# unanan/UNet_Nested4Tiny_Objects_Keypoints

Hardware: AMD Instinct MI355X
Metric: images/sec (train step) UNet++ L=4 256x256 (higher is better)
Workload: dtype f32

## Files before the change

### include/unetpp_hip.h

```cpp
#ifndef UNETPP_HIP_H
#define UNETPP_HIP_H

#include <stdint.h>

#ifdef __cplusplus
extern "C" {
#endif

#define UNETPP_ABI_VERSION 13
#define UNETPP_MAX_VIEWS 8

#define UNETPP_OK 0
#define UNETPP_EINVAL (-1)
#define UNETPP_ELAUNCH (-2)

typedef struct unetpp_view {
  float* ptr;
  int32_t C, c_off, c_len;
  int32_t Hs, Ws;
  int32_t sy, sx, oy, ox;
  const float* scale;
  const float* shift;
  const float* gate;
  int32_t relu;
  int32_t accumulate;
  int32_t gate_sum;
  int32_t reserved;
} unetpp_view;

#define UNETPP_GEMM_DIRECT 1
#define UNETPP_GEMM_BF16 2
typedef struct unetpp_bn_fused {
  const float* gamma;
  const float* beta;
  float* running_mean;
  float* running_var;
  float* mean;
  float* invstd;
  float* scale;
  float* shift;
  int64_t count;
  float eps, momentum;
} unetpp_bn_fused;

typedef struct unetpp_gemm_desc {
  int32_t N, H, W;
  int32_t taps;
  int32_t n_in;
  int32_t n_out;
  int32_t flags;
  int32_t reserved;
  unetpp_view in[UNETPP_MAX_VIEWS];
  unetpp_view out[UNETPP_MAX_VIEWS];
  const float* weight;
  const float* bias;
  float* stats_partial;
  const float* weight_image;
  unetpp_bn_fused bn;
} unetpp_gemm_desc;

typedef struct unetpp_wgrad_desc {
  int32_t N, H, W;
  int32_t taps;
  int32_t n_x;
  int32_t n_dy;
  unetpp_view x[UNETPP_MAX_VIEWS];
  unetpp_view dy[UNETPP_MAX_VIEWS];
  int32_t n_split;
  int32_t flags;
  float* slabs;
} unetpp_wgrad_desc;

int unetpp_abi_version(void);
const char* unetpp_build_arch(void);

const char* unetpp_last_kernel_name(void);

int unetpp_debug_set(const char* name, int64_t value, int32_t set);
int unetpp_debug_get(const char* name, int64_t* value);

int32_t unetpp_set_reserved_cus(int32_t n);
int32_t unetpp_usable_cus(int32_t* physical);

int64_t unetpp_gemm_pixel_blocks(int32_t N, int32_t H, int32_t W);
int64_t unetpp_gemm_stats_rows(int32_t N, int32_t H, int32_t W);
typedef struct unetpp_gemm_sizes {
  int64_t image_floats;
  int64_t bn_rows;
  int32_t workgroups, threads;
  const char* kernel;
} unetpp_gemm_sizes;
int unetpp_gemm_plan(const unetpp_gemm_desc* d, int32_t cus, unetpp_gemm_sizes* out);
int unetpp_gemm_fwd(const unetpp_gemm_desc* d, void* stream);
int64_t unetpp_gemm_weight_image_floats(const unetpp_gemm_desc* d);
int unetpp_gemm_pack_weight_image(const unetpp_gemm_desc* d, float* image, void* stream);
typedef struct unetpp_weight_src {
  const float* src;
  int64_t s_t, s_k, s_ko, s_n, s_no;
  int32_t k_inner, n_inner, flip, reserved;
} unetpp_weight_src;
int unetpp_gemm_pack_weight_image_from(const unetpp_gemm_desc* d, const unetpp_weight_src* src, float* image, void* stream);
typedef struct unetpp_pack_job {
  unetpp_weight_src src;
  float* image;
  int32_t taps, flags, n_in, n_out;
  int32_t in_len[UNETPP_MAX_VIEWS], out_len[UNETPP_MAX_VIEWS];
} unetpp_pack_job;
int unetpp_gemm_pack_weight_images(const unetpp_pack_job* jobs_device, int32_t n_jobs, int64_t max_image_floats,
                                   void* stream);

typedef struct unetpp_wgrad_sizes {
  int32_t n_split;
  int32_t planes;
  int32_t pairs_per_workgroup;
  int32_t reserved;
  int64_t slab_floats;
  const char* kernel;
} unetpp_wgrad_sizes;
int unetpp_wgrad_plan(const unetpp_wgrad_desc* d, int32_t target_blocks, unetpp_wgrad_sizes* out);
int unetpp_wgrad(const unetpp_wgrad_desc* d, void* stream);
int unetpp_wgrad_finish(const float* slabs, int32_t n_split, int32_t taps, int32_t K, int32_t Ncols, int32_t n_inner,
                        float* dw, int64_t d_t, int64_t d_k, int64_t d_n, int64_t d_o, float* db, void* stream);

int unetpp_pack_weight(float* dst, const float* src, int32_t T, int32_t K, int32_t Ncols,
                       int64_t d_t, int64_t d_k, int64_t d_n, int64_t s_t, int64_t s_k, int64_t s_n,
                       int32_t flip, void* stream);
typedef struct unetpp_copy_job {
  const float* src;
  float* dst;
  int64_t n_outer, n_inner, src_stride, dst_stride;
} unetpp_copy_job;
int unetpp_copy_jobs(const unetpp_copy_job* jobs_device, int32_t n_jobs, int64_t max_elems, void* stream);

int unetpp_bn_finalize(const float* partial, int64_t n_blocks, int32_t C, int64_t count,
                       const float* gamma, const float* beta, float eps, float momentum,
                       float* running_mean, float* running_var,
                       float* mean, float* invstd, float* scale, float* shift, void* stream);
int unetpp_bn_eval_coeffs(const float* gamma, const float* beta, const float* running_mean,
                          const float* running_var, float eps, int32_t C, float* scale, float* shift,
                          void* stream);
int unetpp_bn_eval_coeffs_stats(const float* gamma, const float* beta, const float* running_mean,
                                const float* running_var, float eps, int32_t C, float* scale, float* shift,
                                float* mean, float* invstd, void* stream);
int unetpp_affine_relu_pool(const float* y, const float* scale, const float* shift, int32_t relu,
                            int32_t N, int32_t H, int32_t W, int32_t C,
                            float* act, float* pooled, uint8_t* pool_idx, void* stream);
int unetpp_maxpool_bwd(const float* d_pooled, const uint8_t* pool_idx, int32_t N, int32_t H, int32_t W,
                       int32_t C, float* d_act, void* stream);
int64_t unetpp_bn_bwd_blocks(int64_t pixels, int32_t C);
int unetpp_bn_bwd_reduce(const float* d_act, const float* y, const float* scale, const float* shift,
                         const float* mean, const float* invstd, int64_t pixels, int32_t C,
                         float* partial, void* stream);
int unetpp_bn_bwd_finalize(const float* partial, int64_t n_blocks, int32_t C, float* dgamma, float* dbeta,
                           void* stream);
int unetpp_bn_bwd_apply(const float* d_act, const float* y, const float* scale, const float* shift,
                        const float* mean, const float* invstd, const float* gamma,
                        const float* dgamma, const float* dbeta, int64_t pixels, int32_t C,
                        float* dy, void* stream);

int unetpp_bn_bwd_pool_ok(int32_t N, int32_t H, int32_t W, int32_t C);
int unetpp_bn_bwd_reduce_pool(const float* d_act, const float* y, const float* scale, const float* shift,
                              const float* mean, const float* invstd, const float* d_pooled, const uint8_t* pool_idx,
                              int32_t N, int32_t H, int32_t W, int32_t C, float* partial, void* stream);
int unetpp_bn_bwd_apply_pool(const float* d_act, const float* y, const float* scale, const float* shift,
                             const float* mean, const float* invstd, const float* gamma, const float* dgamma,
                             const float* dbeta, const float* d_pooled, const uint8_t* pool_idx, int32_t N, int32_t H,
                             int32_t W, int32_t C, float* dy, void* stream);

int64_t unetpp_bn_frozen_bwd_blocks(int64_t pixels, int32_t C);
int unetpp_bn_frozen_bwd(const float* d_act, const float* y, const float* scale, const float* shift,
                         const float* mean, const float* invstd, const float* d_pooled, const uint8_t* pool_idx,
                         int32_t N, int32_t H, int32_t W, int32_t C, float* dy, float* partial, void* stream);

int unetpp_head_fwd(const float* x, const float* weight, const float* bias, int32_t N, int32_t H, int32_t W,
                    int32_t C, int32_t n_cls, float p_drop, uint64_t seed, const uint8_t* mask, const uint64_t* seed_dev,
                    float* out_nchw, void* stream);
int64_t unetpp_head_bwd_blocks(int64_t pixels);
int unetpp_head_bwd(const float* d_out_nchw, const float* out_nchw, const float* x, const float* weight,
                    int32_t N, int32_t H, int32_t W, int32_t C, int32_t n_cls, float p_drop, uint64_t seed,
                    const uint8_t* mask, const uint64_t* seed_dev, float* dx, int32_t accumulate, int32_t gate_x, float* partial,
                    void* stream);
int unetpp_head_train(const float* x, const float* weight, const float* bias, const float* target_nchw, int32_t N,
                      int32_t H, int32_t W, int32_t C, int32_t n_cls, float p_drop, uint64_t seed, const uint8_t* mask,
                      const uint64_t* seed_dev, int64_t rows, float gamma, int32_t n_heads, float* out_nchw, float* dx,
                      int32_t gate_x, float* partial, void* stream);
int unetpp_sum_partials(const float* partial, int64_t n_blocks, int64_t len, float* out, void* stream);

int unetpp_bilinear2x_fwd(const float* x, int32_t N, int32_t H, int32_t W, int32_t C, float* y, void* stream);
int unetpp_bilinear2x_bwd(const float* dy, int32_t N, int32_t H, int32_t W, int32_t C, float* dx, int32_t accumulate,
                          void* stream);

int64_t unetpp_focal_bce_blocks(int64_t n);
int unetpp_focal_bce(const float* pred, const float* target, int64_t n, int64_t rows, float gamma, float* grad,
                     float* partial, float* loss, void* stream);
#define UNETPP_MAX_HEADS 8
typedef struct unetpp_focal_heads {
  const float* pred[UNETPP_MAX_HEADS];
  float* grad[UNETPP_MAX_HEADS];
  int32_t n_heads, reserved;
} unetpp_focal_heads;
int unetpp_focal_bce_heads(const unetpp_focal_heads* heads, const float* target, int64_t n, int64_t rows, float gamma,
                           float* partial, float* loss, void* stream);
int64_t unetpp_topk_focal_workspace_bytes(int32_t n_heads, int64_t rows, int64_t P);
int unetpp_topk_focal_heads(const unetpp_focal_heads* heads, const float* target, int64_t rows, int64_t P, int64_t k,
                            int64_t denom, float gamma, void* workspace, float* kth, float* loss, void* stream);
int64_t unetpp_pr_focal_workspace_bytes(int32_t n_heads, int64_t n);
int unetpp_pr_focal_heads(const unetpp_focal_heads* heads, const float* target, int64_t n, float alpha, float beta,
                          float eps, float positive, void* workspace, int64_t* n_pos, float* loss ,
                          void* stream);
int unetpp_focal_bce_heads_ignore(const unetpp_focal_heads* heads, const float* target, int64_t n, int64_t rows,
                                  float gamma, float* partial, float* loss, void* stream);
int unetpp_topk_focal_heads_ignore(const unetpp_focal_heads* heads, const float* target, int64_t rows, int64_t P,
                                   int64_t k, int64_t denom, float gamma, void* workspace, float* kth, float* loss,
                                   void* stream);
int unetpp_pr_focal_heads_ignore(const unetpp_focal_heads* heads, const float* target, int64_t n, float alpha, float beta,
                                 float eps, float positive, void* workspace, int64_t* n_pos,
                                 float* loss , void* stream);
typedef struct unetpp_head_src {
  const void* x;
  const float* weight;
  const float* bias;
} unetpp_head_src;
typedef struct unetpp_heads_mean {
  unetpp_head_src head[UNETPP_MAX_HEADS];
  int32_t n_heads, reserved;
} unetpp_heads_mean;
int unetpp_heads_mean_fwd(const unetpp_heads_mean* heads, int32_t N, int32_t H, int32_t W, int32_t C, int32_t n_cls,
                          float* out_nchw, void* stream);
int unetpp_heads_mean_fwd_bf16(const unetpp_heads_mean* heads, int32_t N, int32_t H, int32_t W, int32_t C,
                               int32_t n_cls, float* out_nchw, void* stream);
typedef struct unetpp_head_grad {
  void* dx;
  float* partial;
  int32_t accumulate, gate_x;
} unetpp_head_grad;
typedef struct unetpp_heads_mean_grad {
  unetpp_head_grad head[UNETPP_MAX_HEADS];
  int32_t n_heads, reserved;
} unetpp_heads_mean_grad;
int unetpp_heads_mean_bwd(const unetpp_heads_mean* heads, const unetpp_heads_mean_grad* grads, const float* d_out_nchw,
                          int32_t N, int32_t H, int32_t W, int32_t C, int32_t n_cls, void* stream);
int unetpp_heads_mean_bwd_bf16(const unetpp_heads_mean* heads, const unetpp_heads_mean_grad* grads,
                               const float* d_out_nchw, int32_t N, int32_t H, int32_t W, int32_t C, int32_t n_cls,
                               void* stream);
int64_t unetpp_heatmap_workspace_bytes(int32_t N, int32_t H, int32_t W);
int unetpp_create_heatmap(const float* points, int32_t N, int32_t P, int32_t H, int32_t W, float radius,
                          float* out_nchw, void* workspace, void* stream);

int unetpp_nchw_to_nhwc(const float* src, int32_t N, int32_t C, int32_t H, int32_t W, float* dst, void* stream);
int unetpp_nhwc_to_nchw(const float* src, int32_t N, int32_t C, int32_t H, int32_t W, float* dst, void* stream);

int unetpp_affine_relu_pool_bf16(const void* y, const float* scale, const float* shift, int32_t relu,
                                 int32_t N, int32_t H, int32_t W, int32_t C,
                                 void* act, void* pooled, uint8_t* pool_idx, void* stream);
int64_t unetpp_bn_bwd_blocks_bf16(int64_t pixels, int32_t C);
int unetpp_bn_bwd_reduce_bf16(const void* d_act, const void* y, const float* scale, const float* shift,
                              const float* mean, const float* invstd, const void* d_pooled, const uint8_t* pool_idx,
                              int32_t N, int32_t H, int32_t W, int32_t C, float* partial, void* stream);
int unetpp_bn_bwd_apply_bf16(const void* d_act, const void* y, const float* scale, const float* shift,
                             const float* mean, const float* invstd, const float* gamma, const float* dgamma,
                             const float* dbeta, const void* d_pooled, const uint8_t* pool_idx,
                             int32_t N, int32_t H, int32_t W, int32_t C, void* dy, void* stream);
int64_t unetpp_bn_frozen_bwd_blocks_bf16(int64_t pixels, int32_t C);
int unetpp_bn_frozen_bwd_bf16(const void* d_act, const void* y, const float* scale, const float* shift,
                              const float* mean, const float* invstd, const void* d_pooled, const uint8_t* pool_idx,
                              int32_t N, int32_t H, int32_t W, int32_t C, void* dy, float* partial, void* stream);
int unetpp_head_fwd_bf16(const void* x, const float* weight, const float* bias, int32_t N, int32_t H, int32_t W,
                         int32_t C, int32_t n_cls, float p_drop, uint64_t seed, const uint8_t* mask, const uint64_t* seed_dev,
                         float* out_nchw, void* stream);
int unetpp_head_bwd_bf16(const float* d_out_nchw, const float* out_nchw, const void* x, const float* weight,
                         int32_t N, int32_t H, int32_t W, int32_t C, int32_t n_cls, float p_drop, uint64_t seed,
                         const uint8_t* mask, const uint64_t* seed_dev, void* dx, int32_t accumulate, int32_t gate_x, float* partial,
                         void* stream);

int unetpp_maxpool_bwd_bf16(const void* d_pooled, const uint8_t* pool_idx, int32_t N, int32_t H, int32_t W, int32_t C,
                            void* d_act, const void* gate, void* stream);
int unetpp_bilinear2x_fwd_bf16(const void* x, int32_t N, int32_t H, int32_t W, int32_t C, void* y, void* stream);
int unetpp_bilinear2x_bwd_bf16(const void* dy, int32_t N, int32_t H, int32_t W, int32_t C, void* dx, int32_t accumulate,
                               const void* gate, void* stream);

int unetpp_first_layer_dgrad_bf16(const void* dy, const float* weight, int32_t N, int32_t H, int32_t W, int32_t CIN,
                                  int32_t COUT, float* dx, void* stream);

int64_t unetpp_heatmap_pattern_workspace_bytes(int32_t N, int32_t n_maps, int32_t H, int32_t W);
int unetpp_heatmap_pattern(const float* points, int32_t N, int32_t P, const int32_t* map_points,
                           const int32_t* map_begin, int32_t n_maps, int32_t H, int32_t W, float radius,
                           float* out_nchw, void* workspace, void* stream);
int64_t unetpp_keypoints_workspace_bytes(int32_t maps, int32_t H, int32_t W, int32_t max_regions);
int unetpp_keypoints_extract(int32_t stage, const float* heat, int32_t maps, int32_t H, int32_t W,
                             const float* thr_per_map, int32_t num, int32_t max_regions, int32_t sweeps,
                             void* workspace, int32_t* changed, float* points, int32_t* counts, void* stream);

#define UNETPP_OPTIM_ADAMW 0
#define UNETPP_OPTIM_ADABOUND 1
#define UNETPP_OPTIM_SGDW 2
#define UNETPP_OPTIM_AMS 1
#define UNETPP_OPTIM_CAPTURABLE 2
#define UNETPP_OPTIM_HYPER 8
#define UNETPP_OPTIM_H_MAX_NORM 7
#define UNETPP_OPTIM_SKIP_NONFINITE 4

typedef struct unetpp_optim_segment {
  float* param;
  const float* grad;
  float* exp_avg;
  float* exp_avg_sq;
  float* aux;
  float* step;
  int64_t numel;
  int64_t chunk_begin;
  int32_t group;
  int32_t vec;
} unetpp_optim_segment;

int64_t unetpp_optim_chunk_elems(void);
int unetpp_optim_step(int32_t kind, int32_t flags, const unetpp_optim_segment* segments, int32_t n_segments,
                      const int32_t* chunk_segment, int64_t n_chunks, const double* hyper, const double* steps,
                      int32_t* done, void* stream);
int unetpp_optim_upload(void* dst, const void* host_src, int64_t bytes, void* stream);

typedef struct unetpp_clip_state {
  float total_norm;
  float coef;
  int32_t skipped_steps;
  int32_t reserved;
} unetpp_clip_state;

int unetpp_grad_norm(const unetpp_optim_segment* segments, int32_t n_segments, const int32_t* chunk_segment,
                     int64_t n_chunks, double* partials, void* stream);
int unetpp_optim_step_clip(int32_t kind, int32_t flags, const unetpp_optim_segment* segments, int32_t n_segments,
                           const int32_t* chunk_segment, int64_t n_chunks, const double* hyper, const double* steps,
                           int32_t* done, const double* partials, unetpp_clip_state* state, void* stream);
int unetpp_grad_scale(const unetpp_optim_segment* segments, int32_t n_segments, const int32_t* chunk_segment,
                      int64_t n_chunks, const double* partials, float max_norm, unetpp_clip_state* state, void* stream);

#define UNETPP_MATCH_MAX 64

int unetpp_match_points(const float* points, const int32_t* found, int32_t heads, int32_t N, int32_t C, int32_t K,
                        const float* labels, int32_t S, const int32_t* map_points, const int32_t* map_begin,
                        float* matched, uint8_t* mask, float* loss, int32_t* count, void* stream);

#define UNETPP_AVG_MEAN 0
#define UNETPP_AVG_EMA 1
#define UNETPP_AVG_SWAP 2
#define UNETPP_AVG_CAPTURABLE 1

typedef struct unetpp_avg_segment {
  float* avg;
  float* src;
  int64_t numel;
  int64_t chunk_begin;
  int32_t vec;
  int32_t copy;
} unetpp_avg_segment;

int unetpp_avg_update(int32_t kind, int32_t flags, const unetpp_avg_segment* segments, int32_t n_segments,
                      const int32_t* chunk_segment, int64_t n_chunks, int64_t count, double decay, float* count_dev,
                      const double* hyper_dev, int32_t* done, void* stream);

#define UNETPP_WARP_PARAMS 16
#define UNETPP_WARP_MAX_C 8
#define UNETPP_STORE_U8 0
#define UNETPP_STORE_F32 1

int unetpp_warp_batch(const void* store, int32_t store_type, int64_t M, int32_t Hs, int32_t Ws, int32_t C,
                      const int64_t* index, int32_t N, const float* params, const float* mul, const float* add,
                      float fill, float* out, int32_t Ho, int32_t Wo, const float* labels, int32_t S,
                      float* labels_out, uint8_t* inside, void* stream);

typedef struct unetpp_augment {
  float p_flip_h, p_flip_v;
  int32_t rot90;
  float max_deg;
  float scale_lo, scale_hi;
  float max_tx, max_ty;
  float gain_lo, gain_hi;
  float max_bias;
  int32_t reserved;
} unetpp_augment;

int unetpp_augment_draw(float* params, int32_t N, uint64_t seed, int32_t Hs, int32_t Ws, int32_t Ho, int32_t Wo,
                        const unetpp_augment* augment, void* stream);

#define UNETPP_SCENE_MAX_VARIANTS 8
#define UNETPP_SCENE_FLIP_X 1
#define UNETPP_SCENE_FLIP_Y 2
#define UNETPP_SCENE_TRANSPOSE 4

typedef struct unetpp_scene_rect {
  int32_t frame;
  int32_t oy, ox;
  int32_t y_lo, y_hi, x_lo, x_hi;
  int32_t reserved;
} unetpp_scene_rect;

int unetpp_scene_stitch(const float* tiles, int32_t n_tiles, int32_t K, int32_t C, int32_t Th, int32_t Tw,
// ... 35 lines not shown
```

### unet_nested4tiny_objects_keypoints_amd/_lib.py

```python
from __future__ import annotations

import ctypes as C
import os
import subprocess

_PKG_DIR = os.path.dirname(os.path.abspath(__file__))
_REPO = os.path.dirname(_PKG_DIR)
LIB_PATH = os.environ.get("UNETPP_LIB", os.path.join(_PKG_DIR, "libunetpp_hip.so"))
CSRC = os.path.join(_PKG_DIR, "csrc")
INCLUDE = os.path.join(_REPO, "include")
SOURCES = ("gemm_pix.hip", "gemm_fast.hip", "gemm_pw.hip", "gemm_pw_bf16.hip", "gemm_wino.hip", "gemm_bf16.hip", "gemm_bf16_dma.hip", "wgrad_bf16.hip", "pointwise_bf16.hip", "keypoints.hip", "weight_image.hip", "wgrad.hip", "wgrad_fast.hip", "wgrad_dma.hip", "wgrad_pw.hip", "wgrad_wino.hip", "first_layer.hip", "pointwise.hip", "heads.hip", "caller.hip", "optim.hip", "validate.hip", "average.hip", "loader.hip", "scene.hip",
           "detect.hip", "crops.hip", "topk_loss.hip", "pr_focal.hip")
HEADERS = ("common.h", "gemm_units.h", "wgrad_reduce.h", "lds_asm.h", "bf16_common.h", "dropout.h", "bn_fused.h",
           "wino_experiments.h", "dma_experiments.h", "heads_mean.h", "head_select.h", "focal_element.h", "multi_tensor.h")
MAX_VIEWS = 8
ABI_VERSION = 13
EXTRA_FLAGS = {"gemm_wino.hip": ("-fno-slp-vectorize",), "wgrad_wino.hip": ("-fno-slp-vectorize",)}
GEMM_DIRECT = 1
GEMM_BF16 = 2


class View(C.Structure):
    _fields_ = [
        ("ptr", C.c_void_p),
        ("C", C.c_int32), ("c_off", C.c_int32), ("c_len", C.c_int32),
        ("Hs", C.c_int32), ("Ws", C.c_int32),
        ("sy", C.c_int32), ("sx", C.c_int32), ("oy", C.c_int32), ("ox", C.c_int32),
        ("scale", C.c_void_p), ("shift", C.c_void_p), ("gate", C.c_void_p),
        ("relu", C.c_int32), ("accumulate", C.c_int32), ("gate_sum", C.c_int32), ("reserved", C.c_int32),
    ]


class BnFused(C.Structure):
    _fields_ = [
        ("gamma", C.c_void_p), ("beta", C.c_void_p), ("running_mean", C.c_void_p), ("running_var", C.c_void_p),
        ("mean", C.c_void_p), ("invstd", C.c_void_p), ("scale", C.c_void_p), ("shift", C.c_void_p),
        ("count", C.c_int64), ("eps", C.c_float), ("momentum", C.c_float),
    ]


class GemmDesc(C.Structure):
    _fields_ = [
        ("N", C.c_int32), ("H", C.c_int32), ("W", C.c_int32),
        ("taps", C.c_int32), ("n_in", C.c_int32), ("n_out", C.c_int32),
        ("flags", C.c_int32), ("reserved", C.c_int32),
        ("inp", View * MAX_VIEWS), ("out", View * MAX_VIEWS),
        ("weight", C.c_void_p), ("bias", C.c_void_p), ("stats_partial", C.c_void_p),
        ("weight_image", C.c_void_p),
        ("bn", BnFused),
    ]


class WeightSrc(C.Structure):
    _fields_ = [
        ("src", C.c_void_p),
        ("s_t", C.c_int64), ("s_k", C.c_int64), ("s_ko", C.c_int64), ("s_n", C.c_int64), ("s_no", C.c_int64),
        ("k_inner", C.c_int32), ("n_inner", C.c_int32), ("flip", C.c_int32), ("reserved", C.c_int32),
    ]


class PackJob(C.Structure):
    _fields_ = [
        ("src", WeightSrc),
        ("image", C.c_void_p),
        ("taps", C.c_int32), ("flags", C.c_int32), ("n_in", C.c_int32), ("n_out", C.c_int32),
        ("in_len", C.c_int32 * MAX_VIEWS), ("out_len", C.c_int32 * MAX_VIEWS),
    ]


class CopyJob(C.Structure):
    _fields_ = [
        ("src", C.c_void_p), ("dst", C.c_void_p),
        ("n_outer", C.c_int64), ("n_inner", C.c_int64), ("src_stride", C.c_int64), ("dst_stride", C.c_int64),
    ]


MAX_HEADS = 8


class FocalHeads(C.Structure):
    _fields_ = [
        ("pred", C.c_void_p * MAX_HEADS), ("grad", C.c_void_p * MAX_HEADS),
        ("n_heads", C.c_int32), ("reserved", C.c_int32),
    ]


class HeadSrc(C.Structure):
    _fields_ = [("x", C.c_void_p), ("weight", C.c_void_p), ("bias", C.c_void_p)]


class HeadsMean(C.Structure):
    _fields_ = [("head", HeadSrc * MAX_HEADS), ("n_heads", C.c_int32), ("reserved", C.c_int32)]


class HeadGrad(C.Structure):
    _fields_ = [("dx", C.c_void_p), ("partial", C.c_void_p), ("accumulate", C.c_int32), ("gate_x", C.c_int32)]


class HeadsMeanGrad(C.Structure):
    _fields_ = [("head", HeadGrad * MAX_HEADS), ("n_heads", C.c_int32), ("reserved", C.c_int32)]


class WgradDesc(C.Structure):
    _fields_ = [
        ("N", C.c_int32), ("H", C.c_int32), ("W", C.c_int32),
        ("taps", C.c_int32), ("n_x", C.c_int32), ("n_dy", C.c_int32),
        ("x", View * MAX_VIEWS), ("dy", View * MAX_VIEWS),
        ("n_split", C.c_int32), ("flags", C.c_int32),
        ("slabs", C.c_void_p),
    ]


class WgradSizes(C.Structure):
    _fields_ = [
        ("n_split", C.c_int32), ("planes", C.c_int32), ("pairs_per_workgroup", C.c_int32), ("reserved", C.c_int32),
        ("slab_floats", C.c_int64),
        ("kernel", C.c_char_p),
    ]


class GemmSizes(C.Structure):
    _fields_ = [
        ("image_floats", C.c_int64), ("bn_rows", C.c_int64),
        ("workgroups", C.c_int32), ("threads", C.c_int32),
        ("kernel", C.c_char_p),
    ]


class OptimSegment(C.Structure):
    _fields_ = [
        ("param", C.c_void_p), ("grad", C.c_void_p), ("exp_avg", C.c_void_p), ("exp_avg_sq", C.c_void_p),
        ("aux", C.c_void_p), ("step", C.c_void_p),
        ("numel", C.c_int64), ("chunk_begin", C.c_int64), ("group", C.c_int32), ("vec", C.c_int32),
    ]


class ClipState(C.Structure):
    _fields_ = [("total_norm", C.c_float), ("coef", C.c_float), ("skipped_steps", C.c_int32), ("reserved", C.c_int32)]


class AvgSegment(C.Structure):
    _fields_ = [
        ("avg", C.c_void_p), ("src", C.c_void_p),
        ("numel", C.c_int64), ("chunk_begin", C.c_int64), ("vec", C.c_int32), ("copy", C.c_int32),
    ]


class AugmentDesc(C.Structure):
    _fields_ = [
        ("p_flip_h", C.c_float), ("p_flip_v", C.c_float), ("rot90", C.c_int32), ("max_deg", C.c_float),
        ("scale_lo", C.c_float), ("scale_hi", C.c_float), ("max_tx", C.c_float), ("max_ty", C.c_float),
        ("gain_lo", C.c_float), ("gain_hi", C.c_float), ("max_bias", C.c_float), ("reserved", C.c_int32),
    ]


class SceneRect(C.Structure):
    _fields_ = [
        ("frame", C.c_int32), ("oy", C.c_int32), ("ox", C.c_int32),
        ("y_lo", C.c_int32), ("y_hi", C.c_int32), ("x_lo", C.c_int32), ("x_hi", C.c_int32), ("reserved", C.c_int32),
    ]


OPTIM_ADAMW, OPTIM_ADABOUND, OPTIM_SGDW = 0, 1, 2
OPTIM_AMS, OPTIM_CAPTURABLE = 1, 2
OPTIM_SKIP_NONFINITE = 4
OPTIM_HYPER = 8
OPTIM_H_MAX_NORM = 7
AVG_MEAN, AVG_EMA, AVG_SWAP = 0, 1, 2
AVG_CAPTURABLE = 1
WARP_PARAMS, WARP_MAX_C = 16, 8
STORE_U8, STORE_F32 = 0, 1
SCENE_MAX_VARIANTS = 8
SCENE_FLIP_X, SCENE_FLIP_Y, SCENE_TRANSPOSE = 1, 2, 4
PEAKS_MAX_RADIUS, PEAKS_MAX_MAPS = 8, 65535
MATCH_MAX = 64

_P, _I32, _I64, _F, _U64 = C.c_void_p, C.c_int32, C.c_int64, C.c_float, C.c_uint64

SIGNATURES = {
    "unetpp_abi_version": (C.c_int, []),
    "unetpp_build_arch": (C.c_char_p, []),
    "unetpp_last_kernel_name": (C.c_char_p, []),
    "unetpp_set_reserved_cus": (_I32, [_I32]),
    "unetpp_debug_set": (C.c_int, [C.c_char_p, _I64, _I32]),
    "unetpp_debug_get": (C.c_int, [C.c_char_p, C.POINTER(C.c_int64)]),
    "unetpp_usable_cus": (_I32, [C.POINTER(C.c_int32)]),
    "unetpp_gemm_pixel_blocks": (_I64, [_I32, _I32, _I32]),
    "unetpp_gemm_stats_rows": (_I64, [_I32, _I32, _I32]),
    "unetpp_gemm_plan": (C.c_int, [C.POINTER(GemmDesc), _I32, C.POINTER(GemmSizes)]),
    "unetpp_gemm_fwd": (C.c_int, [C.POINTER(GemmDesc), _P]),
    "unetpp_gemm_weight_image_floats": (_I64, [C.POINTER(GemmDesc)]),
    "unetpp_gemm_pack_weight_image": (C.c_int, [C.POINTER(GemmDesc), _P, _P]),
    "unetpp_gemm_pack_weight_image_from": (C.c_int, [C.POINTER(GemmDesc), C.POINTER(WeightSrc), _P, _P]),
    "unetpp_gemm_pack_weight_images": (C.c_int, [_P, _I32, _I64, _P]),
    "unetpp_wgrad_plan": (C.c_int, [C.POINTER(WgradDesc), _I32, C.POINTER(WgradSizes)]),
    "unetpp_wgrad": (C.c_int, [C.POINTER(WgradDesc), _P]),
    "unetpp_wgrad_finish": (C.c_int, [_P, _I32, _I32, _I32, _I32, _I32, _P, _I64, _I64, _I64, _I64, _P, _P]),
    "unetpp_pack_weight": (C.c_int, [_P, _P, _I32, _I32, _I32, _I64, _I64, _I64, _I64, _I64, _I64, _I32, _P]),
    "unetpp_bn_finalize": (C.c_int, [_P, _I64, _I32, _I64, _P, _P, _F, _F, _P, _P, _P, _P, _P, _P, _P]),
    "unetpp_bn_eval_coeffs": (C.c_int, [_P, _P, _P, _P, _F, _I32, _P, _P, _P]),
    "unetpp_affine_relu_pool": (C.c_int, [_P, _P, _P, _I32, _I32, _I32, _I32, _I32, _P, _P, _P, _P]),
    "unetpp_maxpool_bwd": (C.c_int, [_P, _P, _I32, _I32, _I32, _I32, _P, _P]),
    "unetpp_bn_bwd_blocks": (_I64, [_I64, _I32]),
    "unetpp_bn_bwd_reduce": (C.c_int, [_P, _P, _P, _P, _P, _P, _I64, _I32, _P, _P]),
    "unetpp_bn_bwd_finalize": (C.c_int, [_P, _I64, _I32, _P, _P, _P]),
    "unetpp_bn_bwd_apply": (C.c_int, [_P, _P, _P, _P, _P, _P, _P, _P, _P, _I64, _I32, _P, _P]),
    "unetpp_bn_bwd_pool_ok": (C.c_int, [_I32, _I32, _I32, _I32]),
    "unetpp_bn_bwd_reduce_pool": (C.c_int, [_P, _P, _P, _P, _P, _P, _P, _P, _I32, _I32, _I32, _I32, _P, _P]),
    "unetpp_bn_bwd_apply_pool": (C.c_int, [_P, _P, _P, _P, _P, _P, _P, _P, _P, _P, _P, _I32, _I32, _I32, _I32, _P, _P]),
    "unetpp_head_fwd": (C.c_int, [_P, _P, _P, _I32, _I32, _I32, _I32, _I32, _F, _U64, _P, _P, _P, _P]),
    "unetpp_head_bwd_blocks": (_I64, [_I64]),
    "unetpp_head_bwd": (C.c_int, [_P, _P, _P, _P, _I32, _I32, _I32, _I32, _I32, _F, _U64, _P, _P, _P, _I32, _I32, _P, _P]),
    "unetpp_head_train": (C.c_int, [_P, _P, _P, _P, _I32, _I32, _I32, _I32, _I32, _F, _U64, _P, _P, _I64, _F, _I32, _P, _P,
                                    _I32, _P, _P]),
    "unetpp_sum_partials": (C.c_int, [_P, _I64, _I64, _P, _P]),
    "unetpp_focal_bce_blocks": (_I64, [_I64]),
    "unetpp_focal_bce": (C.c_int, [_P, _P, _I64, _I64, _F, _P, _P, _P, _P]),
    "unetpp_focal_bce_heads": (C.c_int, [C.POINTER(FocalHeads), _P, _I64, _I64, _F, _P, _P, _P]),
    "unetpp_heads_mean_fwd": (C.c_int, [C.POINTER(HeadsMean), _I32, _I32, _I32, _I32, _I32, _P, _P]),
    "unetpp_heads_mean_fwd_bf16": (C.c_int, [C.POINTER(HeadsMean), _I32, _I32, _I32, _I32, _I32, _P, _P]),
    "unetpp_heads_mean_bwd": (C.c_int, [C.POINTER(HeadsMean), C.POINTER(HeadsMeanGrad), _P, _I32, _I32, _I32, _I32, _I32, _P]),
    "unetpp_heads_mean_bwd_bf16": (C.c_int, [C.POINTER(HeadsMean), C.POINTER(HeadsMeanGrad), _P, _I32, _I32, _I32, _I32, _I32,
                                             _P]),
    "unetpp_bn_eval_coeffs_stats": (C.c_int, [_P, _P, _P, _P, _F, _I32, _P, _P, _P, _P, _P]),
    "unetpp_bn_frozen_bwd_blocks": (_I64, [_I64, _I32]),
    "unetpp_bn_frozen_bwd": (C.c_int, [_P, _P, _P, _P, _P, _P, _P, _P, _I32, _I32, _I32, _I32, _P, _P, _P]),
    "unetpp_bn_frozen_bwd_blocks_bf16": (_I64, [_I64, _I32]),
    "unetpp_bn_frozen_bwd_bf16": (C.c_int, [_P, _P, _P, _P, _P, _P, _P, _P, _I32, _I32, _I32, _I32, _P, _P, _P]),
    "unetpp_copy_jobs": (C.c_int, [_P, _I32, _I64, _P]),
    "unetpp_heatmap_workspace_bytes": (_I64, [_I32, _I32, _I32]),
    "unetpp_create_heatmap": (C.c_int, [_P, _I32, _I32, _I32, _I32, _F, _P, _P, _P]),
    "unetpp_bilinear2x_fwd": (C.c_int, [_P, _I32, _I32, _I32, _I32, _P, _P]),
    "unetpp_bilinear2x_bwd": (C.c_int, [_P, _I32, _I32, _I32, _I32, _P, _I32, _P]),
    "unetpp_nchw_to_nhwc": (C.c_int, [_P, _I32, _I32, _I32, _I32, _P, _P]),
    "unetpp_nhwc_to_nchw": (C.c_int, [_P, _I32, _I32, _I32, _I32, _P, _P]),
    "unetpp_affine_relu_pool_bf16": (C.c_int, [_P, _P, _P, _I32, _I32, _I32, _I32, _I32, _P, _P, _P, _P]),
    "unetpp_bn_bwd_blocks_bf16": (_I64, [_I64, _I32]),
    "unetpp_bn_bwd_reduce_bf16": (C.c_int, [_P, _P, _P, _P, _P, _P, _P, _P, _I32, _I32, _I32, _I32, _P, _P]),
    "unetpp_bn_bwd_apply_bf16": (C.c_int, [_P, _P, _P, _P, _P, _P, _P, _P, _P, _P, _P, _I32, _I32, _I32, _I32, _P, _P]),
    "unetpp_head_fwd_bf16": (C.c_int, [_P, _P, _P, _I32, _I32, _I32, _I32, _I32, _F, _U64, _P, _P, _P, _P]),
    "unetpp_first_layer_dgrad_bf16": (C.c_int, [_P, _P, _I32, _I32, _I32, _I32, _I32, _P, _P]),
    "unetpp_maxpool_bwd_bf16": (C.c_int, [_P, _P, _I32, _I32, _I32, _I32, _P, _P, _P]),
    "unetpp_bilinear2x_fwd_bf16": (C.c_int, [_P, _I32, _I32, _I32, _I32, _P, _P]),
    "unetpp_bilinear2x_bwd_bf16": (C.c_int, [_P, _I32, _I32, _I32, _I32, _P, _I32, _P, _P]),
    "unetpp_heatmap_pattern_workspace_bytes": (_I64, [_I32, _I32, _I32, _I32]),
    "unetpp_heatmap_pattern": (C.c_int, [_P, _I32, _I32, _P, _P, _I32, _I32, _I32, _F, _P, _P, _P]),
    "unetpp_keypoints_workspace_bytes": (_I64, [_I32, _I32, _I32, _I32]),
    "unetpp_keypoints_extract": (C.c_int, [_I32, _P, _I32, _I32, _I32, _P, _I32, _I32, _I32, _P, _P, _P, _P, _P]),
    "unetpp_head_bwd_bf16": (C.c_int, [_P, _P, _P, _P, _I32, _I32, _I32, _I32, _I32, _F, _U64, _P, _P, _P, _I32, _I32, _P, _P]),
    "unetpp_optim_chunk_elems": (_I64, []),
    "unetpp_optim_step": (C.c_int, [_I32, _I32, _P, _I32, _P, _I64, _P, _P, _P, _P]),
    "unetpp_optim_upload": (C.c_int, [_P, _P, _I64, _P]),
    "unetpp_match_points": (C.c_int, [_P, _P, _I32, _I32, _I32, _I32, _P, _I32, _P, _P, _P, _P, _P, _P, _P]),
    "unetpp_avg_update": (C.c_int, [_I32, _I32, _P, _I32, _P, _I64, _I64, C.c_double, _P, _P, _P, _P]),
    "unetpp_grad_norm": (C.c_int, [_P, _I32, _P, _I64, _P, _P]),
    "unetpp_optim_step_clip": (C.c_int, [_I32, _I32, _P, _I32, _P, _I64, _P, _P, _P, _P, _P, _P]),
    "unetpp_grad_scale": (C.c_int, [_P, _I32, _P, _I64, _P, _F, _P, _P]),
    "unetpp_warp_batch": (C.c_int, [_P, _I32, _I64, _I32, _I32, _I32, _P, _I32, _P, _P, _P, _F, _P, _I32, _I32, _P, _I32,
                                    _P, _P, _P]),
    "unetpp_augment_draw": (C.c_int, [_P, _I32, _U64, _I32, _I32, _I32, _I32, C.POINTER(AugmentDesc), _P]),
    "unetpp_scene_stitch": (C.c_int, [_P, _I32, _I32, _I32, _I32, _I32, C.POINTER(C.c_int32), C.POINTER(SceneRect), _P, _P,
                                      _I32, _I32, _I32, _P]),
    "unetpp_scene_screen": (C.c_int, [_P, _I32, _I32, _I32, _I32, C.POINTER(SceneRect), _P, _I32, _F, _P, _P, _P]),
    "unetpp_peaks_workspace_bytes": (_I64, [_I32, _I32, _I32]),
    "unetpp_peaks_detect": (C.c_int, [_P, _I32, _I32, _I32, _F, _I32, _I32, _I32, _P, _P, _P, _P, _P]),
    "unetpp_detect_match": (C.c_int, [_P, _P, _P, _I32, _I32, _I32, _P, _P, _I32, _F, _P, _P, _P, _P]),
    "unetpp_points_target": (C.c_int, [_P, _P, _I64, _I32, _P, _I32, _P, _I32, _I32, _I32, _F, _P, _P]),
    "unetpp_crops_draw": (C.c_int, [_P, _P, _P, _I32, _U64, _I32, _I32, _I32, _I32, _I32, _P, _P, _I32, _F, _F, _F,
                                    C.POINTER(AugmentDesc), _P]),
    "unetpp_topk_focal_workspace_bytes": (_I64, [_I32, _I64, _I64]),
    "unetpp_topk_focal_heads": (C.c_int, [C.POINTER(FocalHeads), _P, _I64, _I64, _I64, _I64, _F, _P, _P, _P, _P]),
    "unetpp_pr_focal_workspace_bytes": (_I64, [_I32, _I64]),
    "unetpp_pr_focal_heads": (C.c_int, [C.POINTER(FocalHeads), _P, _I64, _F, _F, _F, _F, _P, _P, _P, _P]),
    "unetpp_focal_bce_heads_ignore": (C.c_int, [C.POINTER(FocalHeads), _P, _I64, _I64, _F, _P, _P, _P]),
    "unetpp_topk_focal_heads_ignore": (C.c_int, [C.POINTER(FocalHeads), _P, _I64, _I64, _I64, _I64, _F, _P, _P, _P, _P]),
    "unetpp_pr_focal_heads_ignore": (C.c_int, [C.POINTER(FocalHeads), _P, _I64, _F, _F, _F, _F, _P, _P, _P, _P]),
    "unetpp_target_ignore": (C.c_int, [_P, _P, _I64, _I32, _P, _I32, _P, _I32, _I32, _I32, _I32, _I32, _I32, _P, _P]),
}

_LIB = None


def source_hash() -> str:
    import hashlib
    h = hashlib.sha256()
    for path in [os.path.join(CSRC, s) for s in SOURCES + HEADERS] + [os.path.join(INCLUDE, "unetpp_hip.h")]:
        with open(path, "rb") as f:
            h.update(f.read())
    return h.hexdigest()[:16]


def build_library(force: bool = False, verbose: bool = False, out_path: str = None, obj_dir: str = None) -> str:
    srcs = [os.path.join(CSRC, s) for s in SOURCES]
    deps = srcs + [os.path.join(CSRC, h) for h in HEADERS] + [os.path.join(INCLUDE, "unetpp_hip.h")]
    lib_path = out_path or LIB_PATH
    if not force and os.path.exists(lib_path) and all(os.path.getmtime(lib_path) >= os.path.getmtime(d) for d in deps):
        return lib_path
    hipcc = os.environ.get("HIPCC", "/opt/rocm/bin/hipcc")
    common = [hipcc, "--offload-arch=gfx950", "-O3", "-std=c++17", "-fPIC", "-I", INCLUDE, "-I", CSRC]
    obj_dir = obj_dir or os.path.join(_REPO, "build", "obj")
    os.makedirs(obj_dir, exist_ok=True)
    jobs = []
    for src in SOURCES:
        obj = os.path.join(obj_dir, src.replace(".hip", ".o"))
        cmd = common + list(EXTRA_FLAGS.get(src, ())) + ["-c", os.path.join(CSRC, src), "-o", obj]
        if verbose:
            print(" ".join(cmd))
        jobs.append((obj, cmd, subprocess.Popen(cmd)))
    for obj, cmd, proc in jobs:
        if proc.wait() != 0:
            raise subprocess.CalledProcessError(proc.returncode, cmd)
    staged = os.path.join(obj_dir, os.path.basename(lib_path) + ".link")
    link = [hipcc, "--offload-arch=gfx950", "-shared", "-fPIC", "-o", staged] + [j[0] for j in jobs]
    if verbose:
        print(" ".join(link))
    subprocess.run(link, check=True)
    os.replace(staged, lib_path)
    if out_path is None:
        global _LIB
        _LIB = None
    return lib_path


def lib():
    global _LIB
    if _LIB is None:
        if not os.path.exists(LIB_PATH):
            raise RuntimeError(
                "unetpp HIP library not built: %s is missing. Run `python -c 'import __graft_entry__ as g; g.build()'` "
                "(there is no CPU fallback for this path)." % LIB_PATH)
        handle = C.CDLL(LIB_PATH)
        for name, (res, args) in SIGNATURES.items():
            fn = getattr(handle, name)
            fn.restype = res
            fn.argtypes = args
        if handle.unetpp_abi_version() != ABI_VERSION:
            raise RuntimeError("unetpp HIP library ABI mismatch")
        _LIB = handle
    return _LIB


def check(status: int, what: str) -> None:
    if status != 0:
        raise RuntimeError("%s failed with status %d (%s)" % (
            what, status, {-1: "invalid argument", -2: "kernel launch error"}.get(status, "unknown")))


class debug_switch:

    def __init__(self, name: str, value: int):
        self.name, self.value = name.encode(), int(value)
        self._before = None

    def __enter__(self):
        old = C.c_int64(0)
        state = lib().unetpp_debug_get(self.name, C.byref(old))
        if state < 0:
            check(state, "unetpp_debug_get")
        self._before = (state == 1, int(old.value))
        check(lib().unetpp_debug_set(self.name, self.value, 1), "unetpp_debug_set")
        return self

    def __exit__(self, *exc):
        was_set, value = self._before
        check(lib().unetpp_debug_set(self.name, value if was_set else 0, 1 if was_set else 0), "unetpp_debug_set")
        return False
```

### unet_nested4tiny_objects_keypoints_amd/csrc/common.h

```cpp
#pragma once
#include <hip/hip_runtime.h>
#include <stdint.h>

#include <atomic>

#include "unetpp_hip.h"

typedef float f32x16 __attribute__((ext_vector_type(16)));
typedef float f32x4 __attribute__((ext_vector_type(4)));

namespace unetpp {

constexpr int kBlockPixels = 256;
constexpr int kThreads = 256;
constexpr int kMaxHaloPixels = 340;

struct TileGeom {
  int log2tw, tiles_x, tiles_y;
};

inline TileGeom tile_geom(int H, int W) {
  int l = 3;
  while ((1 << l) < W && l < 5) ++l;
  TileGeom g;
  g.log2tw = l;
  const int TW = 1 << l, TH = kBlockPixels >> l;
  g.tiles_x = (W + TW - 1) / TW;
  g.tiles_y = (H + TH - 1) / TH;
  return g;
}

template <int OFF>
__device__ __forceinline__ float xor_lane(float v) {
  static_assert(OFF == 1 || OFF == 2 || OFF == 4 || OFF == 8 || OFF == 16, "xor_lane: 1, 2, 4, 8 or 16");
  const int i = __builtin_bit_cast(int, v);
  int r;
  if constexpr (OFF == 1) r = __builtin_amdgcn_mov_dpp(i, 0xB1, 0xF, 0xF, true);
  else if constexpr (OFF == 2) r = __builtin_amdgcn_mov_dpp(i, 0x4E, 0xF, 0xF, true);
  else r = __builtin_amdgcn_ds_swizzle(i, 0x1F | (OFF << 10));
  return __builtin_bit_cast(float, r);
}

__device__ __forceinline__ float row16_sum(float v) {
  v += xor_lane<1>(v);
  v += xor_lane<2>(v);
  v += __builtin_bit_cast(float, __builtin_amdgcn_mov_dpp(__builtin_bit_cast(int, v), 0x141, 0xF, 0xF, true));
  v += __builtin_bit_cast(float, __builtin_amdgcn_mov_dpp(__builtin_bit_cast(int, v), 0x140, 0xF, 0xF, true));
  return v;
}

__device__ __forceinline__ float relu_keep_nan(float v) { return !(v <= 0.f) ? v : 0.f; }
__device__ __forceinline__ float relu_floor(bool relu) { return relu ? 0.f : -__builtin_inff(); }
__device__ __forceinline__ float floor_keep_nan(float v, float floor_v) { return !(v <= floor_v) ? v : floor_v; }

__device__ __forceinline__ bool pool_takes(float t, float best) { return t > best || t != t; }

inline int finish_log2_groups(int n_split) {
  int l = 0;
  while ((1 << l) < n_split && l < 4) ++l;
  return l;
}

inline bool view_ok(const unetpp_view& v, bool need_ptr = true) {
  if (need_ptr && v.ptr == nullptr) return false;
  if (v.C <= 0 || v.c_len <= 0 || v.c_off < 0 || v.c_off + v.c_len > v.C) return false;
  if (v.Hs <= 0 || v.Ws <= 0 || v.sy <= 0 || v.sx <= 0 || v.oy < 0 || v.ox < 0) return false;
  if ((v.scale == nullptr) != (v.shift == nullptr)) return false;
  return true;
}

inline bool view_covers(const unetpp_view& v, int H, int W) {
  return (H - 1) * v.sy + v.oy < v.Hs && (W - 1) * v.sx + v.ox < v.Ws;
}

__device__ __forceinline__ bool view_vec4(const unetpp_view& v) {
  return ((v.C | v.c_off) & 3) == 0 && ((reinterpret_cast<uintptr_t>(v.ptr) & 15) == 0) &&
         (v.gate == nullptr || (reinterpret_cast<uintptr_t>(v.gate) & 15) == 0);
}

__device__ __forceinline__ long view_pixel_offset(const unetpp_view& v, int n, int y, int x) {
  return ((static_cast<long>(n) * v.Hs + (y * v.sy + v.oy)) * v.Ws + (x * v.sx + v.ox)) * v.C + v.c_off;
}

__device__ __forceinline__ f32x4 view_load4(const unetpp_view& v, long off, int c, int rem, bool vec) {
  f32x4 val = {0.f, 0.f, 0.f, 0.f};
  const float* p = v.ptr + off + c;
  if (vec && rem >= 4) {
    val = *reinterpret_cast<const f32x4*>(p);
  } else {
#pragma unroll
    for (int i = 0; i < 4; ++i)
      if (i < rem) val[i] = p[i];
  }
  if (v.scale != nullptr) {
#pragma unroll
    for (int i = 0; i < 4; ++i)
      if (i < rem) val[i] = fmaf(val[i], v.scale[c + i], v.shift[c + i]);
  }
  if (v.relu) {
#pragma unroll
    for (int i = 0; i < 4; ++i) val[i] = relu_keep_nan(val[i]);
  }
  if (v.gate != nullptr) {
    const float* g = v.gate + off + c;
#pragma unroll
    for (int i = 0; i < 4; ++i)
      if (i < rem) val[i] = (g[i] > 0.f) ? val[i] : 0.f;
  }
  return val;
}

inline hipStream_t ST(void* s) { return static_cast<hipStream_t>(s); }
inline bool aligned16(const void* p) { return (reinterpret_cast<uintptr_t>(p) & 15) == 0; }
inline unsigned grid_for(long items, long cap = 2048 * 8) {
  long b = (items + kThreads - 1) / kThreads;
  if (b < 1) b = 1;
  if (b > cap) b = cap;
  return static_cast<unsigned>(b);
}

inline int launch_status() { return hipGetLastError() == hipSuccess ? UNETPP_OK : UNETPP_ELAUNCH; }

constexpr int kMaxDevices = 64;
inline bool allow_dynamic_lds(const void* func, int bytes, std::atomic<bool> (&raised)[kMaxDevices]) {
  int dev = 0;
  if (hipGetDevice(&dev) != hipSuccess || dev < 0 || dev >= kMaxDevices) return false;
  if (raised[dev].load(std::memory_order_acquire)) return true;
  if (hipFuncSetAttribute(func, hipFuncAttributeMaxDynamicSharedMemorySize, bytes) != hipSuccess) return false;
  raised[dev].store(true, std::memory_order_release);
  return true;
}

int reserved_cus();
inline int physical_cu_count() {
  static int cached[64] = {};
  int dev = 0;
  if (hipGetDevice(&dev) != hipSuccess || dev < 0) return 0;
  if (dev < 64 && cached[dev] > 0) return cached[dev];
  int cus = 0;
  if (hipDeviceGetAttribute(&cus, hipDeviceAttributeMultiprocessorCount, dev) != hipSuccess || cus <= 0) return 0;
  if (dev < 64) cached[dev] = cus;
  return cus;
}
inline int device_cu_count() {
  const int cus = physical_cu_count();
  if (cus <= 0) return 0;
  const int left = cus - reserved_cus();
  return left < 8 ? (cus < 8 ? cus : 8) : left;
}

void note_kernel(const char* name);

enum Opt {
  OPT_BF16_NO_DMA,
  OPT_BF16_DMA_ALL,
  OPT_BF16_DMA_MIN8,
  OPT_BF16_DMA_FORM,
  OPT_BF16_DMA_SMALL,
  OPT_BF16_DMA_STATS,
  OPT_BF16_DMA_POINTWISE,
  OPT_BF16_DMA_SPLIT,
  OPT_BF16_WGRAD_QUAD,
  OPT_WINO_NO_LEAN,
  OPT_WINO_ONE_PER_CU,
  OPT_MEMSET_NODES,
  OPT_BF16_PW_PLAIN,
  OPT_PW_DIRECT,
  OPT_PW_NT,
  OPT_HEAD_WGS_PER_CU,
  OPT_SMALL_WGRAD_BLOCKS,
  OPT_COUNT
};
bool opt_is_set(Opt o);
long opt_value(Opt o, long dflt);

struct FastArgs;
struct GemmSel;
int gemm_select(const unetpp_gemm_desc* d, int cus, GemmSel& s);
bool gemm_image_of(const unetpp_gemm_desc* d, GemmSel& s);
bool small_cin_fwd_applies(const unetpp_gemm_desc* d);
void small_cin_fwd_plan(const unetpp_gemm_desc* d, GemmSel& s);
int launch_small_cin_fwd(const unetpp_gemm_desc* d, const GemmSel& s, hipStream_t st);
bool gemm_pw_bf16_applies(const unetpp_gemm_desc* d, GemmSel& s);
int launch_gemm_pw_bf16(const unetpp_gemm_desc* d, const GemmSel& s, hipStream_t st);
bool gemm_bf16_dma_applies(const unetpp_gemm_desc* d, GemmSel& s);
int launch_gemm_bf16_dma(const unetpp_gemm_desc* d, const GemmSel& s, hipStream_t st);
bool bf16_gemm_args(const unetpp_gemm_desc* d, FastArgs& a);
void gemm_bf16_plan(const unetpp_gemm_desc* d, GemmSel& s);
int launch_gemm_bf16(const unetpp_gemm_desc* d, const GemmSel& s, hipStream_t st);
bool wino_applies(const unetpp_gemm_desc* d);
void gemm_wino_plan(const unetpp_gemm_desc* d, GemmSel& s);
int launch_gemm_wino(const unetpp_gemm_desc* d, const GemmSel& s, hipStream_t st);
bool gemm_pw_applies(const unetpp_gemm_desc* d, GemmSel& s);
int launch_gemm_pw(const unetpp_gemm_desc* d, const GemmSel& s, hipStream_t st);
void gemm_fast_plan(const unetpp_gemm_desc* d, GemmSel& s);
int launch_gemm_fast(const unetpp_gemm_desc* d, const GemmSel& s, hipStream_t st);
enum WgradKernel {
  WGRAD_FIRST_LAYER, WGRAD_BF16_QUAD, WGRAD_BF16_PAIR, WGRAD_PW, WGRAD_WINO, WGRAD_DMA, WGRAD_FAST, WGRAD_GENERIC
};
struct WgradSel {
  WgradKernel kernel;
  const char* label;
  int planes;
  int pairs_per_workgroup;
  int max_split;
  int Ktot, Ncols;
  int k_tiles, n_tiles_cols;
};
int wgrad_select(const unetpp_wgrad_desc* d, WgradSel& s);
bool small_cin_wgrad_applies(const unetpp_wgrad_desc* d);
int launch_small_cin_wgrad(const unetpp_wgrad_desc* d, hipStream_t st);
bool wgrad_bf16_views_ok(const unetpp_wgrad_desc* d);
bool wgrad_bf16_quads(const unetpp_wgrad_desc* d);
int launch_wgrad_bf16(const unetpp_wgrad_desc* d, const WgradSel& s, hipStream_t st);
bool wgrad_pw_applies(const unetpp_wgrad_desc* d);
int launch_wgrad_pw(const unetpp_wgrad_desc* d, hipStream_t st);
bool wgrad_wino_applies(const unetpp_wgrad_desc* d);
int launch_wgrad_wino(const unetpp_wgrad_desc* d, const WgradSel& s, hipStream_t st);
int launch_wgrad_finish_wino(const float* slabs, int n_split, int K, int Ncols, float* dw, long d_t, long d_k, long d_n,
                             float* db, hipStream_t st);
bool wgrad_dma_applies(const unetpp_wgrad_desc* d);
int launch_wgrad_dma(const unetpp_wgrad_desc* d, const WgradSel& s, hipStream_t st);
bool wgrad_fast_applies(const unetpp_wgrad_desc* d);
int launch_wgrad_fast(const unetpp_wgrad_desc* d, const WgradSel& s, hipStream_t st);

}
```

### unet_nested4tiny_objects_keypoints_amd/csrc/gemm_pix.hip

```cpp
#include "bn_fused.h"
#include <atomic>
#include <cstdio>
#include <cstdlib>
#include <cstring>
#include <mutex>

#include "common.h"
#include "gemm_units.h"

namespace unetpp {
namespace {

constexpr int KC = 16;
constexpr int KCP = 20;
constexpr int WJ = 12;

struct GemmArgs {
  unetpp_gemm_desc d;
  int log2tw, tiles_x, tiles_y;
  int Ktot, Ncols;
};

template <int TAPS>
__global__ __launch_bounds__(kThreads, 2) void gemm_pix_kernel(const GemmArgs a) {
  constexpr int HALO = (TAPS == 9) ? 1 : 0;
  constexpr int IN_FLOATS = (TAPS == 9 ? kMaxHaloPixels : kBlockPixels) * KCP;
  constexpr int W_FLOATS = TAPS * (KC / 8) * 32 * WJ;
  __shared__ __attribute__((aligned(16))) float smem[IN_FLOATS + W_FLOATS];
  float* in_tile = smem;
  float* w_tile = smem + IN_FLOATS;

  const unetpp_gemm_desc& d = a.d;
  const int tid = threadIdx.x;
  const int wave = tid >> 6, lane = tid & 63, j = lane & 31, h = lane >> 5;

  int bid = blockIdx.x;
  const int txi = bid % a.tiles_x;
  bid /= a.tiles_x;
  const int tyi = bid % a.tiles_y;
  const int n = bid / a.tiles_y;
  const int TW = 1 << a.log2tw, TH = kBlockPixels >> a.log2tw;
  const int ty0 = tyi * TH, tx0 = txi * TW;
  const int HWp = TW + 2 * HALO, HHp = TH + 2 * HALO;
  const int npix = HWp * HHp;

  int ov = 0, nt = blockIdx.y, col_base = 0;
  while (ov < d.n_out - 1) {
    const int tiles_v = (d.out[ov].c_len + 31) >> 5;
    if (nt < tiles_v) break;
    nt -= tiles_v;
    col_base += d.out[ov].c_len;
    ++ov;
  }
  const unetpp_view& O = d.out[ov];
  const int n0 = col_base + nt * 32;
  const int n_cnt = min(32, O.c_len - nt * 32);

  int abase[2];
#pragma unroll
  for (int mt = 0; mt < 2; ++mt) {
    const int p = 64 * wave + 32 * mt + j;
    abase[mt] = ((p >> a.log2tw) * HWp + (p & (TW - 1))) * KCP + 4 * h;
  }
  const int wbase = j * WJ + 4 * h;

  f32x16 acc[2];
#pragma unroll
  for (int mt = 0; mt < 2; ++mt)
#pragma unroll
    for (int r = 0; r < 16; ++r) acc[mt][r] = 0.f;

  int kbase = 0;
  for (int s = 0; s < d.n_in; ++s) {
    const unetpp_view& V = d.in[s];
    const bool vec = view_vec4(V);
    for (int c0 = 0; c0 < V.c_len; c0 += KC) {
      const int c_cnt = min(KC, V.c_len - c0);
      __syncthreads();
      for (int it = tid; it < npix * (KC / 4); it += kThreads) {
        const int hp = it >> 2, cc = (it & 3) * 4;
        const int hy = hp / HWp, hx = hp - hy * HWp;
        const int y = ty0 + hy - HALO, x = tx0 + hx - HALO;
        f32x4 val = {0.f, 0.f, 0.f, 0.f};
        if (cc < c_cnt && y >= 0 && y < d.H && x >= 0 && x < d.W)
          val = view_load4(V, view_pixel_offset(V, n, y, x), c0 + cc, c_cnt - cc, vec);
        *reinterpret_cast<f32x4*>(&in_tile[hp * KCP + cc]) = val;
      }
      for (int it = tid; it < TAPS * (KC / 4) * 32; it += kThreads) {
        const int jj = it & 31, kq = (it >> 5) & 3, tap = it >> 7;
        f32x4 wv = {0.f, 0.f, 0.f, 0.f};
        if (jj < n_cnt) {
          const float* wp = d.weight + (static_cast<long>(tap) * a.Ktot + kbase + c0 + kq * 4) * a.Ncols + n0 + jj;
#pragma unroll
          for (int i = 0; i < 4; ++i)
            if (kq * 4 + i < c_cnt) wv[i] = wp[static_cast<long>(i) * a.Ncols];
        }
        *reinterpret_cast<f32x4*>(&w_tile[((tap * 2 + (kq >> 1)) * 32 + jj) * WJ + (kq & 1) * 4]) = wv;
      }
      __syncthreads();
      const int ngroups = (c_cnt + 7) >> 3;
#pragma unroll
      for (int tap = 0; tap < TAPS; ++tap) {
        const int toff = (TAPS == 9) ? ((tap / 3) * HWp + (tap % 3)) * KCP : 0;
#pragma unroll
        for (int g = 0; g < KC / 8; ++g) {
          if (g < ngroups) {
            const f32x4 b = *reinterpret_cast<const f32x4*>(&w_tile[(tap * 2 + g) * 32 * WJ + wbase]);
#pragma unroll
            for (int mt = 0; mt < 2; ++mt) {
              const f32x4 av = *reinterpret_cast<const f32x4*>(&in_tile[abase[mt] + toff + 8 * g]);
#pragma unroll
              for (int t = 0; t < 4; ++t)
                acc[mt] = __builtin_amdgcn_mfma_f32_32x32x2f32(av[t], b[t], acc[mt], 0, 0, 0);
            }
          }
        }
      }
    }
    kbase += V.c_len;
  }

  const bool col_ok = j < n_cnt;
  const float bj = (d.bias != nullptr && col_ok) ? d.bias[n0 + j] : 0.f;
  float s1 = 0.f, s2 = 0.f;
#pragma unroll
  for (int mt = 0; mt < 2; ++mt) {
#pragma unroll
    for (int r = 0; r < 16; ++r) {
      const int i = (r & 3) + 8 * (r >> 2) + 4 * h;
      const int p = 64 * wave + 32 * mt + i;
      const int y = ty0 + (p >> a.log2tw), x = tx0 + (p & (TW - 1));
      if (col_ok && y < d.H && x < d.W) {
        float v = acc[mt][r] + bj;
        v = floor_keep_nan(v, relu_floor(O.relu));
        s1 += v;
        s2 = fmaf(v, v, s2);
        const long off = view_pixel_offset(O, n, y, x) + nt * 32 + j;
        if (O.gate != nullptr && !O.gate_sum) v = (O.gate[off] > 0.f) ? v : 0.f;
        if (O.accumulate) v += O.ptr[off];
        if (O.gate != nullptr && O.gate_sum) v = (O.gate[off] > 0.f) ? v : 0.f;
        O.ptr[off] = v;
      }
    }
  }
  if (d.stats_partial != nullptr) {
    s1 += __shfl_xor(s1, 32);
    s2 += __shfl_xor(s2, 32);
    __syncthreads();
    if (h == 0) {
      smem[(wave * 32 + j) * 2 + 0] = s1;
      smem[(wave * 32 + j) * 2 + 1] = s2;
    }
    __syncthreads();
    if (tid < 32 && tid < n_cnt) {
      float t1 = 0.f, t2 = 0.f;
#pragma unroll
      for (int w = 0; w < 4; ++w) {
        t1 += smem[(w * 32 + tid) * 2 + 0];
        t2 += smem[(w * 32 + tid) * 2 + 1];
      }
      float* dst = d.stats_partial + (static_cast<long>(blockIdx.x) * a.Ncols + n0 + tid) * 2;
      dst[0] = t1;
      dst[1] = t2;
    }
  }
}

}
}

namespace unetpp {
namespace {
thread_local const char* g_last_kernel = "";

const char* const kOptNames[OPT_COUNT] = {
    "BF16_NO_DMA", "BF16_DMA_ALL", "BF16_DMA_MIN8", "BF16_DMA_FORM", "BF16_DMA_SMALL", "BF16_DMA_STATS",
    "BF16_DMA_POINTWISE", "BF16_DMA_SPLIT", "BF16_WGRAD_QUAD", "WINO_NO_LEAN", "WINO_ONE_PER_CU", "MEMSET_NODES",
    "BF16_PW_PLAIN", "PW_DIRECT", "PW_NT", "HEAD_WGS_PER_CU", "SMALL_WGRAD_BLOCKS"};
struct OptSlot {
  std::atomic<long> value{0};
  std::atomic<bool> set{false};
};
OptSlot g_opts[OPT_COUNT];
std::atomic<int> g_reserved_cus{0};
std::once_flag g_opts_once;

void opts_from_environment() {
  std::call_once(g_opts_once, [] {
    char name[64];
    for (int i = 0; i < OPT_COUNT; ++i) {
      snprintf(name, sizeof(name), "UNETPP_%s", kOptNames[i]);
      const char* e = getenv(name);
      if (e != nullptr) {
        char* end = nullptr;
        const long v = strtol(e, &end, 10);
        g_opts[i].value.store(end == e ? 1 : v, std::memory_order_relaxed);
        g_opts[i].set.store(true, std::memory_order_release);
      }
    }
    if (const char* e = getenv("UNETPP_RESERVED_CUS"); e != nullptr) {
      const int v = atoi(e);
      g_reserved_cus.store(v < 0 ? 0 : v, std::memory_order_relaxed);
    }
  });
}
}

bool opt_is_set(Opt o) {
  opts_from_environment();
  return g_opts[o].set.load(std::memory_order_acquire);
}
long opt_value(Opt o, long dflt) {
  opts_from_environment();
  return g_opts[o].set.load(std::memory_order_acquire) ? g_opts[o].value.load(std::memory_order_relaxed) : dflt;
}
int reserved_cus() {
  opts_from_environment();
  return g_reserved_cus.load(std::memory_order_relaxed);
}
void note_kernel(const char* name) { g_last_kernel = name; }
}

using namespace unetpp;

extern "C" const char* unetpp_last_kernel_name(void) { return g_last_kernel; }

extern "C" int unetpp_debug_set(const char* name, int64_t value, int32_t set) {
  if (name == nullptr) return UNETPP_EINVAL;
  opts_from_environment();
  for (int i = 0; i < OPT_COUNT; ++i)
    if (strcmp(name, kOptNames[i]) == 0) {
      g_opts[i].value.store(static_cast<long>(value), std::memory_order_relaxed);
      g_opts[i].set.store(set != 0, std::memory_order_release);
      return UNETPP_OK;
    }
  return UNETPP_EINVAL;
}

extern "C" int unetpp_debug_get(const char* name, int64_t* value) {
  if (name == nullptr) return UNETPP_EINVAL;
  opts_from_environment();
  for (int i = 0; i < OPT_COUNT; ++i)
    if (strcmp(name, kOptNames[i]) == 0) {
      if (!g_opts[i].set.load(std::memory_order_acquire)) return 0;
      if (value != nullptr) *value = g_opts[i].value.load(std::memory_order_relaxed);
      return 1;
    }
  return UNETPP_EINVAL;
}

extern "C" int32_t unetpp_set_reserved_cus(int32_t n) {
  opts_from_environment();
  if (n >= 0) {
    const int cus = physical_cu_count();
    const int cap = cus > 8 ? cus - 8 : 0;
    g_reserved_cus.store(n > cap ? cap : n, std::memory_order_relaxed);
  }
  return reserved_cus();
}

extern "C" int32_t unetpp_usable_cus(int32_t* physical) {
  if (physical != nullptr) *physical = physical_cu_count();
  return device_cu_count();
}

extern "C" int64_t unetpp_gemm_pixel_blocks(int32_t N, int32_t H, int32_t W) {
  if (N <= 0 || H <= 0 || W <= 0) return 0;
  const TileGeom g = tile_geom(H, W);
  return static_cast<int64_t>(N) * g.tiles_y * g.tiles_x;
}

extern "C" int64_t unetpp_gemm_stats_rows(int32_t N, int32_t H, int32_t W) {
  const int64_t blocks = unetpp_gemm_pixel_blocks(N, H, W);
  if (blocks <= 0) return 0;
  return blocks > kBnFusedRows ? blocks : kBnFusedRows;
}

bool unetpp::gemm_image_of(const unetpp_gemm_desc* d, GemmSel& s) {
  s.image_kind = s.image_kc = 0;
  s.image_floats = 0;
  if (d == nullptr) return false;
  const bool bf = (d->flags & UNETPP_GEMM_BF16) != 0, wino = wino_applies(d);
  const int kc = bf ? 32 : (wino ? 8 : 16);
  if (bf ? !bf16_gemm_args(d, s.fa) : !fast_args(d, s.fa, kc, 32)) return false;
  s.image_kind = bf ? kKindBf16 : (wino ? kKindWino : kKindFast);
  s.image_kc = kc;
  s.image_floats = static_cast<long>(s.fa.n_tiles) * s.fa.n_chunks * (wino ? 4096 : d->taps * 512L);
  return true;
}

namespace {
bool gemm_generic_applies(const unetpp_gemm_desc* d, GemmSel& s) {
  FastArgs& a = s.fa;
  a.Ktot = a.Ncols = a.n_tiles = 0;
  for (int i = 0; i < d->n_in; ++i) {
    if (!view_ok(d->in[i]) || !view_covers(d->in[i], d->H, d->W)) return false;
    a.Ktot += d->in[i].c_len;
  }
  for (int i = 0; i < d->n_out; ++i) {
    if (!view_ok(d->out[i]) || !view_covers(d->out[i], d->H, d->W)) return false;
    a.Ncols += d->out[i].c_len;
    a.n_tiles += (d->out[i].c_len + 31) / 32;
  }
  const TileGeom g = tile_geom(d->H, d->W);
  a.log2tw = g.log2tw;
  a.tiles_x = g.tiles_x;
  a.tiles_y = g.tiles_y;
  const int64_t pix_blocks = static_cast<int64_t>(d->N) * g.tiles_y * g.tiles_x;
  if (pix_blocks > 0x7fffffffLL || a.n_tiles > 65535) return false;
  s.kernel = GEMM_GENERIC;
  s.label = d->taps == 9 ? "gemm_pix_kernel<9>" : "gemm_pix_kernel<1>";
  s.grid_x = static_cast<unsigned>(pix_blocks);
  s.grid_y = static_cast<unsigned>(a.n_tiles);
  return true;
}

int launch_gemm_generic(const unetpp_gemm_desc* d, const GemmSel& s, hipStream_t st) {
  GemmArgs a;
  a.d = *d;
  a.log2tw = s.fa.log2tw;
  a.tiles_x = s.fa.tiles_x;
  a.tiles_y = s.fa.tiles_y;
  a.Ktot = s.fa.Ktot;
  a.Ncols = s.fa.Ncols;
  const dim3 grid(s.grid_x, s.grid_y);
  if (d->taps == 9)
    hipLaunchKernelGGL(gemm_pix_kernel<9>, grid, dim3(kThreads), 0, st, a);
  else
    hipLaunchKernelGGL(gemm_pix_kernel<1>, grid, dim3(kThreads), 0, st, a);
  return launch_status();
}
}

int unetpp::gemm_select(const unetpp_gemm_desc* d, int cus, GemmSel& s) {
  if (d == nullptr || d->N <= 0 || d->H <= 0 || d->W <= 0) return UNETPP_EINVAL;
  if (d->taps != 9 && d->taps != 1) return UNETPP_EINVAL;
  if (d->n_in < 1 || d->n_in > UNETPP_MAX_VIEWS || d->n_out < 1 || d->n_out > UNETPP_MAX_VIEWS) return UNETPP_EINVAL;
  if (d->weight == nullptr && d->weight_image == nullptr) return UNETPP_EINVAL;
  if (d->stats_partial != nullptr && d->n_out != 1) return UNETPP_EINVAL;
  const unetpp_bn_fused& bn = d->bn;
  if (bn.scale != nullptr &&
      (!d->stats_partial || !bn.gamma || !bn.beta || !bn.mean || !bn.invstd || !bn.shift || bn.count < 1 ||
       (bn.running_mean == nullptr) != (bn.running_var == nullptr) || d->n_out != 1))
    return UNETPP_EINVAL;
  const bool bf = (d->flags & UNETPP_GEMM_BF16) != 0;
  const bool has_image = gemm_image_of(d, s);
  s.cus = cus;
  s.grid_y = 1;
  s.threads = kThreads;
  s.lds_bytes = 0;
  s.bn_rows = 0;
  if (d->weight_image == nullptr) {
    const bool small = small_cin_fwd_applies(d);
    if (bf ? !small : !gemm_generic_applies(d, s)) return UNETPP_EINVAL;
    if (cus <= 0) return UNETPP_ELAUNCH;
    if (small) small_cin_fwd_plan(d, s);
    return UNETPP_OK;
  }
  if (!has_image) return UNETPP_EINVAL;
  if (cus <= 0) return UNETPP_ELAUNCH;
  if (bf) {
    if (!gemm_pw_bf16_applies(d, s) && !gemm_bf16_dma_applies(d, s)) gemm_bf16_plan(d, s);
  } else if (wino_applies(d)) {
    gemm_wino_plan(d, s);
  } else if (!gemm_pw_applies(d, s)) {
    gemm_fast_plan(d, s);
  }
  return UNETPP_OK;
}

extern "C" int unetpp_gemm_plan(const unetpp_gemm_desc* d, int32_t cus, unetpp_gemm_sizes* out) {
  GemmSel s;
  if (out == nullptr) return UNETPP_EINVAL;
  const int rc = gemm_select(d, cus > 0 ? cus : device_cu_count(), s);
  if (rc != UNETPP_OK) return rc;
  out->image_floats = s.image_floats;
  out->bn_rows = s.bn_rows;
  out->workgroups = static_cast<int32_t>(s.grid_x * s.grid_y);
  out->threads = static_cast<int32_t>(s.threads);
  out->kernel = s.label;
  return UNETPP_OK;
}

extern "C" int unetpp_gemm_fwd(const unetpp_gemm_desc* d, void* stream) {
  GemmSel s;
  int rc = gemm_select(d, device_cu_count(), s);
  if (rc != UNETPP_OK) return rc;
  hipStream_t st = static_cast<hipStream_t>(stream);
  note_kernel(s.label);
  switch (s.kernel) {
    case GEMM_SMALL_CIN: rc = launch_small_cin_fwd(d, s, st); break;
    case GEMM_BF16_PW: rc = launch_gemm_pw_bf16(d, s, st); break;
    case GEMM_BF16_DMA8:
    case GEMM_BF16_DMA4: rc = launch_gemm_bf16_dma(d, s, st); break;
    case GEMM_BF16: rc = launch_gemm_bf16(d, s, st); break;
    case GEMM_PW: rc = launch_gemm_pw(d, s, st); break;
    case GEMM_WINO: rc = launch_gemm_wino(d, s, st); break;
    case GEMM_FAST: rc = launch_gemm_fast(d, s, st); break;
    case GEMM_GENERIC: rc = launch_gemm_generic(d, s, st); break;
  }
  const unetpp_bn_fused& bn = d->bn;
  if (rc != UNETPP_OK || bn.scale == nullptr) return rc;
  const int64_t rows = s.bn_rows > 0 ? s.bn_rows : unetpp_gemm_pixel_blocks(d->N, d->H, d->W);
  const int fin = unetpp_bn_finalize(d->stats_partial, rows, d->out[0].c_len, bn.count, bn.gamma, bn.beta, bn.eps,
                                     bn.momentum, bn.running_mean, bn.running_var, bn.mean, bn.invstd, bn.scale, bn.shift,
                                     stream);
  note_kernel(s.label);
  return fin;
}
```

### unet_nested4tiny_objects_keypoints_amd/csrc/gemm_units.h

```cpp
#pragma once
#include "common.h"

namespace unetpp {

struct FastArgs {
  unetpp_gemm_desc d;
  int log2tw, tiles_x, tiles_y;
  int Ktot, Ncols, n_tiles, n_chunks;
  int nt_unit, n_groups;
  long total_blocks;
  int bn_in_kernel;
};

__device__ __forceinline__ unsigned view_pixel_offset32(const unetpp_view& v, int n, int y, int x) {
  return ((static_cast<unsigned>(n) * v.Hs + (y * v.sy + v.oy)) * v.Ws + (x * v.sx + v.ox)) * v.C + v.c_off;
}

__device__ __forceinline__ long xcd_remap(long bid, long total) {
  const long q = total >> 3, r = total & 7;
  const long xcd = bid & 7, idx = bid >> 3;
  return (xcd < r ? xcd * (q + 1) : r * (q + 1) + (xcd - r) * q) + idx;
}

struct UnitGeom {
  int n, ty0, tx0;
  int group;
  long patch;
};
struct TileCols {
  int nt, ov;
  int n0, n_cnt;
};

template <int LOG2N = 5>
__device__ __forceinline__ TileCols decode_tile(const FastArgs& a, int nt_global) {
  constexpr int NW = 1 << LOG2N;
  int nt = nt_global, ov = 0, col_base = 0;
  while (ov < a.d.n_out - 1) {
    const int tiles_v = (a.d.out[ov].c_len + NW - 1) >> LOG2N;
    if (nt < tiles_v) break;
    nt -= tiles_v;
    col_base += a.d.out[ov].c_len;
    ++ov;
  }
  TileCols t;
  t.nt = nt;
  t.ov = ov;
  t.n0 = col_base + nt * NW;
  t.n_cnt = min(NW, a.d.out[ov].c_len - nt * NW);
  return t;
}

template <int LOG2TW>
__device__ __forceinline__ UnitGeom decode_unit(const FastArgs& a, long lb) {
  constexpr int TW = 1 << LOG2TW, TH = kBlockPixels >> LOG2TW;
  UnitGeom g;
  unsigned bid = static_cast<unsigned>(lb);
  g.group = static_cast<int>(bid % static_cast<unsigned>(a.n_groups));
  bid /= static_cast<unsigned>(a.n_groups);
  g.patch = bid;
  const int txi = static_cast<int>(bid % static_cast<unsigned>(a.tiles_x));
  bid /= static_cast<unsigned>(a.tiles_x);
  const int tyi = static_cast<int>(bid % static_cast<unsigned>(a.tiles_y));
  g.n = static_cast<int>(bid / static_cast<unsigned>(a.tiles_y));
  g.ty0 = tyi * TH;
  g.tx0 = txi * TW;
  return g;
}

constexpr int kKindFast = 0, kKindWino = 1, kKindBf16 = 2;
enum GemmKernel {
  GEMM_SMALL_CIN, GEMM_BF16_PW, GEMM_BF16_DMA8, GEMM_BF16_DMA4, GEMM_BF16, GEMM_PW, GEMM_WINO, GEMM_FAST, GEMM_GENERIC
};
struct GemmSel {
  GemmKernel kernel;
  const char* label;
  int cus;
  int image_kind, image_kc;
  long image_floats;
  FastArgs fa;
  unsigned grid_x, grid_y, threads;
  int lds_bytes;
  long bn_rows;
  int qc, ncbp, plain, nt_store;
  int mode, narrow;
  int plain_out;
};

inline bool fast_args(const unetpp_gemm_desc* d, FastArgs& a, int kc, int ncol = 32) {
  if (d == nullptr || d->N <= 0 || d->H <= 0 || d->W <= 0) return false;
  if (d->taps != 9 && d->taps != 1) return false;
  if (d->n_in < 1 || d->n_in > UNETPP_MAX_VIEWS || d->n_out < 1 || d->n_out > UNETPP_MAX_VIEWS) return false;
  a.d = *d;
  a.bn_in_kernel = 0;
  a.Ktot = a.Ncols = a.n_tiles = a.n_chunks = 0;
  for (int i = 0; i < d->n_in; ++i) {
    const unetpp_view& v = d->in[i];
    if (!view_ok(v) || !view_covers(v, d->H, d->W)) return false;
    if (v.gate != nullptr) return false;
    if (v.scale != nullptr && ((reinterpret_cast<uintptr_t>(v.scale) | reinterpret_cast<uintptr_t>(v.shift)) & 15) != 0)
      return false;
    if (((v.C | v.c_off | v.c_len) & 3) != 0 || (reinterpret_cast<uintptr_t>(v.ptr) & 15) != 0) return false;
    if (static_cast<long>(d->N) * v.Hs * v.Ws * v.C >= 0x7fffffffL) return false;
    a.Ktot += v.c_len;
    a.n_chunks += (v.c_len + kc - 1) / kc;
  }
  for (int i = 0; i < d->n_out; ++i) {
    if (!view_ok(d->out[i]) || !view_covers(d->out[i], d->H, d->W)) return false;
    if (static_cast<long>(d->N) * d->out[i].Hs * d->out[i].Ws * d->out[i].C >= 0x7fffffffL) return false;
    a.Ncols += d->out[i].c_len;
    a.n_tiles += (d->out[i].c_len + ncol - 1) / ncol;
  }
  const TileGeom g = tile_geom(d->H, d->W);
  a.log2tw = g.log2tw;
  a.tiles_x = g.tiles_x;
  a.tiles_y = g.tiles_y;
  a.nt_unit = (d->taps == 1 && d->stats_partial == nullptr && a.n_tiles % 2 == 0) ? 2 : 1;
  a.n_groups = a.n_tiles / a.nt_unit;
  a.total_blocks = static_cast<long>(d->N) * g.tiles_y * g.tiles_x * a.n_groups;
  return a.total_blocks <= 0x7fffffffL;
}


struct UnitRange {
  long first, step, count;
};
__device__ __forceinline__ UnitRange my_unit_range(long total_blocks) {
  UnitRange u;
  const long W8 = gridDim.x >> 3;
  if (gridDim.x >= total_blocks) {
    u.first = xcd_remap(blockIdx.x, total_blocks);
    u.step = 0;
    u.count = 1;
  } else {
    const long q = total_blocks >> 3, r = total_blocks & 7;
    const long xcd = blockIdx.x & 7, widx = blockIdx.x >> 3;
    const long start = xcd < r ? xcd * (q + 1) : r * (q + 1) + (xcd - r) * q;
    const long cnt = q + (xcd < r ? 1 : 0);
    u.first = start + widx;
    u.step = W8;
    u.count = widx < cnt ? (cnt - widx + W8 - 1) / W8 : 0;
  }
  return u;
}

__device__ __forceinline__ UnitRange my_contiguous_unit_range(long total_blocks) {
  UnitRange u;
  const long W8 = gridDim.x >> 3;
  u.step = 1;
  if (gridDim.x >= total_blocks) {
    u.first = xcd_remap(blockIdx.x, total_blocks);
    u.count = 1;
  } else {
    const long q = total_blocks >> 3, r = total_blocks & 7;
    const long xcd = blockIdx.x & 7, widx = blockIdx.x >> 3;
    const long start = xcd < r ? xcd * (q + 1) : r * (q + 1) + (xcd - r) * q;
    const long cnt = q + (xcd < r ? 1 : 0);
    const long per = cnt / W8, rem = cnt % W8;
    u.first = start + widx * per + (widx < rem ? widx : rem);
    u.count = per + (widx < rem ? 1 : 0);
  }
  return u;
}

}
```

### unet_nested4tiny_objects_keypoints_amd/csrc/gemm_wino.hip

```cpp
#include <cstdlib>
#include <utility>

#include "bn_fused.h"
#include "common.h"
#include "gemm_units.h"
#include "lds_asm.h"
#include "wino_experiments.h"

namespace unetpp {
namespace {

typedef float f32x2 __attribute__((ext_vector_type(2)));
typedef unsigned u32x4v __attribute__((vector_size(16)));
constexpr unsigned kOutOfRange = 0x80000000u;
typedef const __attribute__((address_space(1))) void* gptr_t;
typedef __attribute__((address_space(3))) void* lptr_t;

__device__ __forceinline__ void wino_input_transform(const float (&dd)[16], float (&V)[16]) {
  float t[4][4];
#pragma unroll
  for (int j = 0; j < 4; ++j) {
    t[0][j] = dd[0 + j] - dd[8 + j];
    t[1][j] = dd[4 + j] + dd[8 + j];
    t[2][j] = dd[8 + j] - dd[4 + j];
    t[3][j] = dd[4 + j] - dd[12 + j];
  }
#pragma unroll
  for (int i = 0; i < 4; ++i) {
    V[4 * i + 0] = t[i][0] - t[i][2];
    V[4 * i + 1] = t[i][1] + t[i][2];
    V[4 * i + 2] = t[i][2] - t[i][1];
    V[4 * i + 3] = t[i][1] - t[i][3];
  }
}

__device__ __forceinline__ void wino_input_transform_pk(const f32x2_t (&dd)[8], float (&V)[16]) {
  f32x2_t t[8];
#pragma unroll
  for (int p = 0; p < 2; ++p) {
    t[0 + p] = pk_sub(dd[0 + p], dd[4 + p]);
    t[2 + p] = pk_add(dd[2 + p], dd[4 + p]);
    t[4 + p] = pk_sub(dd[4 + p], dd[2 + p]);
    t[6 + p] = pk_sub(dd[2 + p], dd[6 + p]);
  }
#pragma unroll
  for (int i = 0; i < 4; ++i) {
    const f32x2_t va = pk_sub_add_x(t[2 * i], t[2 * i + 1]);
    const f32x2_t vb = pk_cross_sub(t[2 * i], t[2 * i + 1]);
    V[4 * i + 0] = va[0];
    V[4 * i + 1] = va[1];
    V[4 * i + 2] = vb[0];
    V[4 * i + 3] = vb[1];
  }
}

constexpr int WKC = 8;
constexpr int WNC = 32;
constexpr int WP = 10;
constexpr int WIMG = 4096;

#define WINO_FENCE() __builtin_amdgcn_sched_barrier(0)

template <int LOG2TW, int NH, int MODE, bool BNF = false>
__global__ __launch_bounds__(kThreads, 2) void gemm_wino_kernel(const FastArgs a) {
  constexpr bool LEAN = MODE != 0, FOLD = MODE == 2;
  constexpr int TW = 1 << LOG2TW, TH = kBlockPixels >> LOG2TW;
  constexpr int HWp = TW + 2, HHp = TH + 2;
  constexpr int NPIX = HWp * HHp;
  constexpr int TXN = TW / 2;
  constexpr int IN_FLOATS = 4096;
  constexpr int IN_ITEMS = (NPIX * 2 + kThreads - 1) / kThreads;
  constexpr int W_ITEMS = WIMG / 4 / kThreads;
  static_assert(IN_ITEMS == 3 && W_ITEMS == 4, "the staging lambdas' default ranges");
  static_assert(kMaxHaloPixels * WP <= IN_FLOATS, "input patch does not fit");
  static_assert(((IN_ITEMS * kThreads - 1) >> 1) * WP + 8 <= IN_FLOATS, "staging items past the patch must stay inside the buffer");
  constexpr int BUF = IN_FLOATS + WIMG;
  __shared__ __attribute__((aligned(16))) float smem[2 * BUF];
  float* in_tile = smem;
  float* w_tile = smem + IN_FLOATS;
  constexpr int RUN0 = 4 * WNC * 2;
  __shared__ float stat_lds[BNF ? RUN0 + kBnFusedMaxCols * 2 : RUN0];
  constexpr int kBiasCols = 512;
  __shared__ __attribute__((aligned(16))) float bias_lds[kBiasCols];

  const unetpp_gemm_desc& d = a.d;
  const int tid = threadIdx.x;
  const int wave = __builtin_amdgcn_readfirstlane(tid >> 6), lane = tid & 63, t16 = lane & 15, g = lane >> 4;

  const UnitRange ur = my_contiguous_unit_range(a.total_blocks);
  for (int i = tid; i < kBiasCols; i += kThreads)
    bias_lds[i] = (a.d.bias != nullptr && i < a.Ncols) ? a.d.bias[i] : 0.f;
  constexpr bool bn_fused = BNF;
  if constexpr (BNF) {
    for (int i = tid; i < kBnFusedMaxCols * 2; i += kThreads) stat_lds[RUN0 + i] = 0.f;
  }
  if (ur.count == 0) {
    if constexpr (BNF) {
      __syncthreads();
      bn_rows_store<kThreads>(a.d.stats_partial, a.Ncols, stat_lds + RUN0);
    }
    return;
  }
  const int n_units = __builtin_amdgcn_readfirstlane(static_cast<int>(ur.count));

  const int my_tile = 16 * wave + t16;
  const int a_base = ((2 * (my_tile / TXN)) * HWp + 2 * (my_tile % TXN)) * WP + 2 * g;
  const int b_base = (g * 16 + t16) * 2;

  f32x4 acc[16][NH];
#pragma unroll
  for (int xi = 0; xi < 16; ++xi)
#pragma unroll
    for (int nh = 0; nh < NH; ++nh) acc[xi][nh] = f32x4{0.f, 0.f, 0.f, 0.f};

  f32x4 reg_in[IN_ITEMS];
  unsigned voff[IN_ITEMS];
  unsigned in_mask = 0;
  int pf_cnt = 0;
  int p_unit = 0;
  int p_s = 0, p_c0 = 0, p_chunk = 0;
  int p_n = 0, p_ty0 = 0, p_tx0 = 0;
  const float* p_wimg = nullptr;
  const int cc = (tid & 1) << 2;
  const float* v_ptr = nullptr;
  const float* v_scale = nullptr;
  const float* v_shift = nullptr;
  int v_clen = 0;
  bool v_relu = false;
  int v_bytes = 0, v_pitch = 0, v_origin = 0;
  int pix[IN_ITEMS];
  auto cache_view = [&]() {
    const unetpp_view& V = d.in[p_s];
    v_clen = V.c_len;
    if constexpr (LEAN) {
      v_ptr = V.ptr;
      v_bytes = d.N * V.Hs * V.Ws * V.C * 4;
      v_pitch = V.C * 4;
      v_origin = V.c_off * 4;
      if constexpr (FOLD) {
        v_scale = V.scale;
        v_shift = V.shift;
        v_relu = V.relu != 0;
      }
    } else {
      v_ptr = V.ptr;
      v_scale = V.scale;
      v_shift = V.shift;
      v_relu = V.relu != 0;
    }
  };

  auto step_unit = [&](UnitGeom& u) {
    if (++u.group < a.n_groups) return;
    u.group = 0;
    ++u.patch;
    u.tx0 += TW;
    if (u.tx0 < a.tiles_x * TW) return;
    u.tx0 = 0;
    u.ty0 += TH;
    if (u.ty0 < a.tiles_y * TH) return;
    u.ty0 = 0;
    ++u.n;
  };
  UnitGeom p_ug = decode_unit<LOG2TW>(a, ur.first);
  p_ug.n = __builtin_amdgcn_readfirstlane(p_ug.n);
  p_ug.ty0 = __builtin_amdgcn_readfirstlane(p_ug.ty0);
  p_ug.tx0 = __builtin_amdgcn_readfirstlane(p_ug.tx0);
  p_ug.group = __builtin_amdgcn_readfirstlane(p_ug.group);
  p_ug.patch = __builtin_amdgcn_readfirstlane(static_cast<int>(p_ug.patch));
  UnitGeom c_ug = p_ug;

  long p_patch = -1;
  auto prefetch_unit = [&]() -> bool {
    const UnitGeom& ug = p_ug;
    p_wimg = d.weight_image + static_cast<long>(ug.group) * a.n_chunks * WIMG;
    if (ug.patch == p_patch) return true;
    p_patch = ug.patch;
    p_n = ug.n;
    p_ty0 = ug.ty0;
    p_tx0 = ug.tx0;
    if constexpr (LEAN) {
      const int row0 = p_n * d.H;
#pragma unroll
      for (int q = 0; q < IN_ITEMS; ++q) {
        const int it = tid + q * kThreads;
        const int hp = it >> 1;
        const int hy = hp / HWp, hx = hp - hy * HWp;
        const int y = p_ty0 + hy - 1, x = p_tx0 + hx - 1;
        const bool in_patch = ((q + 1) * kThreads <= NPIX * 2) ? true : (it < NPIX * 2);
        const bool inside = in_patch & (static_cast<unsigned>(y) < static_cast<unsigned>(d.H)) &
                            (static_cast<unsigned>(x) < static_cast<unsigned>(d.W));
        const int linear = (row0 + y) * d.W + x;
        pix[q] = inside ? linear : -1;
      }
      return false;
    }
    in_mask = 0;
#pragma unroll
    for (int q = 0; q < IN_ITEMS; ++q) {
      const int it = tid + q * kThreads;
      const int hp = it >> 1;
      const int hy = hp / HWp, hx = hp - hy * HWp;
      const int y = p_ty0 + hy - 1, x = p_tx0 + hx - 1;
      if ((it < NPIX * 2) && y >= 0 && y < d.H && x >= 0 && x < d.W) in_mask |= 1u << q;
    }
    return false;
  };
  auto view_offsets = [&](const unetpp_view& V) {
    if constexpr (LEAN) {
#pragma unroll
      for (int q = 0; q < IN_ITEMS; ++q)
        voff[q] = static_cast<unsigned>(pix[q] * v_pitch + v_origin + cc * 4) |
                  (static_cast<unsigned>(pix[q] >> 31) & kOutOfRange);
      return;
    }
#pragma unroll
    for (int q = 0; q < IN_ITEMS; ++q) {
      const int hp = min((tid + q * kThreads) >> 1, NPIX - 1);
      const int hy = hp / HWp, hx = hp - hy * HWp;
      const int yy = min(max(p_ty0 + hy - 1, 0), d.H - 1), xx = min(max(p_tx0 + hx - 1, 0), d.W - 1);
      voff[q] = view_pixel_offset32(V, p_n, yy, xx);
    }
  };
  auto advance = [&]() {
    if (p_chunk + 1 < a.n_chunks) {
      ++p_chunk;
      p_c0 += WKC;
      if (p_c0 >= v_clen) {
        ++p_s;
        p_c0 = 0;
        cache_view();
        view_offsets(d.in[p_s]);
      }
    } else if (p_unit + 1 < n_units) {
      ++p_unit;
      p_chunk = 0;
      p_c0 = 0;
      const bool same_view = p_s == 0;
      if (!same_view) {
        p_s = 0;
        cache_view();
      }
      step_unit(p_ug);
      if (!prefetch_unit() || !same_view) view_offsets(d.in[0]);
    }
  };
  f32x4 co_sc = {1.f, 1.f, 1.f, 1.f}, co_sh = {0.f, 0.f, 0.f, 0.f};
  float co_floor = 0.f;
  auto load_coeffs = [&]() {
    if constexpr (!FOLD) return;
    co_floor = v_relu ? 0.f : -__builtin_inff();
    if (v_scale != nullptr) {
      co_sc = *reinterpret_cast<const f32x4*>(v_scale + p_c0 + cc);
      co_sh = *reinterpret_cast<const f32x4*>(v_shift + p_c0 + cc);
    } else {
      co_sc = f32x4{1.f, 1.f, 1.f, 1.f};
      co_sh = f32x4{0.f, 0.f, 0.f, 0.f};
    }
  };
  auto load_inputs = [&]() {
    if constexpr (LEAN) {
      const __amdgpu_buffer_rsrc_t v_rsrc =
          __builtin_amdgcn_make_buffer_rsrc(const_cast<float*>(v_ptr), 0, v_bytes, 0x00020000);
#pragma unroll
      for (int q = 0; q < IN_ITEMS; ++q) {
        const u32x4v v = __builtin_amdgcn_raw_buffer_load_b128(v_rsrc, static_cast<int>(voff[q]), p_c0 * 4, 0);
        reg_in[q] = __builtin_bit_cast(f32x4, v);
      }
      return;
    }
    pf_cnt = min(WKC, v_clen - p_c0);
#pragma unroll
    for (int q = 0; q < IN_ITEMS; ++q) {
      const unsigned off = voff[q] + static_cast<unsigned>(p_c0 + (cc < pf_cnt ? cc : 0));
      reg_in[q] = *reinterpret_cast<const f32x4*>(v_ptr + off);
    }
  };
  auto dma_source = [&]() { return p_wimg + static_cast<long>(p_chunk) * WIMG; };
  auto dma_weights = [&](float* w_dst, const float* wp, int q0 = 0, int q1 = 4) {
#pragma unroll
    for (int q = q0; q < q1; ++q)
      __builtin_amdgcn_global_load_lds((gptr_t)(wp + (tid + q * kThreads) * 4),
                                       (lptr_t)(w_dst + (q * kThreads + wave * 64) * 4), 16, 0, 0);
  };
  auto store_chunk = [&](float* in_dst, int q0 = 0, int q1 = 3) {
    if constexpr (LEAN) {
#pragma unroll
      for (int q = q0; q < q1; ++q) {
        const int it = tid + q * kThreads;
        f32x4 v = reg_in[q];
        if constexpr (FOLD) {
          const unsigned inside = ~static_cast<unsigned>(pix[q] >> 31);
#pragma unroll
          for (int e = 0; e < 4; ++e)
            v[e] = __builtin_bit_cast(float, __builtin_bit_cast(unsigned, floor_keep_nan(fmaf(v[e], co_sc[e], co_sh[e]), co_floor)) & inside);
        }
        *reinterpret_cast<f32x2*>(&in_dst[(it >> 1) * WP + cc]) = f32x2{v[0], v[1]};
        *reinterpret_cast<f32x2*>(&in_dst[(it >> 1) * WP + cc + 2]) = f32x2{v[2], v[3]};
      }
      return;
    }
    const bool affine = v_scale != nullptr;
    f32x4 sc = {1.f, 1.f, 1.f, 1.f}, sh = {0.f, 0.f, 0.f, 0.f};
    if (affine) {
      const int ch = p_c0 + (cc < pf_cnt ? cc : 0);
      sc = *reinterpret_cast<const f32x4*>(v_scale + ch);
      sh = *reinterpret_cast<const f32x4*>(v_shift + ch);
    }
#pragma unroll
    for (int q = 0; q < IN_ITEMS; ++q) {
      const int it = tid + q * kThreads;
      const bool keep = ((in_mask >> q) & 1u) && cc < pf_cnt;
      f32x4 v = reg_in[q];
      if (affine) {
#pragma unroll
        for (int e = 0; e < 4; ++e) v[e] = fmaf(v[e], sc[e], sh[e]);
      }
      if (v_relu) {
#pragma unroll
        for (int e = 0; e < 4; ++e) v[e] = relu_keep_nan(v[e]);
      }
#pragma unroll
      for (int e = 0; e < 4; ++e) v[e] = keep ? v[e] : 0.f;
      if (it < NPIX * 2) {
        *reinterpret_cast<f32x2*>(&in_dst[(it >> 1) * WP + cc]) = f32x2{v[0], v[1]};
        *reinterpret_cast<f32x2*>(&in_dst[(it >> 1) * WP + cc + 2]) = f32x2{v[2], v[3]};
      }
    }
  };

  auto epilogue = [&]() {
    const UnitGeom& ug = c_ug;
    const TileCols tc = decode_tile(a, ug.group);
    const unetpp_view& O = d.out[tc.ov];
    const bool interior = (ug.ty0 + TH <= d.H) && (ug.tx0 + TW <= d.W);
    const unsigned rs = static_cast<unsigned>(O.sy) * O.Ws * O.C, cs = static_cast<unsigned>(O.sx) * O.C;
    const unsigned tile_base = view_pixel_offset32(O, ug.n, ug.ty0, ug.tx0) + tc.nt * WNC;
    float* obase = O.ptr + tile_base;
    const float* gbase = O.gate != nullptr ? O.gate + tile_base : nullptr;
    const bool vec_out = ((O.C | O.c_off | tc.n_cnt) & 3) == 0 && (reinterpret_cast<uintptr_t>(O.ptr) & 15) == 0 &&
                         (O.gate == nullptr || (reinterpret_cast<uintptr_t>(O.gate) & 15) == 0);
    const bool want_stats = d.stats_partial != nullptr;
    const float floor_v = O.relu ? 0.f : -__builtin_inff();
    float s1[NH][4], s2[NH][4];
#pragma unroll
    for (int nh = 0; nh < NH; ++nh)
#pragma unroll
      for (int rr = 0; rr < 4; ++rr) s1[nh][rr] = s2[nh][rr] = 0.f;
    if (d.bias != nullptr && tc.n0 + WNC <= kBiasCols) {
#pragma unroll
      for (int nh = 0; nh < NH; ++nh) acc[5][nh] += *reinterpret_cast<const f32x4*>(&bias_lds[tc.n0 + 16 * nh + 4 * g]);
    } else if (d.bias != nullptr) {
#pragma unroll
      for (int nh = 0; nh < NH; ++nh)
#pragma unroll
        for (int rr = 0; rr < 4; ++rr) {
          const int col = 16 * nh + 4 * g + rr;
          acc[5][nh][rr] += col < tc.n_cnt ? d.bias[tc.n0 + col] : 0.f;
        }
    }
    const unsigned ty2 = 2 * (my_tile / TXN), tx2 = 2 * (my_tile % TXN);
    auto out_row = [&](int ap, int nh, int rr, float (&y)[2]) {
      float tb[4];
#pragma unroll
      for (int b = 0; b < 4; ++b)
        tb[b] = (ap == 0) ? (acc[b][nh][rr] + acc[4 + b][nh][rr]) + acc[8 + b][nh][rr]
                          : (acc[4 + b][nh][rr] - acc[8 + b][nh][rr]) - acc[12 + b][nh][rr];
      y[0] = floor_keep_nan((tb[0] + tb[1]) + tb[2], floor_v);
      y[1] = floor_keep_nan((tb[1] - tb[2]) - tb[3], floor_v);
    };
    if (interior && vec_out && tc.n_cnt == 16 * NH) {
      const bool has_gate = gbase != nullptr, acc_out = O.accumulate != 0;
      const unsigned lane_off = ty2 * rs + tx2 * cs + 4 * g;
#pragma unroll
      for (int ap = 0; ap < 2; ++ap) {
        unsigned off[2][NH];
        f32x4 gt[2][NH], old[2][NH];
#pragma unroll
        for (int bp = 0; bp < 2; ++bp)
#pragma unroll
          for (int nh = 0; nh < NH; ++nh) off[bp][nh] = lane_off + ap * rs + bp * cs + 16 * nh;
        if (has_gate) {
#pragma unroll
          for (int bp = 0; bp < 2; ++bp)
#pragma unroll
            for (int nh = 0; nh < NH; ++nh) gt[bp][nh] = *reinterpret_cast<const f32x4*>(gbase + off[bp][nh]);
        }
        if (acc_out) {
#pragma unroll
          for (int bp = 0; bp < 2; ++bp)
#pragma unroll
            for (int nh = 0; nh < NH; ++nh) old[bp][nh] = *reinterpret_cast<const f32x4*>(obase + off[bp][nh]);
        }
        f32x4 yv[2][NH];
#pragma unroll
        for (int nh = 0; nh < NH; ++nh) {
          f32x2 y[2][2];
#pragma unroll
          for (int cp = 0; cp < 2; ++cp) {
            f32x2 tb[4];
#pragma unroll
            for (int b = 0; b < 4; ++b) {
              const f32x2 m0 = cp ? acc[b][nh].hi : acc[b][nh].lo, m1 = cp ? acc[4 + b][nh].hi : acc[4 + b][nh].lo;
              const f32x2 m2 = cp ? acc[8 + b][nh].hi : acc[8 + b][nh].lo, m3 = cp ? acc[12 + b][nh].hi : acc[12 + b][nh].lo;
              tb[b] = (ap == 0) ? (m0 + m1) + m2 : (m1 - m2) - m3;
            }
            const f32x2 t0 = (tb[0] + tb[1]) + tb[2], t1 = (tb[1] - tb[2]) - tb[3];
            y[0][cp] = f32x2{floor_keep_nan(t0.x, floor_v), floor_keep_nan(t0.y, floor_v)};
            y[1][cp] = f32x2{floor_keep_nan(t1.x, floor_v), floor_keep_nan(t1.y, floor_v)};
          }
          yv[0][nh] = f32x4{y[0][0].x, y[0][0].y, y[0][1].x, y[0][1].y};
          yv[1][nh] = f32x4{y[1][0].x, y[1][0].y, y[1][1].x, y[1][1].y};
          if (want_stats) {
#pragma unroll
            for (int rr = 0; rr < 4; ++rr) {
              const float y0 = yv[0][nh][rr], y1 = yv[1][nh][rr];
              s1[nh][rr] += y0 + y1;
              s2[nh][rr] = fmaf(y0, y0, fmaf(y1, y1, s2[nh][rr]));
            }
          }
        }
        if (!has_gate && !acc_out) {
#pragma unroll
          for (int bp = 0; bp < 2; ++bp)
#pragma unroll
            for (int nh = 0; nh < NH; ++nh) {
              if constexpr (wino_exp::kNoOutStore) asm volatile("" ::"v"(yv[bp][nh]), "v"(off[bp][nh]));
              else *reinterpret_cast<f32x4*>(obase + off[bp][nh]) = yv[bp][nh];
            }
          continue;
        }
#pragma unroll
        for (int bp = 0; bp < 2; ++bp)
#pragma unroll
          for (int nh = 0; nh < NH; ++nh) {
            f32x4 v = yv[bp][nh];
            if (has_gate && !O.gate_sum) {
#pragma unroll
              for (int e = 0; e < 4; ++e) v[e] = (gt[bp][nh][e] > 0.f) ? v[e] : 0.f;
            }
            if (acc_out) {
#pragma unroll
              for (int e = 0; e < 4; ++e) v[e] += old[bp][nh][e];
            }
            if (has_gate && O.gate_sum) {
#pragma unroll
              for (int e = 0; e < 4; ++e) v[e] = (gt[bp][nh][e] > 0.f) ? v[e] : 0.f;
            }
            *reinterpret_cast<f32x4*>(obase + off[bp][nh]) = v;
          }
      }
    } else {
#pragma unroll
      for (int ap = 0; ap < 2; ++ap) {
        const unsigned py = ty2 + ap;
#pragma unroll
        for (int nh = 0; nh < NH; ++nh)
#pragma unroll
          for (int rr = 0; rr < 4; ++rr) {
            float y[2];
            out_row(ap, nh, rr, y);
            const int col = 16 * nh + 4 * g + rr;
#pragma unroll
            for (int bp = 0; bp < 2; ++bp) {
              float v = y[bp];
              if ((col < tc.n_cnt) && (ug.ty0 + py < d.H) && (ug.tx0 + tx2 + bp < d.W)) {
                s1[nh][rr] += v;
                s2[nh][rr] = fmaf(v, v, s2[nh][rr]);
                const unsigned off = py * rs + (tx2 + bp) * cs + col;
                if (gbase != nullptr && !O.gate_sum) v = (gbase[off] > 0.f) ? v : 0.f;
                if (O.accumulate) v += obase[off];
                if (gbase != nullptr && O.gate_sum) v = (gbase[off] > 0.f) ? v : 0.f;
                obase[off] = v;
              }
            }
          }
      }
    }
#pragma unroll
    for (int xi = 0; xi < 16; ++xi)
#pragma unroll
      for (int nh = 0; nh < NH; ++nh) acc[xi][nh] = f32x4{0.f, 0.f, 0.f, 0.f};
    if (want_stats) {
#pragma unroll
      for (int nh = 0; nh < NH; ++nh)
#pragma unroll
        for (int rr = 0; rr < 4; ++rr) {
          s1[nh][rr] = row16_sum(s1[nh][rr]);
          s2[nh][rr] = row16_sum(s2[nh][rr]);
          if (t16 == 0) {
            stat_lds[(wave * WNC + 16 * nh + 4 * g + rr) * 2 + 0] = s1[nh][rr];
            stat_lds[(wave * WNC + 16 * nh + 4 * g + rr) * 2 + 1] = s2[nh][rr];
          }
        }
    }
  };
  auto flush_stats = [&]() {
    if (d.stats_partial == nullptr || tid >= 16 * NH) return;
    const UnitGeom& ug = c_ug;
    const TileCols tc = decode_tile(a, ug.group);
    if (tid >= tc.n_cnt) return;
    float t1 = 0.f, t2 = 0.f;
#pragma unroll
    for (int w = 0; w < 4; ++w) {
      t1 += stat_lds[(w * WNC + tid) * 2 + 0];
      t2 += stat_lds[(w * WNC + tid) * 2 + 1];
    }
    if constexpr (bn_fused) {
      stat_lds[RUN0 + (tc.n0 + tid) * 2 + 0] += t1;
      stat_lds[RUN0 + (tc.n0 + tid) * 2 + 1] += t2;
      return;
    }
    float* dst = d.stats_partial + (ug.patch * a.Ncols + tc.n0 + tid) * 2;
    dst[0] = t1;
    dst[1] = t2;
  };

  cache_view();
  prefetch_unit();
  view_offsets(d.in[0]);
  load_coeffs();
  load_inputs();
  dma_weights(w_tile, dma_source());
  store_chunk(in_tile);
  advance();
  load_coeffs();
  load_inputs();
  asm volatile("s_waitcnt vmcnt(%0)" ::"n"(IN_ITEMS) : "memory");
  __syncthreads();

  int c_chunk = 0, c_unit = 0;
  int cur = 0;
  while (true) {
    const unsigned in_b = lds_offset(in_tile) + a_base * 4, w_b = lds_offset(w_tile) + b_base * 4;
    float dd[16], ddn[16], V[16];
    f32x2_t dp[8], dpn[8];
    unsigned row_b[4];
#pragma unroll
    for (int i = 0; i < 4; ++i) row_b[i] = in_b + i * HWp * WP * 4;
    f32x4 us[2][2];
    if constexpr (LEAN) {
      static_for<8>([&](auto ic) {
        constexpr int e = decltype(ic)::v, j = 2 * (e & 1);
        lds_read2_b32<j * WP, (j + 1) * WP>(dp[e], row_b[e >> 1]);
      });
    } else {
      static_for<16>([&](auto ic) {
        constexpr int e = decltype(ic)::v;
        lds_read_b32<((e / 4) * HWp + (e % 4)) * WP * 4>(dd[e], in_b);
      });
    }
    lds_read2st64_b64<0, 1>(us[0][0], w_b);
    lds_read2st64_b64<2, 3>(us[0][1], w_b);

    float* other = smem + (cur ^ 1) * BUF;
    if constexpr (!LEAN) {
      __builtin_amdgcn_s_setprio(3);
      store_chunk(other);
      dma_weights(other + IN_FLOATS, dma_source());
      advance();
      load_inputs();
    }
    auto staging_piece = [&](auto gc) {
      constexpr int g = decltype(gc)::v;
      if constexpr (!LEAN) return;
      if constexpr (wino_exp::kNoStaging) {
        if constexpr (g == 2) advance();
        return;
      }
      if constexpr (g == 0 && !wino_exp::kNoStore) store_chunk(other);
      if constexpr (g == 0 && !wino_exp::kNoDma) dma_weights(other + IN_FLOATS, dma_source());
      if constexpr (g == 1) {
        advance();
        load_coeffs();
      }
      if constexpr (g == 2 && !wino_exp::kNoLoads) load_inputs();
    };

    __builtin_amdgcn_s_setprio(2);
    if constexpr (LEAN) {
      lds_wait8x2(dp);
      lds_wait(us[0][0], us[0][1]);
      wino_input_transform_pk(dp, V);
    } else {
      lds_wait16(dd);
      lds_wait(us[0][0], us[0][1]);
      wino_input_transform(dd, V);
    }
    static_for<8>([&](auto gc) {
      constexpr int g = decltype(gc)::v, cs = g & 1, ns = cs ^ 1;
      if constexpr (g + 1 < 8) {
        lds_read2st64_b64<4 * (g + 1), 4 * (g + 1) + 1>(us[ns][0], w_b);
        lds_read2st64_b64<4 * (g + 1) + 2, 4 * (g + 1) + 3>(us[ns][1], w_b);
      }
      if constexpr (g == 0) {
        if constexpr (LEAN) {
          static_for<8>([&](auto ic) {
            constexpr int e = decltype(ic)::v, j = 2 * (e & 1);
            lds_read2_b32<j * WP + 1, (j + 1) * WP + 1>(dpn[e], row_b[e >> 1]);
          });
        } else {
          static_for<16>([&](auto ic) {
            constexpr int e = decltype(ic)::v;
            lds_read_b32<(((e / 4) * HWp + (e % 4)) * WP + 1) * 4>(ddn[e], in_b);
          });
        }
      }
      WINO_FENCE();
#pragma unroll
      for (int q = 0; q < 4; ++q) {
        const int xi = (4 * g + q) & 15;
        const f32x4 up = us[cs][q >> 1];
        acc[xi][0] = __builtin_amdgcn_mfma_f32_16x16x4f32(up[(q & 1) * 2], V[xi], acc[xi][0], 0, 0, 0);
        if (NH == 2)
          acc[xi][NH - 1] = __builtin_amdgcn_mfma_f32_16x16x4f32(up[(q & 1) * 2 + 1], V[xi], acc[xi][NH - 1], 0, 0, 0);
      }
      staging_piece(gc);
      WINO_FENCE();
      if constexpr (g == 0) {
        if constexpr (LEAN) lds_wait8x2(dpn);
        else lds_wait16(ddn);
      }
      if constexpr (g + 1 < 8) lds_wait(us[ns][0], us[ns][1]);
      if constexpr (g == 3) {
        if constexpr (LEAN) wino_input_transform_pk(dpn, V);
        else wino_input_transform(ddn, V);
      }
    });
    __builtin_amdgcn_s_setprio(0);
    if constexpr (!wino_exp::kNoBarrier) {
      if (wino_exp::kLaxWait && c_chunk == 0 && c_unit > 0)
        asm volatile("s_waitcnt vmcnt(%0) lgkmcnt(0)" ::"n"(IN_ITEMS + 4 + 4 * NH) : "memory");
      else
      asm volatile("s_waitcnt vmcnt(%0) lgkmcnt(0)" ::"n"(IN_ITEMS) : "memory");
      __builtin_amdgcn_s_barrier();
      asm volatile("" ::: "memory");
    }
    if (c_chunk + 1 == a.n_chunks) {
#pragma unroll
      for (int q = 0; q < IN_ITEMS; ++q) asm volatile("" : "+v"(reg_in[q]));
      if constexpr (wino_exp::kNoEpilogue) {
#pragma unroll
        for (int xi = 0; xi < 16; ++xi)
#pragma unroll
          for (int nh = 0; nh < NH; ++nh) {
            asm volatile("" : "+v"(acc[xi][nh]));
            acc[xi][nh] = f32x4{0.f, 0.f, 0.f, 0.f};
          }
      } else {
        epilogue();
      }
      if (d.stats_partial != nullptr) {
        __syncthreads();
        flush_stats();
      }
      step_unit(c_ug);
      c_chunk = 0;
      if (++c_unit == n_units) break;
    } else {
      ++c_chunk;
    }
    cur ^= 1;
    in_tile = smem + cur * BUF;
    w_tile = in_tile + IN_FLOATS;
  }
  if constexpr (BNF) {
    __syncthreads();
    bn_rows_store<kThreads>(d.stats_partial, a.Ncols, stat_lds + RUN0);
  }
}

}

bool wino_applies(const unetpp_gemm_desc* d) {
  return d != nullptr && d->taps == 9 && (d->flags & (UNETPP_GEMM_DIRECT | UNETPP_GEMM_BF16)) == 0;
}

void gemm_wino_plan(const unetpp_gemm_desc* d, GemmSel& s) {
  s.kernel = GEMM_WINO;
  s.label = "gemm_wino_kernel";
  long workers = (2L * s.cus) & ~7L;
#ifdef UNETPP_WINO_EXP
  if (opt_value(OPT_WINO_ONE_PER_CU, 0) == 1) workers = s.cus & ~7L;
#endif
  if (workers < 8) workers = 8;
  if (workers > kBnFusedRows) workers = kBnFusedRows;
  s.grid_x = static_cast<unsigned>(s.fa.total_blocks <= workers ? s.fa.total_blocks : workers);
  bool narrow = true;
  for (int i = 0; i < d->n_out; ++i) narrow = narrow && d->out[i].c_len <= 16;
  bool lean = opt_value(OPT_WINO_NO_LEAN, 0) == 0, fold = false;
  for (int i = 0; i < d->n_in; ++i) {
    const unetpp_view& v = d->in[i];
    lean = lean && (v.c_len & 7) == 0 && v.Hs == d->H && v.Ws == d->W && v.sy == 1 && v.sx == 1 && v.oy == 0 &&
           v.ox == 0 && static_cast<long>(d->N) * v.Hs * v.Ws * v.C * 4 <= 0x7fffffffL;
    fold = fold || v.scale != nullptr || v.relu != 0;
  }
  s.narrow = narrow ? 1 : 0;
  s.mode = !lean ? 0 : (fold ? 2 : 1);
  s.fa.bn_in_kernel = (s.mode != 0 && bn_rows_per_workgroup(d, s.fa.Ncols)) ? 1 : 0;
  s.bn_rows = s.fa.bn_in_kernel ? s.grid_x : 0;
}

int launch_gemm_wino(const unetpp_gemm_desc*, const GemmSel& s, hipStream_t st) {
  const FastArgs& a = s.fa;
  const int mode = s.mode;
  const bool narrow = s.narrow != 0;
  const dim3 grid(s.grid_x), block(kThreads);
#define UNETPP_LAUNCH_WINO_M(L, NHV)                                                                    \
  do {                                                                                                  \
    if (mode == 0) hipLaunchKernelGGL((gemm_wino_kernel<L, NHV, 0>), grid, block, 0, st, a);            \
    else if (a.bn_in_kernel && mode == 1) hipLaunchKernelGGL((gemm_wino_kernel<L, NHV, 1, true>), grid, block, 0, st, a); \
    else if (a.bn_in_kernel) hipLaunchKernelGGL((gemm_wino_kernel<L, NHV, 2, true>), grid, block, 0, st, a);             \
    else if (mode == 1) hipLaunchKernelGGL((gemm_wino_kernel<L, NHV, 1>), grid, block, 0, st, a);       \
    else hipLaunchKernelGGL((gemm_wino_kernel<L, NHV, 2>), grid, block, 0, st, a);                      \
  } while (0)
#define UNETPP_LAUNCH_WINO(L)                 \
  do {                                        \
    if (narrow) UNETPP_LAUNCH_WINO_M(L, 1);   \
    else UNETPP_LAUNCH_WINO_M(L, 2);          \
  } while (0)
  if (a.log2tw == 5) UNETPP_LAUNCH_WINO(5);
  else if (a.log2tw == 4) UNETPP_LAUNCH_WINO(4);
  else UNETPP_LAUNCH_WINO(3);
#undef UNETPP_LAUNCH_WINO
#undef UNETPP_LAUNCH_WINO_M
  return launch_status();
}

}
```

### unet_nested4tiny_objects_keypoints_amd/engine.py

```python
from __future__ import annotations

import os

from typing import Dict, List, Optional, Tuple

import torch

from . import ops
from .ops import V


USE_PACK_PLAN = os.environ.get("UNETPP_NO_PACK_PLAN") is None
USE_GROUPED_DGRAD = os.environ.get("UNETPP_NO_GROUPED_DGRAD") is None
USE_PLAN_COPIES = os.environ.get("UNETPP_NO_PLAN_COPIES") is None
_A1_MATERIALIZE_BYTES = int(float(os.environ.get("UNETPP_BF16_A1_MAX_MB", "80")) * (1 << 20))
_A1_MATERIALIZE_BYTES_F32 = int(float(os.environ.get("UNETPP_F32_A1_MAX_MB", "80")) * (1 << 20))


def _empty(n, like):
    return torch.empty(n, dtype=torch.float32, device=like.device)


def _packed(w, t, k, n, dstr, sstr, flip=False):
    dst = _empty(t * k * n, w)
# ... 162 lines not shown
    if is_deconv:
        co = upmod.out_channels
        u.up = torch.empty((b, 2 * hs, 2 * ws, co), dtype=adt, device=src.device)
        ops.gemm_fwd(b, hs, ws, 1, [V(src)], _phase_views(u.up), pack_deconv_fwd(upmod.weight.detach()),
                     tile_bias4(upmod.bias.detach()))
    else:
        conv = getattr(upmod, "1")
        ci, co = conv.in_channels, conv.out_channels
        u.interp = torch.empty((b, 2 * hs, 2 * ws, ci), dtype=adt, device=src.device)
        ops.bilinear2x_fwd(src, u.interp)
        u.up = torch.empty((b, 2 * hs, 2 * ws, co), dtype=adt, device=src.device)
        ops.gemm_fwd(b, 2 * hs, 2 * ws, 1, [V(u.interp)], [V(u.up)], pack_conv_fwd(conv.weight.detach()),
                     conv.bias.detach())
    return u


def _check_input(model, x):
    if x.dim() != 4:
        raise ValueError("expected NCHW input, got %d dims" % x.dim())
    if not x.is_cuda:
        raise RuntimeError("UNet_Nested (HIP) needs its input on the GPU: there is no CPU fallback for this path")
    if x.dtype != torch.float32:
        raise TypeError("expected float32 input, got %s" % x.dtype)
    if x.shape[1] != model.in_channels:
        raise ValueError("expected %d input channels, got %d" % (model.in_channels, x.shape[1]))
    m = 1 << (model.depth - 1)
    if x.shape[2] % m or x.shape[3] % m:
        raise ValueError("H and W must be divisible by %d, got %dx%d" % (m, x.shape[2], x.shape[3]))
    if next(model.parameters()).device != x.device:
        raise RuntimeError("model and input are on different devices")


def _activation_dtype(model):
    adt = getattr(model, "activation_dtype", torch.float32)
    if adt == torch.bfloat16:
        if any(f % 8 or (f // 8) & (f // 8 - 1) for f in model.filters):
            raise NotImplementedError("bf16 storage needs channel counts 8 * 2^k, got %s" % (model.filters,))
    return adt


def _dropout_config(model, training):
    p = float(model.drop_out.p) if (training and model.drop_out.training) else 0.0
    heads = model.depth - 1
    masks = model.dropout_masks if p > 0.0 else None
    if masks is not None and len(masks) != heads:
        raise ValueError("dropout_masks needs one mask per head")
    seed_dev = getattr(model, "_dropout_seed_dev", None) if (p > 0.0 and masks is None) else None
    base = int(torch.randint(0, 2 ** 62, (1,)).item()) if (p > 0.0 and masks is None and seed_dev is None) else 0
    seeds = [(base + 0x632BE59BD9B4E019 * (j + 1)) & 0xFFFFFFFFFFFFFFFF for j in range(heads)]
    return p, seeds, masks, seed_dev


def needed_nodes(depth: int, head: int) -> List[Tuple[int, int]]:
    head = check_head(depth, head)
    return [(i, 0) for i in range(head + 1)] + [(i, j) for j in range(1, head + 1) for i in range(head + 1 - j)]


def check_head(depth: int, head) -> int:
    if head is None:
        return depth - 1
    if isinstance(head, bool) or not isinstance(head, int) or not 1 <= head <= depth - 1:
        raise ValueError("head must be an int in 1..%d (or None for the last head), got %r" % (depth - 1, head))
    return head


def plan_phase(depth: int, head=None, backward: bool = False) -> str:
    head = check_head(depth, head)
    base = "bwd" if backward else "fwd"
    return base if head == depth - 1 else "%s/%d" % (base, head)


def pruned_parameters(model, head=None) -> List[torch.nn.Parameter]:
    from .checkpoint import _pruned_prefixes
    prefixes = _pruned_prefixes(model.depth, check_head(model.depth, head))
    return [p for name, p in model.named_parameters() if name.startswith(prefixes)]


STATS_PHASE = "stats"


def stats_nodes(depth: int) -> List[Tuple[int, int]]:
    if isinstance(depth, bool) or not isinstance(depth, int) or depth < 1:
        raise ValueError("depth must be a positive int, got %r" % (depth,))
    return [(i, 0) for i in range(depth)]


def stats_pass(model, x) -> None:
    _check_input(model, x)
    if not model.is_batchnorm:
        return
    _PENDING_COUNTERS.clear()
    try:
        with torch.no_grad():
            plan = None
            if USE_PACK_PLAN:
                plan = _plan_of(model)
                plan.begin(STATS_PHASE)
                ops.set_pack_plan(plan)
            try:
                b, _, h, w = x.shape
                d = model.depth
                adt = _activation_dtype(model)
                inp = ops.nchw_to_nhwc(x.detach().contiguous())
                for (i, _) in stats_nodes(d):
                    with ops.region("X%d0.stats" % i):
                        r = _pair_fwd(getattr(model, "conv%d0" % i), [V(inp)], b, h, w, True, pool=(i < d - 1), adt=adt,
                                      stats=False)
                    if i < d - 1:
                        inp, h, w = r.pooled, h // 2, w // 2
            finally:
                if plan is not None:
                    ops.set_pack_plan(None)
    finally:
        flush_batch_counters()


def forward_impl(model, x, training: bool, save: bool, head: Optional[int] = None, ensemble: bool = False,
                 all_heads: bool = False):
    _check_input(model, x)
    _PENDING_COUNTERS.clear()
    try:
        if not USE_PACK_PLAN:
            return _forward_impl(model, x, training, save, head, ensemble, all_heads)
        plan = _plan_of(model)
        plan.begin(plan_phase(model.depth, head))
        ops.set_pack_plan(plan)
        try:
            return _forward_impl(model, x, training, save, head, ensemble, all_heads)
        finally:
            ops.set_pack_plan(None)
    finally:
        flush_batch_counters()


def infer(model, x, head=None, ensemble: bool = False):
    top = check_head(model.depth, head)
    if model.training:
        raise RuntimeError("UNet_Nested.infer is the eval forward: call model.eval() first")
    pruned_to = getattr(model, "pruned_to", None)
    if pruned_to is not None and top > pruned_to:
        raise RuntimeError("this model holds a checkpoint pruned to head %d: the nodes head %d needs were never loaded"
                           % (pruned_to, top))
    if model.is_batchnorm:
        for i in range(top + 1):
            for stage in ("conv1", "conv2"):
                if getattr(getattr(getattr(model, "conv%d0" % i), stage), "1").training:
                    raise RuntimeError("UNet_Nested.infer is the eval forward, but BatchNorm layer conv%d0.%s.1 is in training "
                                       "mode: call model.eval() (or .eval() on that layer) first" % (i, stage))
    with torch.no_grad():
        outs, _ = forward_impl(model, x, False, save=False, head=top, ensemble=bool(ensemble))
    return outs[0]


def _plan_of(model) -> "ops.PackPlan":
    plan = model.__dict__.get("_pack_plan")
    if plan is None:
        plan = ops.PackPlan()
        model.__dict__["_pack_plan"] = plan
    return plan


def _forward_impl(model, x, training: bool, save: bool, head: Optional[int] = None, ensemble: bool = False,
                  all_heads: bool = False):
    b, _, h0, w0 = x.shape
    d = model.depth
    top = d - 1 if head is None else head
    adt = _activation_dtype(model)
    x_nhwc = ops.nchw_to_nhwc(x.detach().contiguous())
    X: Dict[Tuple[int, int], torch.Tensor] = {}
    pairs: Dict[Tuple[int, int], _PairRec] = {}
    ups: Dict[Tuple[int, int], _UpRec] = {}
    inp, h, w = x_nhwc, h0, w0
    for (i, j) in needed_nodes(d, top):
        if j == 0:
            with ops.region("X%d0.fwd" % i):
                r = _pair_fwd(getattr(model, "conv%d0" % i), [V(inp)], b, h, w, training, pool=(i < top), adt=adt,
                              stats=save)
            pairs[(i, 0)], X[(i, 0)] = r, r.out
            if i < top:
                inp, h, w = r.pooled, h // 2, w // 2
        else:
            mod = getattr(model, "up_concat%d%d" % (i, j))
            hi, wi = h0 >> i, w0 >> i
            u = _up_fwd(mod.up, model.is_deconv, X[(i + 1, j - 1)], b, hi // 2, wi // 2, adt)
            ins = [V(u.up)] + [V(X[(i, jj)]) for jj in range(j)]
            r = _pair_fwd(mod.conv, ins, b, hi, wi, training, pool=False, adt=adt, stats=save)
            ups[(i, j)], pairs[(i, j)], X[(i, j)] = u, r, r.out
    p_drop, seeds, masks, seed_dev = _dropout_config(model, training)
    outs = []
    if head is not None and ensemble:
        finals = [getattr(model, "final_%d" % j) for j in range(1, head + 1)]
        o = torch.empty((b, model.n_classes, h0, w0), dtype=torch.float32, device=x.device)
        ops.heads_mean_fwd([X[(0, j)] for j in range(1, head + 1)],
                           [f.weight.detach().view(model.n_classes, -1) for f in finals],
                           [f.bias.detach() for f in finals], o)
        outs.append(o)
    cols = list(range(1, d) if head is None else () if ensemble else range(1, head + 1) if all_heads else (head,))
    ctx = _HEAD_TRAIN[0]
    head_train = None
    if (ctx is not None and save and training and cols and adt == torch.float32
            and ctx.target.device == x.device and tuple(ctx.target.shape) == (b, model.n_classes, h0, w0)):
        head_train = {}
    for j in cols:
        final = getattr(model, "final_%d" % j)
        o = torch.empty((b, model.n_classes, h0, w0), dtype=torch.float32, device=x.device)
        wt, mask = final.weight.detach().view(model.n_classes, -1), None if masks is None else masks[j - 1]
        got = None
        if head_train is not None:
            dx = torch.empty_like(X[(0, j)])
            rows = ctx.target.numel() if ctx.size_average else b * model.n_classes
            got = ops.head_train(X[(0, j)], wt, final.bias.detach(), ctx.target, rows, ctx.gamma, len(cols), p_drop,
                                 seeds[j - 1], mask, o, dx, gate_x=(j == top), seed_dev=seed_dev)
            if got is None:
                head_train = None
            else:
                head_train[j] = (dx,) + got
        if got is None:
            ops.head_fwd(X[(0, j)], wt, final.bias.detach(), p_drop, seeds[j - 1], mask, o, seed_dev=seed_dev)
        outs.append(o)
    if not save:
        return outs, None
    s = _Saved()
    s.x_nhwc, s.X, s.pairs, s.ups, s.outs = x_nhwc, X, pairs, ups, outs
    s.p_drop, s.seeds, s.masks, s.seed_dev = p_drop, seeds, masks, seed_dev
    s.shape = (b, h0, w0)
    s.top, s.ensemble = top, bool(head is not None and ensemble)
    s.head_train = head_train
    if head_train is not None:
        ctx.used = True
    return outs, s


class _GradBook:

    def __init__(self, X, top, gate_keys, grouped=False):
        self.X = X
        self.buf: Dict[Tuple[int, int], torch.Tensor] = {}
        self.got: Dict[Tuple[int, int], int] = {}
        self.gate_keys = gate_keys
        self.gated = set()
        self.expected = {}
        for (i, j) in X:
            n = (1 if (i == 0 and j >= 1) else 0)
            consumers = max(0, (top - i) - j)
            n += min(consumers, 1) if grouped else consumers
            n += 1 if i >= 1 else 0
            n += 1 if (j == 0 and i < top) else 0
            self.expected[(i, j)] = n

    def target(self, key, can_gate=False):
        self.got[key] = self.got.get(key, 0) + 1
        gate = None
        if can_gate and key in self.gate_keys and self.got[key] == self.expected[key]:
            gate = self.X[key]
            self.gated.add(key)
        if key in self.buf:
            return self.buf[key], True, gate
        t = torch.empty_like(self.X[key])
        self.buf[key] = t
        return t, False, gate

    def preset(self, key, tensor, gated):
        assert key not in self.buf and self.got.get(key, 0) == 0, "a preset gradient is the node's first contribution"
        assert gated == (key in self.gate_keys and self.expected[key] == 1), "ReLU mask of node %s" % (key,)
        self.got[key] = 1
        self.buf[key] = tensor
        if gated:
            self.gated.add(key)

    def take(self, key):
        assert self.got.get(key, 0) == self.expected[key], "gradient fan-in mismatch at node %s" % (key,)
        return self.buf.pop(key), key in self.gated


_ALLOC = [None]


def _new_grad(p):
    return torch.empty_like(p) if _ALLOC[0] is None else _ALLOC[0](p)


def _conv_wgrad(conv, xs, dys, b, h, w, grads):
    co, ci, kh, kw = conv.weight.shape
    t = kh * kw
    dw = _new_grad(conv.weight)
    db = _new_grad(conv.bias)
    ops.wgrad(b, h, w, t, xs, dys, dw, (1, t, ci * t, 0), db)
    grads[conv.weight] = dw
    grads[conv.bias] = db


def _bn_bwd(bn, coeffs, frozen, d_act, y, pool_grad):
    mean, invstd, scale, shift = coeffs
    if not frozen:
        return ops.bn_backward(d_act, y, scale, shift, mean, invstd, bn.weight.detach(), d_act,
                               _new_grad(bn.weight), _new_grad(bn.bias), pool=pool_grad)
    if not (bn.weight.requires_grad or bn.bias.requires_grad):
        return ops.bn_frozen_backward(d_act, y, scale, shift, None, None, d_act, pool=pool_grad, want_sums=False)
    return ops.bn_frozen_backward(d_act, y, scale, shift, mean, invstd, d_act, _new_grad(bn.weight), _new_grad(bn.bias),
                                  pool=pool_grad)


def _pair_bwd(blk, r: _PairRec, d_out, in_targets: Optional[List[V]], b, grads, pre_gated=False, pool_grad=None,
              flush=None, in_slice: Optional[Tuple[int, int]] = None):
    conv1, conv2 = getattr(blk.conv1, "0"), getattr(blk.conv2, "0")
    h, w = r.h, r.w
    if blk.is_batchnorm:
        bn1, bn2 = getattr(blk.conv1, "1"), getattr(blk.conv2, "1")
        grads[bn2.weight], grads[bn2.bias] = _bn_bwd(bn2, r.bn2, r.frozen2, d_out, r.y2, pool_grad)
        dy2 = V(d_out)
        mean, invstd, scale, shift = r.bn1
        if r.a1 is not None:
            _conv_wgrad(conv2, [V(r.a1)], [dy2], b, h, w, grads)
        else:
            _conv_wgrad(conv2, [V(r.y1, scale=scale, shift=shift, relu=True)], [dy2], b, h, w, grads)
        if flush is not None:
            flush()
        d_a1 = torch.empty_like(r.y1)
        ops.gemm_fwd(b, h, w, 9, [dy2], [V(d_a1)], pack_conv_dgrad(conv2.weight.detach()))
        grads[bn1.weight], grads[bn1.bias] = _bn_bwd(bn1, r.bn1, r.frozen1, d_a1, r.y1, None)
        dy1 = V(d_a1)
    else:
        dy2 = V(d_out) if pre_gated else V(d_out, gate=r.out)
        _conv_wgrad(conv2, [V(r.a1)], [dy2], b, h, w, grads)
        if flush is not None:
            flush()
        d_a1 = torch.empty_like(r.a1)
        ops.gemm_fwd(b, h, w, 9, [dy2], [V(d_a1, gate=r.a1)], pack_conv_dgrad(conv2.weight.detach()))
        dy1 = V(d_a1)
    _conv_wgrad(conv1, r.ins, [dy1], b, h, w, grads)
    if flush is not None:
        flush()
    if in_targets is not None:
        if dy1.t.dtype == torch.bfloat16 and in_targets[0].t.dtype == torch.float32:
            ops.first_layer_dgrad_bf16(dy1.t, conv1.weight.detach(), in_targets[0].t)
        elif in_slice is not None:
            ops.gemm_fwd(b, h, w, 9, [dy1], in_targets, pack_conv_dgrad_slice(conv1.weight.detach(), in_slice[0], in_slice[1]))
        else:
            ops.gemm_fwd(b, h, w, 9, [dy1], in_targets, pack_conv_dgrad(conv1.weight.detach()))
    return dy1


def _up_bwd(upmod, is_deconv, u: _UpRec, d_up, d_src, accumulate, gate, b, grads):
    hs, ws = u.h, u.w
    if is_deconv:
        ci, co = upmod.weight.shape[0], upmod.weight.shape[1]
        dw = _new_grad(upmod.weight)
        db = _new_grad(upmod.bias)
        ops.wgrad(b, hs, ws, 1, [V(u.src)], _phase_views(d_up), dw, (0, 4 * co, 4, 1), db, n_inner=co)
        grads[upmod.weight], grads[upmod.bias] = dw, db
        ops.gemm_fwd(b, hs, ws, 1, _phase_views(d_up), [V(d_src, accumulate=accumulate, gate=gate, gate_sum=True)],
                     pack_deconv_dgrad(upmod.weight.detach()))
    else:
        conv = getattr(upmod, "1")
        _conv_wgrad(conv, [V(u.interp)], [V(d_up)], b, 2 * hs, 2 * ws, grads)
        d_interp = torch.empty_like(u.interp)
        ops.gemm_fwd(b, 2 * hs, 2 * ws, 1, [V(d_up)], [V(d_interp)], pack_conv_dgrad(conv.weight.detach()))
        ops.bilinear2x_bwd(d_interp, d_src, accumulate, gate)


def _grouped_weights(model, refresh=False, plan=None, top=None):
    d = model.depth
    top = d - 1 if top is None else top
    whole = top == d - 1
    phase = plan_phase(d, top, backward=True)
    cache = getattr(model, "_grouped_dgrad_w", None) if whole else (getattr(model, "_grouped_dgrad_w_cut", None) or {}).get(top)
    if cache is None or refresh:
        fresh = {}
        for i in range(top):
            for jj in range(top - i):
                ws = [getattr(getattr(model, "up_concat%d%d" % (i, jc)).conv.conv1, "0").weight.detach()
                      for jc in range(jj + 1, top + 1 - i)]
                f = ws[0].shape[0]
                parts = [w[:, (1 + jj) * f:(2 + jj) * f] for w in ws]
                old = None if cache is None else cache.get((i, jj))
                if old is not None and not (old.device == parts[0].device and old.dtype == parts[0].dtype):
                    old = None
                if plan is not None and all(w.is_contiguous() and w.dtype == torch.float32 for w in ws):
                    key, sig = ("grouped", i, jj) + ops.phase_tag(phase), tuple(w.data_ptr() for w in ws)
                    if old is not None and plan.knows_copy(key, phase, sig + (old.data_ptr(),)):
                        plan.copy_for(key, phase, sig + (old.data_ptr(),), None)
                        fresh[(i, jj)] = old
                        continue
                    buf = old if old is not None else torch.empty((len(ws) * f, f) + tuple(ws[0].shape[2:]),
                                                                   dtype=ws[0].dtype, device=ws[0].device)
                    t = ws[0].shape[2] * ws[0].shape[3]
                    items = [(w, (1 + jj) * f * t, q * f * f * t, f, f * t, w.shape[1] * t, f * t) for q, w in enumerate(ws)]
                    plan.copy_for(key, phase, sig + (buf.data_ptr(),), lambda: (buf, list(ws), items))
                    old = buf
                if old is not None:
                    torch.cat(parts, 0, out=old)
                    fresh[(i, jj)] = old
                else:
                    fresh[(i, jj)] = torch.cat(parts, 0).contiguous()
        cache = fresh
        if whole:
            model._grouped_dgrad_w = cache
        else:
            if getattr(model, "_grouped_dgrad_w_cut", None) is None:
                model._grouped_dgrad_w_cut = {}
            model._grouped_dgrad_w_cut[top] = cache
    return cache


def backward_impl(model, s: _Saved, d_outs, want_input_grad: bool, grad_sink=None):
    if USE_GROUPED_DGRAD:
        _grouped_weights(model, refresh=True, plan=_plan_of(model) if (USE_PACK_PLAN and USE_PLAN_COPIES) else None,
                         top=s.top)
    if not USE_PACK_PLAN:
        return _backward_impl(model, s, d_outs, want_input_grad, grad_sink)
    plan = _plan_of(model)
    plan.begin(plan_phase(model.depth, s.top, backward=True))
    ops.set_pack_plan(plan)
    try:
        return _backward_impl(model, s, d_outs, want_input_grad, grad_sink)
    finally:
        ops.set_pack_plan(None)


def _backward_impl(model, s: _Saved, d_outs, want_input_grad: bool, grad_sink=None):
    b, h0, w0 = s.shape
    top = s.top
    grads: Dict[torch.nn.Parameter, torch.Tensor] = {}
    gate_keys = {k for k in s.X if k[1] >= 1 or not model.is_batchnorm}
    grouped = USE_GROUPED_DGRAD
    book = _GradBook(s.X, top, gate_keys, grouped)
    bf16 = s.X[(0, 0)].dtype == torch.bfloat16
    dy1s: Dict[Tuple[int, int], V] = {}
    seen = set()
    head_train = getattr(s, "head_train", None)

    def flush():
        if grad_sink is not None and len(grads) > len(seen):
            fresh = [(p, g) for p, g in grads.items() if id(p) not in seen]
            seen.update(id(p) for p, _ in fresh)
            if fresh:
                grad_sink(fresh)

    if s.ensemble:
        finals = [getattr(model, "final_%d" % j) for j in range(1, top + 1)]
        go = d_outs[0]
        if go is None:
            go = torch.zeros_like(s.outs[0])
        tg = {j: book.target((0, j), can_gate=True) for j in range(top, 0, -1)}
        cols = range(1, top + 1)
        got = ops.heads_mean_bwd([s.X[(0, j)] for j in cols], [f.weight.detach().view(model.n_classes, -1) for f in finals],
                                 [f.bias.detach() for f in finals], go.contiguous(), [tg[j][0] for j in cols],
                                 [tg[j][1] for j in cols], [tg[j][2] is not None for j in cols])
        for j in range(top, 0, -1):
            head, (dw, db) = finals[j - 1], got[j - 1]
            if _ALLOC[0] is not None:
                gw, gb = _new_grad(head.weight), _new_grad(head.bias)
                gw.copy_(dw)
                gb.copy_(db)
                dw, db = gw, gb
            grads[head.weight], grads[head.bias] = dw, db
    for j in (() if s.ensemble else range(top, 0, -1)):
        head = getattr(model, "final_%d" % j)
        if head_train is not None:
            dx, dw, db = head_train.pop(j)
            book.preset((0, j), dx, gated=(j == top))
        else:
            go = d_outs[j - 1]
            if go is None:
                go = torch.zeros_like(s.outs[j - 1])
            go = go.contiguous()
            dx, acc, gate = book.target((0, j), can_gate=True)
            dw, db = ops.head_bwd(go, s.outs[j - 1], s.X[(0, j)], head.weight.detach().view(model.n_classes, -1), s.p_drop,
                                  s.seeds[j - 1], None if s.masks is None else s.masks[j - 1], dx, acc,
                                  gate_x=gate is not None, seed_dev=s.seed_dev)
        if _ALLOC[0] is not None:
            gw, gb = _new_grad(head.weight), _new_grad(head.bias)
            gw.copy_(dw)
            gb.copy_(db)
            dw, db = gw, gb
        grads[head.weight], grads[head.bias] = dw, db
    flush()
    for j in range(top, 0, -1):
        for i in range(top - j, -1, -1):
            mod = getattr(model, "up_concat%d%d" % (i, j))
            r, u = s.pairs[(i, j)], s.ups[(i, j)]
            d_out, pre_gated = book.take((i, j))
            d_up = torch.empty_like(u.up)
            targets = [V(d_up)]
            if grouped:
                c_up = u.up.shape[3]
                dy1s[(i, j)] = _pair_bwd(mod.conv, r, d_out, targets, b, grads, pre_gated, flush=flush, in_slice=(0, c_up))
                consumers = list(range(j, top + 1 - i))
                t, acc, gate = book.target((i, j - 1), can_gate=True)
                ops.gemm_fwd(b, r.h, r.w, 9, [dy1s[(i, jc)] for jc in consumers],
                             [V(t, accumulate=acc, gate=gate, gate_sum=True)],
                             pack_conv_dgrad(_grouped_weights(model, top=top)[(i, j - 1)]))
                if j == 1:
                    for jc in consumers:
                        del dy1s[(i, jc)]
            else:
                for jj in range(j):
                    t, acc, gate = book.target((i, jj), can_gate=True)
                    targets.append(V(t, accumulate=acc, gate=gate, gate_sum=True))
                _pair_bwd(mod.conv, r, d_out, targets, b, grads, pre_gated, flush=flush)
            t, acc, gate = book.target((i + 1, j - 1), can_gate=model.is_deconv or bf16)
            _up_bwd(mod.up, model.is_deconv, u, d_up, t, acc, gate, b, grads)
            flush()
    dx_in = None
    pool_grad = None
    for i in range(top, -1, -1):
        blk = getattr(model, "conv%d0" % i)
        r = s.pairs[(i, 0)]
        d_out, pre_gated = book.take((i, 0))
        if pool_grad is not None and not model.is_batchnorm:
            ops.maxpool_bwd(pool_grad[0], pool_grad[1], d_out, gate=r.out if (bf16 and not pre_gated) else None)
            pre_gated = pre_gated or bf16
            pool_grad = None
        mine, pool_grad = pool_grad, None
        if i > 0:
            d_pooled = torch.empty_like(s.pairs[(i - 1, 0)].pooled)
            _pair_bwd(blk, r, d_out, [V(d_pooled)], b, grads, pre_gated, pool_grad=mine, flush=flush)
            t, acc, _ = book.target((i - 1, 0))
            if not acc:
                t.zero_()
            pool_grad = (d_pooled, s.pairs[(i - 1, 0)].pool_idx)
        elif want_input_grad:
            if bf16 and s.x_nhwc.shape[3] > 4:
                raise NotImplementedError("bf16 storage: the input gradient needs at most 4 input channels")
            dx_in = torch.empty_like(s.x_nhwc)
            _pair_bwd(blk, r, d_out, [V(dx_in)], b, grads, pre_gated, pool_grad=mine, flush=flush)
        else:
            _pair_bwd(blk, r, d_out, None, b, grads, pre_gated, pool_grad=mine, flush=flush)
        flush()
    return grads, dx_in


class _UNetNestedFn(torch.autograd.Function):
    @staticmethod
    def forward(ctx, model, x, cut, *params):
        if cut is None:
            outs, saved = forward_impl(model, x, model.training, save=True)
        else:
            outs, saved = forward_impl(model, x, model.training, save=True, head=cut[0], ensemble=cut[1], all_heads=True)
        if getattr(model, "_debug_keep_saved", False):
            model._debug_saved = saved
        ctx.model, ctx.saved = model, saved
        ctx.params = params
        return tuple(outs)

    @staticmethod
    @torch.autograd.function.once_differentiable
    def backward(ctx, *d_outs):
        model, saved = ctx.model, ctx.saved
        if saved is None:
            raise RuntimeError("UNet_Nested (HIP): backward called twice on the same forward")
        ctx.saved = None
        sink = getattr(model, "_grad_sink", None)
        _ALLOC[0] = getattr(model, "_grad_alloc", None)
        try:
            grads, dx = backward_impl(model, saved, d_outs, ctx.needs_input_grad[1], sink)
        finally:
            _ALLOC[0] = None
        dx_nchw = None
        if dx is not None:
            dx_nchw = ops.nhwc_to_nchw(dx)
        done = getattr(model, "_grad_done", None)
        if done is not None and done():
            return (None, dx_nchw, None) + (None,) * len(ctx.params)
        return (None, dx_nchw, None) + tuple(grads.get(p) if need else None
                                            for p, need in zip(ctx.params, ctx.needs_input_grad[3:]))


def run(model, x):
    if getattr(model, "_grad_sink", None) is not None and getattr(model, "_grad_head", model.depth - 1) != model.depth - 1:
        raise RuntimeError("the attached data-parallel averager holds the gradients of the network cut at head %d only: "
                           "use forward_pruned / train_step(..., head=%d)" % (model._grad_head, model._grad_head))
    params = tuple(model.parameters())
    track = torch.is_grad_enabled() and (x.requires_grad or any(p.requires_grad for p in params))
    if track:
        return _UNetNestedFn.apply(model, x, None, *params)
    outs, _ = forward_impl(model, x, model.training, save=False)
    return tuple(outs)


def run_pruned(model, x, head=None, ensemble: bool = False):
    top = check_head(model.depth, head)
    pruned_to = getattr(model, "pruned_to", None)
    if pruned_to is not None and top > pruned_to:
        raise RuntimeError("this model holds a checkpoint pruned to head %d: the nodes head %d needs were never loaded"
                           % (pruned_to, top))
    ensemble = bool(ensemble)
    if ensemble and model.training and model.drop_out.training and float(model.drop_out.p) > 0.0:
        raise RuntimeError("the ensemble mean has no dropout: call model.drop_out.eval() before "
                           "forward_pruned(..., ensemble=True)")
    if getattr(model, "_grad_sink", None) is not None and getattr(model, "_grad_head", model.depth - 1) != top:
        raise RuntimeError("the attached data-parallel averager holds the gradients of another cut: build it with "
                           "make_data_parallel(model, head=%d)" % top)
    params = tuple(pruned_parameters(model, top))
    if torch.is_grad_enabled() and (x.requires_grad or any(p.requires_grad for p in params)):
        outs = _UNetNestedFn.apply(model, x, (top, ensemble), *params)
    else:
        outs, _ = forward_impl(model, x, model.training, save=False, head=top, ensemble=ensemble, all_heads=True)
    return outs[0] if ensemble else tuple(outs)
```

### unet_nested4tiny_objects_keypoints_amd/ops.py

```python
from __future__ import annotations

import ctypes as C
import functools
import os
from dataclasses import dataclass
from typing import Optional, Sequence

import torch

from . import _lib
from ._lib import MAX_VIEWS, GemmDesc, PackJob, View, WeightSrc, WgradDesc, check


def _stream():
    return C.c_void_p(torch.cuda.current_stream().cuda_stream)


class LaunchTimer:

    def __init__(self):
        self.launches = []
        self.regions = []
        self.want_launches = True
        self.want_regions = True
# ... 46 lines not shown

def _timed_call(kind, flops, fn, nbytes=0.0):
    if _TIMER is None or not _TIMER.want_launches:
        return fn()
    s, e = _TIMER._pair()
    s.record()
    r = fn()
    e.record()
    if kind is None:
        kind = _lib.lib().unetpp_last_kernel_name().decode()
    _TIMER.launches.append((kind, flops, nbytes, s, e))
    return r


def _ptr(t: Optional[torch.Tensor]):
    return None if t is None else C.c_void_p(t.data_ptr())


def _need(t: torch.Tensor, what: str, dtype=torch.float32):
    if not t.is_cuda:
        raise RuntimeError("%s must live on the GPU: this path has no CPU fallback" % what)
    if t.dtype != dtype:
        raise TypeError("%s must be %s, got %s" % (what, dtype, t.dtype))
    if not t.is_contiguous():
        raise ValueError("%s must be contiguous" % what)
    return t


_ACT_DTYPES = (torch.float32, torch.bfloat16)


def _storage_flag(outs, ins):
    bf = outs[0].t.dtype == torch.bfloat16
    for v in outs:
        if (v.t.dtype == torch.bfloat16) != bf:
            raise TypeError("mixed fp32 / bf16 output views in one launch")
    for v in ins:
        if (v.t.dtype == torch.bfloat16) != bf and not (bf and len(ins) == 1 and v.t.shape[3] <= 4):
            raise TypeError("mixed fp32 / bf16 views in one launch")
    return _lib.GEMM_BF16 if bf else 0


@dataclass
class V:
    t: torch.Tensor
    c_off: int = 0
    c_len: Optional[int] = None
    sy: int = 1
    sx: int = 1
    oy: int = 0
    ox: int = 0
    scale: Optional[torch.Tensor] = None
    shift: Optional[torch.Tensor] = None
    gate: Optional[torch.Tensor] = None
    relu: bool = False
    accumulate: bool = False
    gate_sum: bool = False

    def fill(self, dst: View) -> int:
        t = _need(self.t, "view tensor", self.t.dtype if self.t.dtype in _ACT_DTYPES else torch.float32)
        if t.dim() != 4:
            raise ValueError("view tensor must be NHWC [N,H,W,C]")
        c = t.shape[3]
        n = c - self.c_off if self.c_len is None else self.c_len
        dst.ptr = t.data_ptr()
        dst.C, dst.c_off, dst.c_len = c, self.c_off, n
        dst.Hs, dst.Ws = t.shape[1], t.shape[2]
        dst.sy, dst.sx, dst.oy, dst.ox = self.sy, self.sx, self.oy, self.ox
        dst.scale = None if self.scale is None else _need(self.scale, "scale").data_ptr()
        dst.shift = None if self.shift is None else _need(self.shift, "shift").data_ptr()
        if self.gate is not None:
            g = _need(self.gate, "gate", t.dtype)
            if g.shape != t.shape:
                raise ValueError("gate must have the geometry of the gated tensor")
            dst.gate = g.data_ptr()
        else:
            dst.gate = None
        dst.relu = int(self.relu)
        dst.accumulate = int(self.accumulate)
        dst.gate_sum = int(self.gate_sum)
        return n


USE_FAST_GEMM = True
USE_WINOGRAD = os.environ.get("UNETPP_NO_WINOGRAD") is None


@dataclass
class WSrc:
    t: torch.Tensor
    taps: int
    k: int
    n: int
    s_t: int
    s_k: int
    s_n: int
    s_ko: int = 0
    s_no: int = 0
    k_inner: int = 0
    n_inner: int = 0
    flip: bool = False
    pack: Optional[callable] = None

    def numel(self) -> int:
        return self.taps * self.k * self.n

    @property
    def device(self):
        return self.t.device

    def fill(self, dst: WeightSrc) -> None:
        dst.src = _need(self.t, "weight").data_ptr()
        dst.s_t, dst.s_k, dst.s_ko, dst.s_n, dst.s_no = self.s_t, self.s_k, self.s_ko, self.s_n, self.s_no
        dst.k_inner, dst.n_inner, dst.flip = self.k_inner, self.n_inner, int(self.flip)

    def packed(self) -> torch.Tensor:
        if self.pack is None:
            raise ValueError("this weight source has no packed form")
        return self.pack()


class PackPlan:

    class _Entry:
        __slots__ = ("image", "n_img", "job", "src", "phase", "fresh", "used")

    class _Copy:
        __slots__ = ("dst", "jobs", "srcs", "srcsig", "phase", "fresh", "used", "elems")

    def __init__(self):
        self.entries = {}
        self.copies = {}
        self._copy_tables = {}
        self.copy_launches = 0
        self._tables = {}
        self._packed = set()
        self.frozen = False
        self.phase = None
        self.pass_id = 0
        self.launches = 0
        self.pinned = 0
        self._retired = []

    def pin(self) -> None:
        self.pinned += 1

    def unpin(self) -> None:
        self.pinned = max(0, self.pinned - 1)
        if not self.pinned:
            self._retired.clear()

    def invalidate(self) -> None:
        self._packed.clear()

    def __deepcopy__(self, memo):
        return PackPlan()

    def __reduce__(self):
        return (PackPlan, ())

    def begin(self, phase: str) -> None:
        self.phase = phase
        self.pass_id += 1
        if not self.pinned:
            stale = [k for k, e in self.entries.items() if self.pass_id - e.used > 16]
            for k in stale:
                self._tables.pop(self.entries[k].phase, None)
                del self.entries[k]
            for k in [k for k, c in self.copies.items() if self.pass_id - c.used > 16]:
                self._copy_tables.pop(self.copies[k].phase, None)
                del self.copies[k]
        self._begin_copies(phase)
        sigs = tuple(k for k, e in self.entries.items() if e.phase == phase)
        if not sigs:
            return
        ents = [self.entries[k] for k in sigs]
        tab = self._tables.get(phase)
        if tab is None or tab[2] != sigs:
            arr = (PackJob * len(ents))(*[e.job for e in ents])
            dev = torch.frombuffer(bytearray(bytes(arr)), dtype=torch.uint8).to(ents[0].image.device)
            if self.pinned and phase in self._tables:
                self._retired.append(self._tables[phase])
            tab = (dev, arr, sigs, max(e.n_img for e in ents))
            self._tables[phase] = tab
            self._packed.discard(phase)
        if not (self.frozen and phase in self._packed):
            check(_lib.lib().unetpp_gemm_pack_weight_images(_ptr(tab[0]), len(ents), tab[3], _stream()),
                  "unetpp_gemm_pack_weight_images")
            self.launches += 1
            self._packed.add(phase)
        for e in ents:
            e.fresh = self.pass_id

    def _begin_copies(self, phase: str) -> None:
        keys = tuple(k for k, c in self.copies.items() if c.phase == phase)
        if not keys:
            return
        cps = [self.copies[k] for k in keys]
        tab = self._copy_tables.get(phase)
        if tab is None or tab[1] != keys:
            jobs = [j for c in cps for j in c.jobs]
            arr = (_lib.CopyJob * len(jobs))(*jobs)
            dev = torch.frombuffer(bytearray(bytes(arr)), dtype=torch.uint8).to(cps[0].dst.device)
            if self.pinned and phase in self._copy_tables:
                self._retired.append(self._copy_tables[phase])
            tab = (dev, keys, max(c.elems for c in cps), len(jobs))
            self._copy_tables[phase] = tab
            self._packed.discard(phase)
        if not (self.frozen and phase in self._packed):
            check(_lib.lib().unetpp_copy_jobs(_ptr(tab[0]), tab[3], tab[2], _stream()), "unetpp_copy_jobs")
            self.copy_launches += 1
        for c in cps:
            c.fresh = self.pass_id

    def copy_for(self, key, phase: str, srcsig, make):
        c = self.copies.get(key)
        if c is None or c.srcsig != srcsig or c.phase != phase:
            dst, srcs, items = make()
            c = PackPlan._Copy()
            c.dst, c.srcs, c.srcsig, c.phase, c.fresh = dst, srcs, srcsig, phase, -1
            c.jobs, c.elems = [], 1
            for (src, s_off, d_off, n_outer, n_inner, s_stride, d_stride) in items:
                j = _lib.CopyJob()
                j.src, j.dst = src.data_ptr() + 4 * s_off, dst.data_ptr() + 4 * d_off
                j.n_outer, j.n_inner, j.src_stride, j.dst_stride = n_outer, n_inner, s_stride, d_stride
                if n_outer * n_inner >= 2 ** 31:
                    raise ValueError("copy job too large")
                c.jobs.append(j)
                c.elems = max(c.elems, n_outer * n_inner)
            self.copies[key] = c
            old_tab = self._copy_tables.pop(phase, None)
            if old_tab is not None and self.pinned:
                self._retired.append(old_tab)
        c.used = self.pass_id
        return c.dst, c.fresh == self.pass_id

    def knows_copy(self, key, phase: str, srcsig) -> bool:
        c = self.copies.get(key)
        return c is not None and c.srcsig == srcsig and c.phase == phase

    def image_for(self, sig, n_img: int, weight: "WSrc", d: GemmDesc):
        e = self.entries.get(sig)
        if e is None:
            e = PackPlan._Entry()
            e.image = torch.empty(n_img, dtype=torch.float32, device=weight.device)
            e.n_img, e.src, e.phase, e.fresh = n_img, weight.t, self.phase, -1
            job = PackJob()
            weight.fill(job.src)
            job.image = e.image.data_ptr()
            job.taps, job.flags, job.n_in, job.n_out = d.taps, d.flags, d.n_in, d.n_out
            for i in range(d.n_in):
                job.in_len[i] = d.inp[i].c_len
            for i in range(d.n_out):
                job.out_len[i] = d.out[i].c_len
            e.job = job
            self.entries[sig] = e
        e.used = self.pass_id
        return e.image, e.fresh == self.pass_id


_PLAN: Optional[PackPlan] = None
_NO_IMAGE_YET = 16


def set_pack_plan(plan: Optional[PackPlan]) -> None:
    global _PLAN
    _PLAN = plan


def current_plan() -> Optional[PackPlan]:
    return _PLAN if (_PLAN is not None and _PLAN.phase is not None) else None


def phase_tag(phase) -> tuple:
    return () if phase in ("fwd", "bwd") else (phase,)


def gemm_pixel_blocks(n: int, h: int, w: int) -> int:
    return int(_lib.lib().unetpp_gemm_pixel_blocks(n, h, w))


@dataclass
class BatchNormFinish:
    gamma: torch.Tensor
    beta: torch.Tensor
    running_mean: Optional[torch.Tensor]
    running_var: Optional[torch.Tensor]
    eps: float
    momentum: float
    count: int

    def outputs(self, c: int):
        dev = self.gamma.device
        self.mean, self.invstd, self.scale, self.shift = (torch.empty(c, dtype=torch.float32, device=dev) for _ in range(4))
        return self.mean, self.invstd, self.scale, self.shift


def gemm_stats_rows(n: int, h: int, w: int) -> int:
    return int(_lib.lib().unetpp_gemm_stats_rows(n, h, w))


def gemm_fwd(n: int, h: int, w: int, taps: int, ins: Sequence[V], outs: Sequence[V], weight: torch.Tensor,
             bias: Optional[torch.Tensor] = None, stats_partial: Optional[torch.Tensor] = None,
             direct: bool = False, bn: Optional[BatchNormFinish] = None) -> _lib.GemmSizes:
    if len(ins) > MAX_VIEWS or len(outs) > MAX_VIEWS:
        raise ValueError("too many views")
    d = GemmDesc()
    d.N, d.H, d.W, d.taps = n, h, w, taps
    d.flags = (_lib.GEMM_DIRECT if (direct or not USE_WINOGRAD) else 0) | _storage_flag(outs, ins)
    d.n_in, d.n_out = len(ins), len(outs)
    k = sum(v.fill(d.inp[i]) for i, v in enumerate(ins))
    nc = sum(v.fill(d.out[i]) for i, v in enumerate(outs))
    from_src = isinstance(weight, WSrc)
    if not from_src:
        _need(weight, "packed weight")
    if weight.numel() != taps * k * nc or (from_src and (weight.taps, weight.k, weight.n) != (taps, k, nc)):
        raise ValueError("weight has %d elements, expected %d*%d*%d" % (weight.numel(), taps, k, nc))
    if bias is not None and _need(bias, "bias").numel() != nc:
        raise ValueError("bias length mismatch")
    rows = gemm_pixel_blocks(n, h, w) if bn is None else gemm_stats_rows(n, h, w)
    if stats_partial is not None and _need(stats_partial, "stats").numel() != rows * nc * 2:
        raise ValueError("stats_partial size mismatch")
    if bn is not None:
        if stats_partial is None or len(outs) != 1:
            raise ValueError("a fused BatchNorm finalize needs stats_partial and a single output view")
        mean, invstd, scale, shift = bn.outputs(nc)
        for t, what in ((bn.gamma, "gamma"), (bn.beta, "beta")):
            if _need(t, what).numel() != nc:
                raise ValueError("BatchNorm %s length mismatch" % what)
        d.bn.gamma, d.bn.beta = bn.gamma.data_ptr(), bn.beta.data_ptr()
        d.bn.running_mean = None if bn.running_mean is None else _need(bn.running_mean, "running_mean").data_ptr()
        d.bn.running_var = None if bn.running_var is None else _need(bn.running_var, "running_var").data_ptr()
        d.bn.mean, d.bn.invstd, d.bn.scale, d.bn.shift = mean.data_ptr(), invstd.data_ptr(), scale.data_ptr(), shift.data_ptr()
        d.bn.count, d.bn.eps, d.bn.momentum = int(bn.count), float(bn.eps), float(bn.momentum)

    d.weight = None if from_src else weight.data_ptr()
    d.bias = None if bias is None else bias.data_ptr()
    d.stats_partial = None if stats_partial is None else stats_partial.data_ptr()
    lib = _lib.lib()
    plan = _lib.GemmSizes()
    d.weight_image = _NO_IMAGE_YET if USE_FAST_GEMM else None
    if USE_FAST_GEMM and lib.unetpp_gemm_plan(C.byref(d), 0, C.byref(plan)) != 0:
        d.weight_image = None
    if d.weight_image is not None:
        n_img = int(plan.image_floats)
        ready = False
        if from_src and _PLAN is not None and _PLAN.phase is not None:
            sig = (weight.t.data_ptr(), weight.s_t, weight.s_k, weight.s_ko, weight.s_n, weight.s_no, weight.k_inner,
                   weight.n_inner, weight.flip, taps, d.flags, tuple(v.c_len for v in d.inp[:d.n_in]),
                   tuple(v.c_len for v in d.out[:d.n_out])) + phase_tag(_PLAN.phase)
            image, ready = _PLAN.image_for(sig, n_img, weight, d)
        else:
            image = torch.empty(n_img, dtype=torch.float32, device=weight.device)
        if ready:
            pass
        elif from_src:
            ws = WeightSrc()
            weight.fill(ws)
            check(lib.unetpp_gemm_pack_weight_image_from(C.byref(d), C.byref(ws), _ptr(image), _stream()),
                  "unetpp_gemm_pack_weight_image_from")
        else:
            check(lib.unetpp_gemm_pack_weight_image(C.byref(d), _ptr(image), _stream()),
                  "unetpp_gemm_pack_weight_image")
        d.weight_image = image.data_ptr()
    if d.weight_image is None:
        if from_src:
            packed = weight.packed()
            d.weight = packed.data_ptr()
        check(lib.unetpp_gemm_plan(C.byref(d), 0, C.byref(plan)), "unetpp_gemm_plan")
    acc = sum(v.c_len for v in d.out[:d.n_out] if v.accumulate) + sum(v.c_len for v in d.out[:d.n_out] if v.gate)
    _timed_call(None, 2.0 * n * h * w * taps * k * nc,
                lambda: check(lib.unetpp_gemm_fwd(C.byref(d), _stream()), "unetpp_gemm_fwd"),
                (2.0 if d.flags & _lib.GEMM_BF16 else 4.0) * n * h * w * (k + nc + acc))
    return plan


def first_layer_dgrad_bf16(dy: torch.Tensor, weight: torch.Tensor, dx: torch.Tensor) -> None:
    n, h, w, co = dy.shape
    ci = dx.shape[3]
    _need(dy, "dy", torch.bfloat16)
    _need(weight, "weight")
    _need(dx, "dx")
    if tuple(weight.shape) != (co, ci, 3, 3) or tuple(dx.shape[:3]) != (n, h, w):
        raise ValueError("shape mismatch")
    check(_lib.lib().unetpp_first_layer_dgrad_bf16(_ptr(dy), _ptr(weight), n, h, w, ci, co, _ptr(dx), _stream()),
          "unetpp_first_layer_dgrad_bf16")


def pack_weight(dst: torch.Tensor, src: torch.Tensor, t: int, k: int, n: int, dstr, sstr, flip: bool = False) -> None:
    _need(dst, "pack dst")
    _need(src, "pack src")
    check(_lib.lib().unetpp_pack_weight(_ptr(dst), _ptr(src), t, k, n, dstr[0], dstr[1], dstr[2],
                                        sstr[0], sstr[1], sstr[2], int(flip), _stream()), "unetpp_pack_weight")


def wgrad(n: int, h: int, w: int, taps: int, xs: Sequence[V], dys: Sequence[V], dw: Optional[torch.Tensor],
          dw_strides, db: Optional[torch.Tensor], n_inner: Optional[int] = None, target_blocks: int = 256,
          direct: bool = False) -> _lib.WgradSizes:
    lib = _lib.lib()
    d = WgradDesc()
    d.N, d.H, d.W, d.taps = n, h, w, taps
    d.n_x, d.n_dy = len(xs), len(dys)
    k = sum(v.fill(d.x[i]) for i, v in enumerate(xs))
    nc = sum(v.fill(d.dy[i]) for i, v in enumerate(dys))
    d.flags = (_lib.GEMM_DIRECT if (direct or not USE_WINOGRAD) else 0) | _storage_flag(dys, xs)
    plan = _lib.WgradSizes()
    check(lib.unetpp_wgrad_plan(C.byref(d), target_blocks, C.byref(plan)), "unetpp_wgrad_plan")
    slabs = torch.empty(plan.slab_floats, dtype=torch.float32, device=xs[0].t.device)
    d.n_split, d.slabs = plan.n_split, slabs.data_ptr()
    _timed_call(None, 2.0 * n * h * w * taps * k * nc,
                lambda: check(lib.unetpp_wgrad(C.byref(d), _stream()), "unetpp_wgrad"),
                (2.0 if d.flags & _lib.GEMM_BF16 else 4.0) * n * h * w * (k + nc))
    if n_inner is None:
        n_inner = nc
    check(lib.unetpp_wgrad_finish(_ptr(slabs), plan.n_split, plan.planes, k, nc, n_inner, _ptr(dw), dw_strides[0],
                                  dw_strides[1], dw_strides[2], dw_strides[3], _ptr(db), _stream()), "unetpp_wgrad_finish")
    return plan


def bn_finalize(partial, n_blocks, c, count, gamma, beta, eps, momentum, running_mean, running_var):
    dev = partial.device
    mean, invstd, scale, shift = (torch.empty(c, dtype=torch.float32, device=dev) for _ in range(4))
    check(_lib.lib().unetpp_bn_finalize(_ptr(partial), n_blocks, c, count, _ptr(gamma), _ptr(beta), eps, momentum,
                                        _ptr(running_mean), _ptr(running_var), _ptr(mean), _ptr(invstd), _ptr(scale),
                                        _ptr(shift), _stream()), "unetpp_bn_finalize")
    return mean, invstd, scale, shift


def bn_eval_coeffs(gamma, beta, running_mean, running_var, eps):
    c = gamma.numel()
    scale, shift = (torch.empty(c, dtype=torch.float32, device=gamma.device) for _ in range(2))
    check(_lib.lib().unetpp_bn_eval_coeffs(_ptr(gamma), _ptr(beta), _ptr(running_mean), _ptr(running_var), eps, c,
                                           _ptr(scale), _ptr(shift), _stream()), "unetpp_bn_eval_coeffs")
    return scale, shift


def bn_eval_coeffs_stats(gamma, beta, running_mean, running_var, eps):
    c = gamma.numel()
    mean, invstd, scale, shift = (torch.empty(c, dtype=torch.float32, device=gamma.device) for _ in range(4))
    check(_lib.lib().unetpp_bn_eval_coeffs_stats(_ptr(gamma), _ptr(beta), _ptr(running_mean), _ptr(running_var), eps, c,
                                                 _ptr(scale), _ptr(shift), _ptr(mean), _ptr(invstd), _stream()),
          "unetpp_bn_eval_coeffs_stats")
    return mean, invstd, scale, shift


def _is_bf16(t):
    return t.dtype == torch.bfloat16


def affine_relu_pool(y, scale, shift, relu, act, pooled, pool_idx):
    n, h, w, c = y.shape
    if _is_bf16(y):
        check(_lib.lib().unetpp_affine_relu_pool_bf16(_ptr(y), _ptr(scale), _ptr(shift), int(relu), n, h, w, c, _ptr(act),
                                                      _ptr(pooled), _ptr(pool_idx), _stream()),
              "unetpp_affine_relu_pool_bf16")
        return
    check(_lib.lib().unetpp_affine_relu_pool(_ptr(y), _ptr(scale), _ptr(shift), int(relu), n, h, w, c, _ptr(act),
                                             _ptr(pooled), _ptr(pool_idx), _stream()), "unetpp_affine_relu_pool")


def maxpool_bwd(d_pooled, pool_idx, d_act, gate=None):
    n, h, w, c = d_act.shape
    if _is_bf16(d_act):
        check(_lib.lib().unetpp_maxpool_bwd_bf16(_ptr(d_pooled), _ptr(pool_idx), n, h, w, c, _ptr(d_act), _ptr(gate), _stream()),
              "unetpp_maxpool_bwd_bf16")
        return
    if gate is not None:
        raise ValueError("the fused ReLU mask is a bf16-storage option")
    check(_lib.lib().unetpp_maxpool_bwd(_ptr(d_pooled), _ptr(pool_idx), n, h, w, c, _ptr(d_act), _stream()),
          "unetpp_maxpool_bwd")


def _bn_backward_bf16(d_act, y, scale, shift, mean, invstd, gamma, dy_out, dgamma, dbeta, pool):
    lib = _lib.lib()
    n, h, w, c = y.shape
    blocks = int(lib.unetpp_bn_bwd_blocks_bf16(n * h * w, c))
    if blocks < 1:
        raise ValueError("bf16 BatchNorm backward needs C = 8 * 2^k channels, got %d" % c)
    partial = torch.empty(blocks * c * 2, dtype=torch.float32, device=y.device)
    dp, pi = (None, None) if pool is None else (_need(pool[0], "d_pooled", torch.bfloat16), _need(pool[1], "pool_idx", torch.uint8))
    st = _stream()
    check(lib.unetpp_bn_bwd_reduce_bf16(_ptr(d_act), _ptr(y), _ptr(scale), _ptr(shift), _ptr(mean), _ptr(invstd), _ptr(dp),
                                        _ptr(pi), n, h, w, c, _ptr(partial), st), "unetpp_bn_bwd_reduce_bf16")
    check(lib.unetpp_bn_bwd_finalize(_ptr(partial), blocks, c, _ptr(dgamma), _ptr(dbeta), st), "unetpp_bn_bwd_finalize")
    check(lib.unetpp_bn_bwd_apply_bf16(_ptr(d_act), _ptr(y), _ptr(scale), _ptr(shift), _ptr(mean), _ptr(invstd), _ptr(gamma),
                                       _ptr(dgamma), _ptr(dbeta), _ptr(dp), _ptr(pi), n, h, w, c, _ptr(dy_out), st),
          "unetpp_bn_bwd_apply_bf16")
    return dgamma, dbeta


def bn_backward(d_act, y, scale, shift, mean, invstd, gamma, dy_out, dgamma=None, dbeta=None, pool=None):
    lib = _lib.lib()
    n, h, w, c = y.shape
    pixels = n * h * w
    if dgamma is None:
        dgamma = torch.empty(c, dtype=torch.float32, device=y.device)
    if dbeta is None:
        dbeta = torch.empty(c, dtype=torch.float32, device=y.device)
    if _is_bf16(y):
        return _bn_backward_bf16(d_act, y, scale, shift, mean, invstd, gamma, dy_out, dgamma, dbeta, pool)
    if pool is not None and not lib.unetpp_bn_bwd_pool_ok(n, h, w, c):
        maxpool_bwd(pool[0], pool[1], d_act)
        pool = None
    blocks = int(lib.unetpp_bn_bwd_blocks(pixels, c))
    partial = torch.empty(blocks * c * 2, dtype=torch.float32, device=y.device)
    st = _stream()
    if pool is None:
        check(lib.unetpp_bn_bwd_reduce(_ptr(d_act), _ptr(y), _ptr(scale), _ptr(shift), _ptr(mean), _ptr(invstd), pixels,
                                       c, _ptr(partial), st), "unetpp_bn_bwd_reduce")
    else:
        d_pooled, pool_idx = _need(pool[0], "d_pooled"), _need(pool[1], "pool_idx", torch.uint8)
        check(lib.unetpp_bn_bwd_reduce_pool(_ptr(d_act), _ptr(y), _ptr(scale), _ptr(shift), _ptr(mean), _ptr(invstd),
                                            _ptr(d_pooled), _ptr(pool_idx), n, h, w, c, _ptr(partial), st),
              "unetpp_bn_bwd_reduce_pool")
    check(lib.unetpp_bn_bwd_finalize(_ptr(partial), blocks, c, _ptr(dgamma), _ptr(dbeta), st), "unetpp_bn_bwd_finalize")
    if pool is None:
        check(lib.unetpp_bn_bwd_apply(_ptr(d_act), _ptr(y), _ptr(scale), _ptr(shift), _ptr(mean), _ptr(invstd),
                                      _ptr(gamma), _ptr(dgamma), _ptr(dbeta), pixels, c, _ptr(dy_out), st),
              "unetpp_bn_bwd_apply")
    else:
        check(lib.unetpp_bn_bwd_apply_pool(_ptr(d_act), _ptr(y), _ptr(scale), _ptr(shift), _ptr(mean), _ptr(invstd),
                                           _ptr(gamma), _ptr(dgamma), _ptr(dbeta), _ptr(pool[0]), _ptr(pool[1]), n, h,
                                           w, c, _ptr(dy_out), st), "unetpp_bn_bwd_apply_pool")
    return dgamma, dbeta


def bn_frozen_backward(d_act, y, scale, shift, mean, invstd, dy_out, dgamma=None, dbeta=None, pool=None, want_sums=True):
    lib = _lib.lib()
    n, h, w, c = y.shape
    pixels = n * h * w
    bf16 = _is_bf16(y)
    adt = torch.bfloat16 if bf16 else torch.float32
    _need(d_act, "d_act", adt), _need(y, "y", adt), _need(dy_out, "dy", adt)
    if tuple(d_act.shape) != tuple(y.shape) or tuple(dy_out.shape) != tuple(y.shape):
        raise ValueError("d_act, y and dy must have one shape")
    if want_sums and (mean is None or invstd is None):
        raise ValueError("the gamma / beta sums need the running mean snapshot and invstd")
    blocks_fn = lib.unetpp_bn_frozen_bwd_blocks_bf16 if bf16 else lib.unetpp_bn_frozen_bwd_blocks
    blocks = int(blocks_fn(pixels, c))
    if blocks < 1:
        raise ValueError("bf16 BatchNorm backward needs C = 8 * 2^k channels, got %d" % c)
    if pool is not None and not bf16 and not (lib.unetpp_bn_bwd_pool_ok(n, h, w, c) and scale.data_ptr() % 16 == 0
                                              and shift.data_ptr() % 16 == 0 and pool[1].data_ptr() % 4 == 0):
        maxpool_bwd(pool[0], pool[1], d_act)
        pool = None
    dp, pi = (None, None) if pool is None else (_need(pool[0], "d_pooled", adt), _need(pool[1], "pool_idx", torch.uint8))
    partial = torch.empty(blocks * c * 2, dtype=torch.float32, device=y.device) if want_sums else None
    st = _stream()
    fn = lib.unetpp_bn_frozen_bwd_bf16 if bf16 else lib.unetpp_bn_frozen_bwd
    _timed_call(None, 0.0, lambda: check(fn(_ptr(d_act), _ptr(y), _ptr(scale), _ptr(shift), _ptr(mean), _ptr(invstd),
                                             _ptr(dp), _ptr(pi), n, h, w, c, _ptr(dy_out), _ptr(partial), st),
                                          "unetpp_bn_frozen_bwd"),
                (2.0 if bf16 else 4.0) * pixels * c * 3)
    if not want_sums:
        return None, None
    if dgamma is None:
        dgamma = torch.empty(c, dtype=torch.float32, device=y.device)
    if dbeta is None:
        dbeta = torch.empty(c, dtype=torch.float32, device=y.device)
    check(lib.unetpp_bn_bwd_finalize(_ptr(partial), blocks, c, _ptr(dgamma), _ptr(dbeta), st), "unetpp_bn_bwd_finalize")
    return dgamma, dbeta


def head_fwd(x, weight, bias, p_drop, seed, mask, out_nchw, seed_dev=None):
    n, h, w, c = x.shape
    n_cls = weight.shape[0]
    fn = _lib.lib().unetpp_head_fwd_bf16 if _is_bf16(x) else _lib.lib().unetpp_head_fwd
    check(fn(_ptr(x), _ptr(weight), _ptr(bias), n, h, w, c, n_cls, float(p_drop), C.c_uint64(seed), _ptr(mask),
             _ptr(seed_dev), _ptr(out_nchw), _stream()), "unetpp_head_fwd")


def heads_mean_fwd(xs, weights, biases, out_nchw):
    n_heads = len(xs)
    if not (1 <= n_heads <= _lib.MAX_HEADS) or len(weights) != n_heads or len(biases) != n_heads:
        raise ValueError("heads_mean_fwd takes 1..%d heads with one weight and one bias each" % _lib.MAX_HEADS)
    adt = xs[0].dtype
    if adt not in _ACT_DTYPES:
        raise TypeError("features must be float32 or bfloat16, got %s" % adt)
    n, h, w, c = xs[0].shape
    n_cls = weights[0].shape[0]
    d = _lib.HeadsMean()
    d.n_heads = n_heads
    for i, (x, wt, b) in enumerate(zip(xs, weights, biases)):
        if tuple(_need(x, "head features", adt).shape) != (n, h, w, c):
            raise ValueError("every head reads a feature tensor of the same shape")
        if tuple(_need(wt, "head weight").shape) != (n_cls, c) or _need(b, "head bias").numel() != n_cls:
            raise ValueError("head weight must be [n_cls, C] and bias [n_cls]")
        d.head[i].x, d.head[i].weight, d.head[i].bias = x.data_ptr(), wt.data_ptr(), b.data_ptr()
    if tuple(_need(out_nchw, "output").shape) != (n, n_cls, h, w):
        raise ValueError("output must be [N, n_cls, H, W]")
    fn = _lib.lib().unetpp_heads_mean_fwd_bf16 if adt == torch.bfloat16 else _lib.lib().unetpp_heads_mean_fwd
    check(fn(C.byref(d), n, h, w, c, n_cls, _ptr(out_nchw), _stream()), "unetpp_heads_mean_fwd")


def heads_mean_bwd(xs, weights, biases, d_out, dxs, accumulates, gates):
    lib = _lib.lib()
    n_heads = len(xs)
    if not (1 <= n_heads <= _lib.MAX_HEADS) or not all(len(v) == n_heads for v in (weights, biases, dxs, accumulates, gates)):
        raise ValueError("heads_mean_bwd takes 1..%d heads with one weight, bias, dx, accumulate and gate each" % _lib.MAX_HEADS)
    adt = xs[0].dtype
    if adt not in _ACT_DTYPES:
        raise TypeError("features must be float32 or bfloat16, got %s" % adt)
    n, h, w, c = xs[0].shape
    n_cls = weights[0].shape[0]
    if tuple(_need(d_out, "gradient of the mean").shape) != (n, n_cls, h, w):
        raise ValueError("d_out must be [N, n_cls, H, W]")
    blocks = int(lib.unetpp_head_bwd_blocks(n * h * w))
    ln = n_cls * c + n_cls
    partial = torch.empty((n_heads, blocks * ln), dtype=torch.float32, device=d_out.device)
    sums = torch.empty((n_heads, ln), dtype=torch.float32, device=d_out.device)
    d, g = _lib.HeadsMean(), _lib.HeadsMeanGrad()
    d.n_heads = g.n_heads = n_heads
    for i, (x, wt, b, dx) in enumerate(zip(xs, weights, biases, dxs)):
        if tuple(_need(x, "head features", adt).shape) != (n, h, w, c) or tuple(_need(dx, "feature gradient", adt).shape) != (n, h, w, c):
            raise ValueError("every head reads a feature tensor and writes a gradient of the same shape")
        if tuple(_need(wt, "head weight").shape) != (n_cls, c) or _need(b, "head bias").numel() != n_cls:
            raise ValueError("head weight must be [n_cls, C] and bias [n_cls]")
        d.head[i].x, d.head[i].weight, d.head[i].bias = x.data_ptr(), wt.data_ptr(), b.data_ptr()
        g.head[i].dx, g.head[i].partial = dx.data_ptr(), partial[i].data_ptr()
        g.head[i].accumulate, g.head[i].gate_x = int(bool(accumulates[i])), int(bool(gates[i]))
    st = _stream()
    fn = lib.unetpp_heads_mean_bwd_bf16 if adt == torch.bfloat16 else lib.unetpp_heads_mean_bwd
    check(fn(C.byref(d), C.byref(g), _ptr(d_out), n, h, w, c, n_cls, st), "unetpp_heads_mean_bwd")
    out = []
    for i in range(n_heads):
        check(lib.unetpp_sum_partials(_ptr(partial[i]), blocks, ln, _ptr(sums[i]), st), "unetpp_sum_partials")
        out.append((sums[i, :n_cls * c].view(n_cls, c, 1, 1), sums[i, n_cls * c:]))
    return out


def head_bwd(d_out, out, x, weight, p_drop, seed, mask, dx, accumulate, gate_x=False, seed_dev=None):
    lib = _lib.lib()
    n, h, w, c = x.shape
    n_cls = weight.shape[0]
    blocks = int(lib.unetpp_head_bwd_blocks(n * h * w))
    ln = n_cls * c + n_cls
    partial = torch.empty(blocks * ln, dtype=torch.float32, device=x.device)
    sums = torch.empty(ln, dtype=torch.float32, device=x.device)
    st = _stream()
    fn = lib.unetpp_head_bwd_bf16 if _is_bf16(x) else lib.unetpp_head_bwd
    check(fn(_ptr(d_out), _ptr(out), _ptr(x), _ptr(weight), n, h, w, c, n_cls, float(p_drop), C.c_uint64(seed), _ptr(mask),
             _ptr(seed_dev), _ptr(dx), int(accumulate), int(gate_x), _ptr(partial), st), "unetpp_head_bwd")
    check(lib.unetpp_sum_partials(_ptr(partial), blocks, ln, _ptr(sums), st), "unetpp_sum_partials")
    return sums[:n_cls * c].view(n_cls, c, 1, 1), sums[n_cls * c:]


def head_train(x, weight, bias, target, rows, gamma, n_heads, p_drop, seed, mask, out_nchw, dx, gate_x=False,
               seed_dev=None, partial=None):
    lib = _lib.lib()
    n, h, w, c = x.shape
    n_cls = weight.shape[0]
    if _is_bf16(x):
        return None
    _need(x, "head features"), _need(dx, "feature gradient"), _need(target, "target"), _need(out_nchw, "output")
    if tuple(dx.shape) != (n, h, w, c) or tuple(target.shape) != (n, n_cls, h, w) or tuple(out_nchw.shape) != (n, n_cls, h, w):
        raise ValueError("dx must be [N, H, W, C], target and output [N, n_cls, H, W]")
    blocks = int(lib.unetpp_head_bwd_blocks(n * h * w))
    ln = n_cls * c + n_cls
    if partial is None:
        partial = torch.empty(blocks * ln, dtype=torch.float32, device=x.device)
    elif _need(partial, "partial rows").numel() != blocks * ln:
        raise ValueError("partial must hold %d rows of %d floats" % (blocks, ln))
    st = _stream()
    status = lib.unetpp_head_train(_ptr(x), _ptr(weight), _ptr(bias), _ptr(target), n, h, w, c, n_cls, float(p_drop),
                                   C.c_uint64(seed), _ptr(mask), _ptr(seed_dev), int(rows), float(gamma), int(n_heads),
                                   _ptr(out_nchw), _ptr(dx), int(bool(gate_x)), _ptr(partial), st)
    if status == -1:
        return None
    check(status, "unetpp_head_train")
    sums = torch.empty(ln, dtype=torch.float32, device=x.device)
    check(lib.unetpp_sum_partials(_ptr(partial), blocks, ln, _ptr(sums), st), "unetpp_sum_partials")
    return sums[:n_cls * c].view(n_cls, c, 1, 1), sums[n_cls * c:]


def bilinear2x_fwd(x, y):
    n, h, w, c = x.shape
    if _is_bf16(x):
        check(_lib.lib().unetpp_bilinear2x_fwd_bf16(_ptr(x), n, h, w, c, _ptr(y), _stream()), "unetpp_bilinear2x_fwd_bf16")
        return
    check(_lib.lib().unetpp_bilinear2x_fwd(_ptr(x), n, h, w, c, _ptr(y), _stream()), "unetpp_bilinear2x_fwd")


def bilinear2x_bwd(dy, dx, accumulate, gate=None):
    n, h, w, c = dx.shape
    if _is_bf16(dx):
        check(_lib.lib().unetpp_bilinear2x_bwd_bf16(_ptr(dy), n, h, w, c, _ptr(dx), int(accumulate), _ptr(gate), _stream()),
              "unetpp_bilinear2x_bwd_bf16")
        return
    if gate is not None:
        raise ValueError("the fused ReLU mask is a bf16-storage option")
    check(_lib.lib().unetpp_bilinear2x_bwd(_ptr(dy), n, h, w, c, _ptr(dx), int(accumulate), _stream()),
          "unetpp_bilinear2x_bwd")


def nchw_to_nhwc(src):
    n, c, h, w = src.shape
    _need(src, "input")
    if c == 1:
        return src.view(n, h, w, 1)
    dst = torch.empty((n, h, w, c), dtype=torch.float32, device=src.device)
    check(_lib.lib().unetpp_nchw_to_nhwc(_ptr(src), n, c, h, w, _ptr(dst), _stream()), "unetpp_nchw_to_nhwc")
    return dst


def nhwc_to_nchw(src):
    n, h, w, c = src.shape
    if c == 1:
        return src.view(n, 1, h, w)
    dst = torch.empty((n, c, h, w), dtype=torch.float32, device=src.device)
    check(_lib.lib().unetpp_nhwc_to_nchw(_ptr(src), n, c, h, w, _ptr(dst), _stream()), "unetpp_nhwc_to_nchw")
    return dst


def _aligned16(t: torch.Tensor) -> torch.Tensor:
    return t if t.data_ptr() % 16 == 0 else t.clone(memory_format=torch.contiguous_format)


def focal_bce(pred: torch.Tensor, target: torch.Tensor, rows: int, gamma: float, want_grad: bool = True):
    lib = _lib.lib()
    _need(pred, "pred")
    _need(target, "target")
    if pred.shape != target.shape:
        raise ValueError("pred and target must have the same shape")
    pred, target = _aligned16(pred), _aligned16(target)
    n = pred.numel()
    blocks = int(lib.unetpp_focal_bce_blocks(n))
    partial = torch.empty(blocks, dtype=torch.float32, device=pred.device)
    grad = torch.empty_like(pred) if want_grad else None
    loss = torch.empty(1, dtype=torch.float32, device=pred.device)
    check(lib.unetpp_focal_bce(_ptr(pred), _ptr(target), n, rows, float(gamma), _ptr(grad), _ptr(partial), _ptr(loss),
                               _stream()), "unetpp_focal_bce")
    return loss.reshape(()), grad


def focal_bce_heads(preds, target: torch.Tensor, rows: int, gamma: float, want_grad: bool = True, ignore: bool = False):
    lib = _lib.lib()
    if not 1 <= len(preds) <= _lib.MAX_HEADS:
        raise ValueError("1 to %d heads" % _lib.MAX_HEADS)
    _need(target, "target")
    for p in preds:
        _need(p, "pred")
        if p.shape != target.shape:
            raise ValueError("pred and target must have the same shape")
    preds, target = [_aligned16(p) for p in preds], _aligned16(target)
    n = target.numel()
    blocks = int(lib.unetpp_focal_bce_blocks(n))
    partial = torch.empty(len(preds) * blocks, dtype=torch.float32, device=target.device)
    grads = [torch.empty_like(p) for p in preds] if want_grad else None
    loss = torch.empty(1 + len(preds), dtype=torch.float32, device=target.device)
    hd = _lib.FocalHeads()
    hd.n_heads = len(preds)
    for i, p in enumerate(preds):
        hd.pred[i] = p.data_ptr()
        hd.grad[i] = grads[i].data_ptr() if want_grad else None
    fn = lib.unetpp_focal_bce_heads_ignore if ignore else lib.unetpp_focal_bce_heads
    check(fn(C.byref(hd), _ptr(target), n, rows, float(gamma), _ptr(partial), _ptr(loss), _stream()),
          "unetpp_focal_bce_heads_ignore" if ignore else "unetpp_focal_bce_heads")
    return loss, grads


def topk_focal_heads(preds, target: torch.Tensor, k: int, denom: int, gamma: float, want_grad: bool = True,
                     ignore: bool = False):
    lib = _lib.lib()
    if not 1 <= len(preds) <= _lib.MAX_HEADS:
        raise ValueError("1 to %d heads" % _lib.MAX_HEADS)
    _need(target, "target")
    if target.dim() < 3:
        raise ValueError("target must be [..., H, W]")
    for p in preds:
        _need(p, "pred")
        if p.shape != target.shape:
            raise ValueError("pred and target must have the same shape")
    if int(k) < 1 or int(denom) < 1:
        raise ValueError("k and denom must be at least 1")
    preds, target = [_aligned16(p) for p in preds], _aligned16(target)
    pixels = target.shape[-2] * target.shape[-1]
    rows = target.numel() // max(pixels, 1)
    nbytes = int(lib.unetpp_topk_focal_workspace_bytes(len(preds), rows, pixels))
    if nbytes <= 0:
        raise ValueError("topk_focal_heads: %d rows of %d pixels are outside what the kernel takes" % (rows, pixels))
    workspace = torch.empty(nbytes // 4, dtype=torch.float32, device=target.device)
    grads = [torch.empty_like(p) for p in preds] if want_grad else None
    loss = torch.empty(1 + len(preds), dtype=torch.float32, device=target.device)
    kth = torch.empty(len(preds), rows, dtype=torch.float32, device=target.device)
    hd = _lib.FocalHeads()
    hd.n_heads = len(preds)
    for i, p in enumerate(preds):
        hd.pred[i] = p.data_ptr()
        hd.grad[i] = grads[i].data_ptr() if want_grad else None
    fn = lib.unetpp_topk_focal_heads_ignore if ignore else lib.unetpp_topk_focal_heads
    check(fn(C.byref(hd), _ptr(target), rows, pixels, int(k), int(denom), float(gamma), _ptr(workspace), _ptr(kth),
             _ptr(loss), _stream()), "unetpp_topk_focal_heads_ignore" if ignore else "unetpp_topk_focal_heads")
    return loss, grads, kth


def pr_focal_heads(preds, target: torch.Tensor, alpha: float, beta: float, eps: float, positive: float,
                   want_grad: bool = True, ignore: bool = False):
    lib = _lib.lib()
    if not 1 <= len(preds) <= _lib.MAX_HEADS:
        raise ValueError("1 to %d heads" % _lib.MAX_HEADS)
    _need(target, "target")
    for p in preds:
        _need(p, "pred")
        if p.shape != target.shape:
            raise ValueError("pred and target must have the same shape")
    preds, target = [_aligned16(p) for p in preds], _aligned16(target)
    n = target.numel()
    nbytes = int(lib.unetpp_pr_focal_workspace_bytes(len(preds), n))
    if nbytes <= 0:
        raise ValueError("pr_focal_heads: %d elements are outside what the kernel takes" % n)
    workspace = torch.empty((nbytes + 7) // 8, dtype=torch.int64, device=target.device)
    grads = [torch.empty_like(p) for p in preds] if want_grad else None
    loss = torch.empty(1 + len(preds), dtype=torch.float32, device=target.device)
    n_pos = torch.empty((), dtype=torch.int64, device=target.device)
    hd = _lib.FocalHeads()
    hd.n_heads = len(preds)
    for i, p in enumerate(preds):
        hd.pred[i] = p.data_ptr()
        hd.grad[i] = grads[i].data_ptr() if want_grad else None
    fn = lib.unetpp_pr_focal_heads_ignore if ignore else lib.unetpp_pr_focal_heads
    check(fn(C.byref(hd), _ptr(target), n, float(alpha), float(beta), float(eps), float(positive), _ptr(workspace),
             _ptr(n_pos), _ptr(loss), _stream()), "unetpp_pr_focal_heads_ignore" if ignore else "unetpp_pr_focal_heads")
    return loss, grads, n_pos


def create_heatmap(points: torch.Tensor, height: int, width: int, radius: float = 3.0) -> torch.Tensor:
    lib = _lib.lib()
# ... 445 lines not shown
```

Baseline: 1737.

## Fuse BatchNorm backward sums into the Winograd dgrad conv epilogue

Adds a Winograd dgrad kernel mode that, while it writes d_a1, also reads the saved BN output y and accumulates the per-channel relu-masked dbeta and dgamma partial sums into per-workgroup rows. A finalize step then reduces the rows, so the separate BN backward reduce pass over d_a1 and y is skipped and only the apply pass remains. The goal is to save one full read of two fp32 activation tensors per conv pair in backward. In exchange the epilogue does extra loads of y and the BN coefficients and uses more LDS and registers, which may lower occupancy. It falls back to the old path when the Winograd lean mode does not apply.

```diff
diff --git a/include/unetpp_hip.h b/include/unetpp_hip.h
--- a/include/unetpp_hip.h
+++ b/include/unetpp_hip.h
@@ -13,6 +13,7 @@
 #define UNETPP_OK 0
 #define UNETPP_EINVAL (-1)
 #define UNETPP_ELAUNCH (-2)
+#define UNETPP_NOT_TAKEN 1
 
 typedef struct unetpp_view {
   float* ptr;
@@ -92,6 +93,18 @@
 } unetpp_gemm_sizes;
 int unetpp_gemm_plan(const unetpp_gemm_desc* d, int32_t cus, unetpp_gemm_sizes* out);
 int unetpp_gemm_fwd(const unetpp_gemm_desc* d, void* stream);
+typedef struct unetpp_bn_bwd_sums {
+  const float* y;
+  const float* scale;
+  const float* shift;
+  const float* mean;
+  const float* invstd;
+  float* rows;
+  float* dgamma;
+  float* dbeta;
+} unetpp_bn_bwd_sums;
+int unetpp_gemm_dgrad_bn_sums(const unetpp_gemm_desc* d, const unetpp_bn_bwd_sums* b, int32_t cus, unetpp_gemm_sizes* plan,
+                              void* stream);
 int64_t unetpp_gemm_weight_image_floats(const unetpp_gemm_desc* d);
 int unetpp_gemm_pack_weight_image(const unetpp_gemm_desc* d, float* image, void* stream);
 typedef struct unetpp_weight_src {
diff --git a/unet_nested4tiny_objects_keypoints_amd/_lib.py b/unet_nested4tiny_objects_keypoints_amd/_lib.py
--- a/unet_nested4tiny_objects_keypoints_amd/_lib.py
+++ b/unet_nested4tiny_objects_keypoints_amd/_lib.py
@@ -127,6 +127,16 @@
     ]
 
 
+class BnBwdSums(C.Structure):
+    _fields_ = [
+        ("y", C.c_void_p), ("scale", C.c_void_p), ("shift", C.c_void_p), ("mean", C.c_void_p), ("invstd", C.c_void_p),
+        ("rows", C.c_void_p), ("dgamma", C.c_void_p), ("dbeta", C.c_void_p),
+    ]
+
+
+NOT_TAKEN = 1
+
+
 class OptimSegment(C.Structure):
     _fields_ = [
         ("param", C.c_void_p), ("grad", C.c_void_p), ("exp_avg", C.c_void_p), ("exp_avg_sq", C.c_void_p),
@@ -189,6 +199,7 @@
     "unetpp_gemm_stats_rows": (_I64, [_I32, _I32, _I32]),
     "unetpp_gemm_plan": (C.c_int, [C.POINTER(GemmDesc), _I32, C.POINTER(GemmSizes)]),
     "unetpp_gemm_fwd": (C.c_int, [C.POINTER(GemmDesc), _P]),
+    "unetpp_gemm_dgrad_bn_sums": (C.c_int, [C.POINTER(GemmDesc), C.POINTER(BnBwdSums), _I32, C.POINTER(GemmSizes), _P]),
     "unetpp_gemm_weight_image_floats": (_I64, [C.POINTER(GemmDesc)]),
     "unetpp_gemm_pack_weight_image": (C.c_int, [C.POINTER(GemmDesc), _P, _P]),
     "unetpp_gemm_pack_weight_image_from": (C.c_int, [C.POINTER(GemmDesc), C.POINTER(WeightSrc), _P, _P]),
diff --git a/unet_nested4tiny_objects_keypoints_amd/csrc/common.h b/unet_nested4tiny_objects_keypoints_amd/csrc/common.h
--- a/unet_nested4tiny_objects_keypoints_amd/csrc/common.h
+++ b/unet_nested4tiny_objects_keypoints_amd/csrc/common.h
@@ -169,6 +169,7 @@
   OPT_PW_NT,
   OPT_HEAD_WGS_PER_CU,
   OPT_SMALL_WGRAD_BLOCKS,
+  OPT_BN_BWD_EPILOGUE,
   OPT_COUNT
 };
 bool opt_is_set(Opt o);
@@ -176,7 +177,7 @@
 
 struct FastArgs;
 struct GemmSel;
-int gemm_select(const unetpp_gemm_desc* d, int cus, GemmSel& s);
+int gemm_select(const unetpp_gemm_desc* d, int cus, GemmSel& s, bool bn_bwd = false);
 bool gemm_image_of(const unetpp_gemm_desc* d, GemmSel& s);
 bool small_cin_fwd_applies(const unetpp_gemm_desc* d);
 void small_cin_fwd_plan(const unetpp_gemm_desc* d, GemmSel& s);
@@ -191,6 +192,8 @@
 bool wino_applies(const unetpp_gemm_desc* d);
 void gemm_wino_plan(const unetpp_gemm_desc* d, GemmSel& s);
 int launch_gemm_wino(const unetpp_gemm_desc* d, const GemmSel& s, hipStream_t st);
+bool gemm_wino_bn_bwd_applies(const unetpp_gemm_desc* d, GemmSel& s);
+int launch_gemm_wino_bn_bwd(const unetpp_bn_bwd_sums* b, const GemmSel& s, hipStream_t st);
 bool gemm_pw_applies(const unetpp_gemm_desc* d, GemmSel& s);
 int launch_gemm_pw(const unetpp_gemm_desc* d, const GemmSel& s, hipStream_t st);
 void gemm_fast_plan(const unetpp_gemm_desc* d, GemmSel& s);
diff --git a/unet_nested4tiny_objects_keypoints_amd/csrc/gemm_pix.hip b/unet_nested4tiny_objects_keypoints_amd/csrc/gemm_pix.hip
--- a/unet_nested4tiny_objects_keypoints_amd/csrc/gemm_pix.hip
+++ b/unet_nested4tiny_objects_keypoints_amd/csrc/gemm_pix.hip
@@ -176,7 +176,7 @@
 const char* const kOptNames[OPT_COUNT] = {
     "BF16_NO_DMA", "BF16_DMA_ALL", "BF16_DMA_MIN8", "BF16_DMA_FORM", "BF16_DMA_SMALL", "BF16_DMA_STATS",
     "BF16_DMA_POINTWISE", "BF16_DMA_SPLIT", "BF16_WGRAD_QUAD", "WINO_NO_LEAN", "WINO_ONE_PER_CU", "MEMSET_NODES",
-    "BF16_PW_PLAIN", "PW_DIRECT", "PW_NT", "HEAD_WGS_PER_CU", "SMALL_WGRAD_BLOCKS"};
+    "BF16_PW_PLAIN", "PW_DIRECT", "PW_NT", "HEAD_WGS_PER_CU", "SMALL_WGRAD_BLOCKS", "BN_BWD_EPILOGUE"};
 struct OptSlot {
   std::atomic<long> value{0};
   std::atomic<bool> set{false};
@@ -332,7 +332,7 @@
 }
 }
 
-int unetpp::gemm_select(const unetpp_gemm_desc* d, int cus, GemmSel& s) {
+int unetpp::gemm_select(const unetpp_gemm_desc* d, int cus, GemmSel& s, bool bn_bwd) {
   if (d == nullptr || d->N <= 0 || d->H <= 0 || d->W <= 0) return UNETPP_EINVAL;
   if (d->taps != 9 && d->taps != 1) return UNETPP_EINVAL;
   if (d->n_in < 1 || d->n_in > UNETPP_MAX_VIEWS || d->n_out < 1 || d->n_out > UNETPP_MAX_VIEWS) return UNETPP_EINVAL;
@@ -363,6 +363,7 @@
     if (!gemm_pw_bf16_applies(d, s) && !gemm_bf16_dma_applies(d, s)) gemm_bf16_plan(d, s);
   } else if (wino_applies(d)) {
     gemm_wino_plan(d, s);
+    if (bn_bwd) gemm_wino_bn_bwd_applies(d, s);
   } else if (!gemm_pw_applies(d, s)) {
     gemm_fast_plan(d, s);
   }
@@ -398,6 +399,7 @@
     case GEMM_WINO: rc = launch_gemm_wino(d, s, st); break;
     case GEMM_FAST: rc = launch_gemm_fast(d, s, st); break;
     case GEMM_GENERIC: rc = launch_gemm_generic(d, s, st); break;
+    case GEMM_WINO_BN_BWD: rc = UNETPP_EINVAL; break;
   }
   const unetpp_bn_fused& bn = d->bn;
   if (rc != UNETPP_OK || bn.scale == nullptr) return rc;
@@ -408,3 +410,27 @@
   note_kernel(s.label);
   return fin;
 }
+
+extern "C" int unetpp_gemm_dgrad_bn_sums(const unetpp_gemm_desc* d, const unetpp_bn_bwd_sums* b, int32_t cus,
+                                         unetpp_gemm_sizes* plan, void* stream) {
+  if (b == nullptr || !b->y || !b->scale || !b->shift || !b->mean || !b->invstd || !b->rows || !b->dgamma || !b->dbeta)
+    return UNETPP_EINVAL;
+  GemmSel s;
+  int rc = gemm_select(d, (plan != nullptr && cus > 0) ? cus : device_cu_count(), s, true);
+  if (rc != UNETPP_OK) return rc;
+  if (s.kernel != GEMM_WINO_BN_BWD) return UNETPP_NOT_TAKEN;
+  if (plan != nullptr) {
+    plan->image_floats = s.image_floats;
+    plan->bn_rows = s.bn_rows;
+    plan->workgroups = static_cast<int32_t>(s.grid_x * s.grid_y);
+    plan->threads = static_cast<int32_t>(s.threads);
+    plan->kernel = s.label;
+    return UNETPP_OK;
+  }
+  note_kernel(s.label);
+  rc = launch_gemm_wino_bn_bwd(b, s, static_cast<hipStream_t>(stream));
+  if (rc != UNETPP_OK) return rc;
+  const int fin = unetpp_bn_bwd_finalize(b->rows, s.bn_rows, d->out[0].c_len, b->dgamma, b->dbeta, stream);
+  note_kernel(s.label);
+  return fin;
+}
diff --git a/unet_nested4tiny_objects_keypoints_amd/csrc/gemm_units.h b/unet_nested4tiny_objects_keypoints_amd/csrc/gemm_units.h
--- a/unet_nested4tiny_objects_keypoints_amd/csrc/gemm_units.h
+++ b/unet_nested4tiny_objects_keypoints_amd/csrc/gemm_units.h
@@ -70,7 +70,8 @@
 
 constexpr int kKindFast = 0, kKindWino = 1, kKindBf16 = 2;
 enum GemmKernel {
-  GEMM_SMALL_CIN, GEMM_BF16_PW, GEMM_BF16_DMA8, GEMM_BF16_DMA4, GEMM_BF16, GEMM_PW, GEMM_WINO, GEMM_FAST, GEMM_GENERIC
+  GEMM_SMALL_CIN, GEMM_BF16_PW, GEMM_BF16_DMA8, GEMM_BF16_DMA4, GEMM_BF16, GEMM_PW, GEMM_WINO, GEMM_FAST, GEMM_GENERIC,
+  GEMM_WINO_BN_BWD
 };
 struct GemmSel {
   GemmKernel kernel;
diff --git a/unet_nested4tiny_objects_keypoints_amd/csrc/gemm_wino.hip b/unet_nested4tiny_objects_keypoints_amd/csrc/gemm_wino.hip
--- a/unet_nested4tiny_objects_keypoints_amd/csrc/gemm_wino.hip
+++ b/unet_nested4tiny_objects_keypoints_amd/csrc/gemm_wino.hip
@@ -63,7 +63,8 @@
 
 template <int LOG2TW, int NH, int MODE, bool BNF = false>
 __global__ __launch_bounds__(kThreads, 2) void gemm_wino_kernel(const FastArgs a) {
-  constexpr bool LEAN = MODE != 0, FOLD = MODE == 2;
+  constexpr bool LEAN = MODE != 0, FOLD = MODE == 2, BWD = MODE == 3;
+  static_assert(!BWD || BNF, "the backward sums leave as per-workgroup rows");
   constexpr int TW = 1 << LOG2TW, TH = kBlockPixels >> LOG2TW;
   constexpr int HWp = TW + 2, HHp = TH + 2;
   constexpr int NPIX = HWp * HHp;
@@ -82,6 +83,8 @@
   __shared__ float stat_lds[BNF ? RUN0 + kBnFusedMaxCols * 2 : RUN0];
   constexpr int kBiasCols = 512;
   __shared__ __attribute__((aligned(16))) float bias_lds[kBiasCols];
+  constexpr int CO = kBnFusedMaxCols;
+  __shared__ __attribute__((aligned(16))) float coef_lds[BWD ? 4 * CO : 4];
 
   const unetpp_gemm_desc& d = a.d;
   const int tid = threadIdx.x;
@@ -93,6 +96,15 @@
   constexpr bool bn_fused = BNF;
   if constexpr (BNF) {
     for (int i = tid; i < kBnFusedMaxCols * 2; i += kThreads) stat_lds[RUN0 + i] = 0.f;
+  }
+  if constexpr (BWD) {
+    for (int i = tid; i < CO; i += kThreads) {
+      const bool in = i < a.Ncols;
+      coef_lds[0 * CO + i] = in ? a.d.bn.scale[i] : 0.f;
+      coef_lds[1 * CO + i] = in ? a.d.bn.shift[i] : 0.f;
+      coef_lds[2 * CO + i] = in ? a.d.bn.mean[i] : 0.f;
+      coef_lds[3 * CO + i] = in ? a.d.bn.invstd[i] : 0.f;
+    }
   }
   if (ur.count == 0) {
     if constexpr (BNF) {
@@ -340,7 +352,12 @@
     const float* gbase = O.gate != nullptr ? O.gate + tile_base : nullptr;
     const bool vec_out = ((O.C | O.c_off | tc.n_cnt) & 3) == 0 && (reinterpret_cast<uintptr_t>(O.ptr) & 15) == 0 &&
                          (O.gate == nullptr || (reinterpret_cast<uintptr_t>(O.gate) & 15) == 0);
-    const bool want_stats = d.stats_partial != nullptr;
+    const bool want_stats = BWD || d.stats_partial != nullptr;
+    auto bwd_sums = [&](float v, float yy, float sc, float sh, float mu, float is, float& t1, float& t2) {
+      const float gg = (fmaf(yy, sc, sh) > 0.f) ? v : 0.f;
+      t1 += gg;
+      t2 += gg * (yy - mu) * is;
+    };
     const float floor_v = O.relu ? 0.f : -__builtin_inff();
     float s1[NH][4], s2[NH][4];
 #pragma unroll
@@ -370,8 +387,18 @@
       y[1] = floor_keep_nan((tb[1] - tb[2]) - tb[3], floor_v);
     };
     if (interior && vec_out && tc.n_cnt == 16 * NH) {
-      const bool has_gate = gbase != nullptr, acc_out = O.accumulate != 0;
+      const bool has_gate = !BWD && gbase != nullptr, acc_out = !BWD && O.accumulate != 0;
       const unsigned lane_off = ty2 * rs + tx2 * cs + 4 * g;
+      f32x4 yt[2][2][NH];
+      if constexpr (BWD) {
+#pragma unroll
+        for (int ap = 0; ap < 2; ++ap)
+#pragma unroll
+          for (int bp = 0; bp < 2; ++bp)
+#pragma unroll
+            for (int nh = 0; nh < NH; ++nh)
+              yt[ap][bp][nh] = *reinterpret_cast<const f32x4*>(gbase + (lane_off + ap * rs + bp * cs + 16 * nh));
+      }
 #pragma unroll
       for (int ap = 0; ap < 2; ++ap) {
         unsigned off[2][NH];
@@ -411,7 +438,7 @@
           }
           yv[0][nh] = f32x4{y[0][0].x, y[0][0].y, y[0][1].x, y[0][1].y};
           yv[1][nh] = f32x4{y[1][0].x, y[1][0].y, y[1][1].x, y[1][1].y};
-          if (want_stats) {
+          if (!BWD && want_stats) {
 #pragma unroll
             for (int rr = 0; rr < 4; ++rr) {
               const float y0 = yv[0][nh][rr], y1 = yv[1][nh][rr];
@@ -428,6 +455,21 @@
               if constexpr (wino_exp::kNoOutStore) asm volatile("" ::"v"(yv[bp][nh]), "v"(off[bp][nh]));
               else *reinterpret_cast<f32x4*>(obase + off[bp][nh]) = yv[bp][nh];
             }
+          if constexpr (BWD) {
+#pragma unroll
+            for (int nh = 0; nh < NH; ++nh) {
+              const int c0 = tc.n0 + 16 * nh + 4 * g;
+              const f32x4 sc = *reinterpret_cast<const f32x4*>(&coef_lds[0 * CO + c0]);
+              const f32x4 sh = *reinterpret_cast<const f32x4*>(&coef_lds[1 * CO + c0]);
+              const f32x4 mu = *reinterpret_cast<const f32x4*>(&coef_lds[2 * CO + c0]);
+              const f32x4 is = *reinterpret_cast<const f32x4*>(&coef_lds[3 * CO + c0]);
+#pragma unroll
+              for (int rr = 0; rr < 4; ++rr)
+#pragma unroll
+                for (int bp = 0; bp < 2; ++bp)
+                  bwd_sums(yv[bp][nh][rr], yt[ap][bp][nh][rr], sc[rr], sh[rr], mu[rr], is[rr], s1[nh][rr], s2[nh][rr]);
+            }
+          }
           continue;
         }
 #pragma unroll
@@ -465,6 +507,13 @@
             for (int bp = 0; bp < 2; ++bp) {
               float v = y[bp];
               if ((col < tc.n_cnt) && (ug.ty0 + py < d.H) && (ug.tx0 + tx2 + bp < d.W)) {
+                if constexpr (BWD) {
+                  const int c = tc.n0 + col;
+                  bwd_sums(v, gbase[py * rs + (tx2 + bp) * cs + col], coef_lds[0 * CO + c], coef_lds[1 * CO + c],
+                           coef_lds[2 * CO + c], coef_lds[3 * CO + c], s1[nh][rr], s2[nh][rr]);
+                  obase[py * rs + (tx2 + bp) * cs + col] = v;
+                  continue;
+                }
                 s1[nh][rr] += v;
                 s2[nh][rr] = fmaf(v, v, s2[nh][rr]);
                 const unsigned off = py * rs + (tx2 + bp) * cs + col;
@@ -699,6 +748,44 @@
   s.mode = !lean ? 0 : (fold ? 2 : 1);
   s.fa.bn_in_kernel = (s.mode != 0 && bn_rows_per_workgroup(d, s.fa.Ncols)) ? 1 : 0;
   s.bn_rows = s.fa.bn_in_kernel ? s.grid_x : 0;
+}
+
+bool gemm_wino_bn_bwd_applies(const unetpp_gemm_desc* d, GemmSel& s) {
+  if (opt_value(OPT_BN_BWD_EPILOGUE, 1) == 0) return false;
+  if (s.kernel != GEMM_WINO || s.mode != 1) return false;
+  if (d->n_out != 1 || s.fa.Ncols > kBnFusedMaxCols || d->stats_partial != nullptr || d->bn.scale != nullptr) return false;
+  const unetpp_view& o = d->out[0];
+  if (o.c_off != 0 || o.c_len != o.C || o.Hs != d->H || o.Ws != d->W || o.sy != 1 || o.sx != 1 || o.oy != 0 || o.ox != 0)
+    return false;
+  if (o.gate != nullptr || o.accumulate != 0 || o.relu != 0) return false;
+  s.kernel = GEMM_WINO_BN_BWD;
+  s.label = "gemm_wino_kernel/bn_bwd_sums";
+  s.mode = 3;
+  s.fa.bn_in_kernel = 1;
+  s.bn_rows = s.grid_x;
+  return true;
+}
+
+int launch_gemm_wino_bn_bwd(const unetpp_bn_bwd_sums* b, const GemmSel& s, hipStream_t st) {
+  FastArgs a = s.fa;
+  a.d.out[0].gate = b->y;
+  a.d.stats_partial = b->rows;
+  a.d.bn.scale = const_cast<float*>(b->scale);
+  a.d.bn.shift = const_cast<float*>(b->shift);
+  a.d.bn.mean = const_cast<float*>(b->mean);
+  a.d.bn.invstd = const_cast<float*>(b->invstd);
+  const bool narrow = s.narrow != 0;
+  const dim3 grid(s.grid_x), block(kThreads);
+#define UNETPP_LAUNCH_WINO_BWD(L)                                                                        \
+  do {                                                                                                   \
+    if (narrow) hipLaunchKernelGGL((gemm_wino_kernel<L, 1, 3, true>), grid, block, 0, st, a);            \
+    else hipLaunchKernelGGL((gemm_wino_kernel<L, 2, 3, true>), grid, block, 0, st, a);                   \
+  } while (0)
+  if (a.log2tw == 5) UNETPP_LAUNCH_WINO_BWD(5);
+  else if (a.log2tw == 4) UNETPP_LAUNCH_WINO_BWD(4);
+  else UNETPP_LAUNCH_WINO_BWD(3);
+#undef UNETPP_LAUNCH_WINO_BWD
+  return launch_status();
 }
 
 int launch_gemm_wino(const unetpp_gemm_desc*, const GemmSel& s, hipStream_t st) {
diff --git a/unet_nested4tiny_objects_keypoints_amd/engine.py b/unet_nested4tiny_objects_keypoints_amd/engine.py
--- a/unet_nested4tiny_objects_keypoints_amd/engine.py
+++ b/unet_nested4tiny_objects_keypoints_amd/engine.py
@@ -488,7 +488,7 @@
 
 
 def _pair_bwd(blk, r: _PairRec, d_out, in_targets: Optional[List[V]], b, grads, pre_gated=False, pool_grad=None,
-              flush=None, in_slice: Optional[Tuple[int, int]] = None):
+              flush=None, in_slice: Optional[Tuple[int, int]] = None, bn1_sums_in_dgrad: bool = False):
     conv1, conv2 = getattr(blk.conv1, "0"), getattr(blk.conv2, "0")
     h, w = r.h, r.w
     if blk.is_batchnorm:
@@ -503,8 +503,17 @@
         if flush is not None:
             flush()
         d_a1 = torch.empty_like(r.y1)
-        ops.gemm_fwd(b, h, w, 9, [dy2], [V(d_a1)], pack_conv_dgrad(conv2.weight.detach()))
-        grads[bn1.weight], grads[bn1.bias] = _bn_bwd(bn1, r.bn1, r.frozen1, d_a1, r.y1, None)
+        if bn1_sums_in_dgrad and not r.frozen1 and r.y1.dtype == torch.float32:
+            dg, db = _new_grad(bn1.weight), _new_grad(bn1.bias)
+            if ops.gemm_dgrad_bn_sums(b, h, w, dy2, d_a1, pack_conv_dgrad(conv2.weight.detach()), r.y1, scale, shift, mean,
+                                      invstd, dg, db):
+                ops.bn_backward_apply(d_a1, r.y1, scale, shift, mean, invstd, bn1.weight.detach(), dg, db, d_a1)
+            else:
+                ops.bn_backward(d_a1, r.y1, scale, shift, mean, invstd, bn1.weight.detach(), d_a1, dg, db)
+            grads[bn1.weight], grads[bn1.bias] = dg, db
+        else:
+            ops.gemm_fwd(b, h, w, 9, [dy2], [V(d_a1)], pack_conv_dgrad(conv2.weight.detach()))
+            grads[bn1.weight], grads[bn1.bias] = _bn_bwd(bn1, r.bn1, r.frozen1, d_a1, r.y1, None)
         dy1 = V(d_a1)
     else:
         dy2 = V(d_out) if pre_gated else V(d_out, gate=r.out)
@@ -671,7 +680,7 @@
             targets = [V(d_up)]
             if grouped:
                 c_up = u.up.shape[3]
-                dy1s[(i, j)] = _pair_bwd(mod.conv, r, d_out, targets, b, grads, pre_gated, flush=flush, in_slice=(0, c_up))
+                dy1s[(i, j)] = _pair_bwd(mod.conv, r, d_out, targets, b, grads, pre_gated, flush=flush, bn1_sums_in_dgrad=True, in_slice=(0, c_up))
                 consumers = list(range(j, top + 1 - i))
                 t, acc, gate = book.target((i, j - 1), can_gate=True)
                 ops.gemm_fwd(b, r.h, r.w, 9, [dy1s[(i, jc)] for jc in consumers],
@@ -684,7 +693,7 @@
                 for jj in range(j):
                     t, acc, gate = book.target((i, jj), can_gate=True)
                     targets.append(V(t, accumulate=acc, gate=gate, gate_sum=True))
-                _pair_bwd(mod.conv, r, d_out, targets, b, grads, pre_gated, flush=flush)
+                _pair_bwd(mod.conv, r, d_out, targets, b, grads, pre_gated, flush=flush, bn1_sums_in_dgrad=True)
             t, acc, gate = book.target((i + 1, j - 1), can_gate=model.is_deconv or bf16)
             _up_bwd(mod.up, model.is_deconv, u, d_up, t, acc, gate, b, grads)
             flush()
@@ -701,7 +710,7 @@
         mine, pool_grad = pool_grad, None
         if i > 0:
             d_pooled = torch.empty_like(s.pairs[(i - 1, 0)].pooled)
-            _pair_bwd(blk, r, d_out, [V(d_pooled)], b, grads, pre_gated, pool_grad=mine, flush=flush)
+            _pair_bwd(blk, r, d_out, [V(d_pooled)], b, grads, pre_gated, pool_grad=mine, flush=flush, bn1_sums_in_dgrad=True)
             t, acc, _ = book.target((i - 1, 0))
             if not acc:
                 t.zero_()
@@ -710,9 +719,9 @@
             if bf16 and s.x_nhwc.shape[3] > 4:
                 raise NotImplementedError("bf16 storage: the input gradient needs at most 4 input channels")
             dx_in = torch.empty_like(s.x_nhwc)
-            _pair_bwd(blk, r, d_out, [V(dx_in)], b, grads, pre_gated, pool_grad=mine, flush=flush)
-        else:
-            _pair_bwd(blk, r, d_out, None, b, grads, pre_gated, pool_grad=mine, flush=flush)
+            _pair_bwd(blk, r, d_out, [V(dx_in)], b, grads, pre_gated, pool_grad=mine, flush=flush, bn1_sums_in_dgrad=True)
+        else:
+            _pair_bwd(blk, r, d_out, None, b, grads, pre_gated, pool_grad=mine, flush=flush, bn1_sums_in_dgrad=True)
         flush()
     return grads, dx_in
 
diff --git a/unet_nested4tiny_objects_keypoints_amd/ops.py b/unet_nested4tiny_objects_keypoints_amd/ops.py
--- a/unet_nested4tiny_objects_keypoints_amd/ops.py
+++ b/unet_nested4tiny_objects_keypoints_amd/ops.py
@@ -372,7 +372,7 @@
 
 def gemm_fwd(n: int, h: int, w: int, taps: int, ins: Sequence[V], outs: Sequence[V], weight: torch.Tensor,
              bias: Optional[torch.Tensor] = None, stats_partial: Optional[torch.Tensor] = None,
-             direct: bool = False, bn: Optional[BatchNormFinish] = None) -> _lib.GemmSizes:
+             direct: bool = False, bn: Optional[BatchNormFinish] = None, _launch=None) -> _lib.GemmSizes:
     if len(ins) > MAX_VIEWS or len(outs) > MAX_VIEWS:
         raise ValueError("too many views")
     d = GemmDesc()
@@ -439,10 +439,39 @@
             d.weight = packed.data_ptr()
         check(lib.unetpp_gemm_plan(C.byref(d), 0, C.byref(plan)), "unetpp_gemm_plan")
     acc = sum(v.c_len for v in d.out[:d.n_out] if v.accumulate) + sum(v.c_len for v in d.out[:d.n_out] if v.gate)
-    _timed_call(None, 2.0 * n * h * w * taps * k * nc,
-                lambda: check(lib.unetpp_gemm_fwd(C.byref(d), _stream()), "unetpp_gemm_fwd"),
+    if _launch is None:
+        _launch = lambda desc: check(lib.unetpp_gemm_fwd(C.byref(desc), _stream()), "unetpp_gemm_fwd")
+    _timed_call(None, 2.0 * n * h * w * taps * k * nc, lambda: _launch(d),
                 (2.0 if d.flags & _lib.GEMM_BF16 else 4.0) * n * h * w * (k + nc + acc))
     return plan
+
+
+def gemm_dgrad_bn_sums(n: int, h: int, w: int, dy: V, d_a1: torch.Tensor, weight, y: torch.Tensor, scale, shift, mean,
+                       invstd, dgamma: torch.Tensor, dbeta: torch.Tensor, direct: bool = False) -> bool:
+    if tuple(y.shape) != tuple(d_a1.shape) or _is_bf16(y) or _is_bf16(d_a1):
+        raise ValueError("y and d_a1 must be fp32 tensors of one shape")
+    nc = y.shape[3]
+    lib = _lib.lib()
+    rows = torch.empty(gemm_stats_rows(n, h, w) * nc * 2, dtype=torch.float32, device=y.device)
+    b = _lib.BnBwdSums()
+    b.y, b.rows = _need(y, "y").data_ptr(), rows.data_ptr()
+    b.scale, b.shift = _need(scale, "scale").data_ptr(), _need(shift, "shift").data_ptr()
+    b.mean, b.invstd = _need(mean, "mean").data_ptr(), _need(invstd, "invstd").data_ptr()
+    b.dgamma, b.dbeta = _need(dgamma, "dgamma").data_ptr(), _need(dbeta, "dbeta").data_ptr()
+    if any(t.numel() != nc for t in (scale, shift, mean, invstd, dgamma, dbeta)):
+        raise ValueError("BatchNorm vector length mismatch")
+    taken = []
+
+    def launch(desc):
+        rc = lib.unetpp_gemm_dgrad_bn_sums(C.byref(desc), C.byref(b), 0, None, _stream())
+        if rc == _lib.NOT_TAKEN:
+            check(lib.unetpp_gemm_fwd(C.byref(desc), _stream()), "unetpp_gemm_fwd")
+            return
+        check(rc, "unetpp_gemm_dgrad_bn_sums")
+        taken.append(True)
+
+    gemm_fwd(n, h, w, 9, [dy], [V(d_a1)], weight, direct=direct, _launch=launch)
+    return bool(taken)
 
 
 def first_layer_dgrad_bf16(dy: torch.Tensor, weight: torch.Tensor, dx: torch.Tensor) -> None:
@@ -593,6 +622,13 @@
                                            _ptr(gamma), _ptr(dgamma), _ptr(dbeta), _ptr(pool[0]), _ptr(pool[1]), n, h,
                                            w, c, _ptr(dy_out), st), "unetpp_bn_bwd_apply_pool")
     return dgamma, dbeta
+
+
+def bn_backward_apply(d_act, y, scale, shift, mean, invstd, gamma, dgamma, dbeta, dy_out):
+    n, h, w, c = y.shape
+    check(_lib.lib().unetpp_bn_bwd_apply(_ptr(d_act), _ptr(y), _ptr(scale), _ptr(shift), _ptr(mean), _ptr(invstd),
+                                         _ptr(gamma), _ptr(dgamma), _ptr(dbeta), n * h * w, c, _ptr(dy_out), _stream()),
+          "unetpp_bn_bwd_apply")
 
 
 def bn_frozen_backward(d_act, y, scale, shift, mean, invstd, dy_out, dgamma=None, dbeta=None, pool=None, want_sums=True):
```

Result: no change. 1752, median of 6 (+0.9%).
